# tambetm/simple_dqn

Hardware: AMD Instinct MI355X
Metric: train_steps/sec (batch=32, 4x84x84 uint8) (higher is better)
Workload: dtype f32; 1 GPU; BASELINE.json configs[1]: Breakout shapes, batch_size=32, replay_size=1000000, num_actions=4, HIP Q-net + device replay gather fused into conv1; global_batch=32, parallelism=dp1 (independent learners, RCCL grad all-reduce), ring=HBM mirror

## Files before the change

simple_dqn_amd/csrc/api_internal.h:

```cpp
#pragma once
#include <hip/hip_runtime.h>
#include <dlfcn.h>
#include <stdarg.h>
#include <stdio.h>
#include <stdlib.h>
#include <math.h>
#include <string.h>
#include <string>
#include <vector>
#include <chrono>
#include <thread>

#include "../../include/sdqn.h"
#include "kernels.h"
#include "generic_net.h"
#include "sampler.h"
#include "sdqn_per.h"

using namespace sdqn;


static constexpr int Q_SLOT_FLOATS = 8 * ACT_Q_STRIDE;
static constexpr int COST_RING = 64;
static constexpr int Q_SLOTS = 8;
// ... 44 lines not shown
};
inline bool replay_idx_ok(const sdqn_replay_s* r, int64_t i) {
  if (!r->lanes) return i >= r->hist && i + r->ns.n - 1 < r->count;
  if (i < 0 || i >= r->size) return false;
  const int64_t l = i % r->lane_len;
  return l >= r->hist && l + r->ns.n - 1 < r->lane_fill;
}
inline int64_t replay_filled(const sdqn_replay_s* r) { return r->lanes ? r->lanes * r->lane_fill : r->count; }
extern std::vector<sdqn_replay_s*> g_replays;

struct Id128 { char b[128]; };
struct Rccl {
  void* lib = nullptr;
  int (*GetUniqueId)(void*) = nullptr;
  int (*CommInitRank)(void**, int, Id128, int) = nullptr;
  int (*AllReduce)(const void*, void*, size_t, int, int, void*, hipStream_t) = nullptr;
  int (*Broadcast)(const void*, void*, size_t, int, int, void*, hipStream_t) = nullptr;
  int (*CommDestroy)(void*) = nullptr;
  int (*CommSplit)(void*, int, int, void**, void*) = nullptr;
  int (*CommAbort)(void*) = nullptr;
  int (*GroupStart)() = nullptr;
  int (*GroupEnd)() = nullptr;
  const char* (*GetErrorString)(int) = nullptr;
  int (*CommCount)(void*, int*) = nullptr;
  int (*CommUserRank)(void*, int*) = nullptr;
  int (*CommCuDevice)(void*, int*) = nullptr;
};
extern Rccl g_rccl;
#define NCCLCHK(x) do { int e_ = (x); if (e_ != 0) { set_error("%s -> %s", #x, g_rccl.GetErrorString ? g_rccl.GetErrorString(e_) : "rccl error"); return SDQN_ERR_RCCL; } } while (0)

struct ProfPair { int id; hipEvent_t a, b; };
struct sdqn_net_s {
  GenericNet* gen = nullptr;
  sdqn_net_cfg cfg; int B = 0, A = 0; int64_t NP = 0;
  int64_t NPW = 0;
  bool bn = false;
  float *x1 = nullptr, *x2 = nullptr, *x3 = nullptr;
  float *bn_mean = nullptr, *bn_rstd = nullptr; double* bn_partial = nullptr;
  float *theta = nullptr, *theta_t = nullptr, *state = nullptr, *state2 = nullptr, *g = nullptr;
  int epoch = 0;
  float *a1 = nullptr, *a2 = nullptr, *a3 = nullptr, *slab4 = nullptr, *a4 = nullptr, *d4 = nullptr;
  float *d3 = nullptr, *d2 = nullptr;
  half_t *h_a1 = nullptr, *h_a2 = nullptr, *h_a3 = nullptr, *h_d4 = nullptr, *h_d3p = nullptr, *h_d3 = nullptr,
         *h_d2p = nullptr, *h_d2 = nullptr, *h_d1 = nullptr, *wh[2] = {nullptr, nullptr}, *wht[2] = {nullptr, nullptr};
  float *d3p = nullptr, *d2p = nullptr, *d1 = nullptr, *slab1 = nullptr, *slab2 = nullptr, *slab3 = nullptr;
  float *q = nullptr, *maxq = nullptr, *dq = nullptr, *cost_terms = nullptr, *cost_out = nullptr; double* cost_accum = nullptr;
  bool double_dqn = false, slots3 = false;
  int n_step = 1;
  uint8_t *st_states = nullptr, *st_act = nullptr, *st_term = nullptr; int64_t* st_rew = nullptr; int64_t* d_idx = nullptr;
  float* h_f = nullptr;
  float *q_host = nullptr, *q_host_dev = nullptr;
  int q_slot = 0;
  bool head_q_system = false;
  float *act_scratch = nullptr, *act_q = nullptr; unsigned* act_ctl = nullptr; unsigned act_seq = 0;
  bool act_on = false, act_last = false, act_inject = false; int act_fallbacks = 0;
  int64_t tuple_calls = 0, tuple_states_skipped = 0, tuple_small_skipped = 0;
  double* cost_ring = nullptr; int cost_steps[64] = {0}; int64_t cost_ticket = 0;
  bool spec_pending = false; const void* spec_sb = nullptr; uint64_t spec_gen = 0;
  uint8_t* h_stage[2] = {nullptr, nullptr}; hipEvent_t stage_ev[2] = {nullptr, nullptr}; bool stage_busy[2] = {false, false}; int stage_next = 0;
  int S4 = 7, S4_cap = 7, tps1 = 1, tps2 = 1, tps3 = 1, ns1 = 1, ns2 = 1, ns3 = 1;
  int64_t train_iterations = 0;
  bool keep_grads = false;
  half_t* gh = nullptr; int* ovf_flag = nullptr; int64_t* ovf_count = nullptr;
  int dp_half = 1, dp_half_scale_log2 = -1;
  bool h16_wgrad_mfma = true;
  int c1w_in_wgrads = 1;
  bool half_payload_pending = false;
  bool grad_only = false;
  int nw_override[12] = {0};
  int f4_share[2] = {100, 0};
  int ns_cap[3] = {1, 1, 1};
  bool bt_xcd = true;
  bool bt_on = true; int bt[K_COUNT] = {0};
  int xcd_mask[K_COUNT] = {0};
  bool xcd_map = false;
  bool conv1_bf16 = true;
  unsigned short* w1p[2] = {nullptr, nullptr};
  const int64_t* host_idx_cur = nullptr;
  int r3_xcd = 2;
  bool prep_inline = true;
  int wt = WT_ALL;
  int conv1w_bf16 = 1;
  bool conv3_c36 = true;
  bool fused_launches = true;
  bool prof_on = false; int prof_filter = -1;
  int prof_mode = 1;
  int prof_every = 1; int64_t prof_seen[K_COUNT] = {0};
  std::vector<ProfPair> prof_pending; std::vector<hipEvent_t> prof_free;
  double prof_ms[K_COUNT]; int64_t prof_n[K_COUNT];
  void* comm = nullptr; int rank = 0, nranks = 1; int nccl_rc = 0;
  void* comm2 = nullptr; hipEvent_t ev_g4 = nullptr, ev_w4 = nullptr; bool w4_pending = false;
  bool dp_sync_replicas = true;
  int dp_overlap_req = -1;
  bool dp_overlap = false;
  int dp_probe_result = -1;
  int wt_kid = -1; unsigned long long* wt_words = nullptr;
  uint8_t* col_win = nullptr; void* col_recs = nullptr; int col_N = 0; int64_t col_t = 0; size_t col_state = 0; int col_game = 0;
  std::vector<void*> allocs;
};
#define GENCHK(x) do { hipError_t ge_ = (x); if (ge_ != hipSuccess) { set_error("%s -> %s", #x, hipGetErrorString(ge_)); return ge_ == hipErrorInvalidValue ? SDQN_ERR_ARG : SDQN_ERR_HIP; } } while (0)

constexpr int SB_SLOTS = 64;
uint64_t next_statebuf_gen();
struct sdqn_statebuf_s {
  uint8_t* d = nullptr;
  uint8_t* host = nullptr;
  uint8_t* stage = nullptr;
  int hist = 0;
  int64_t frame = 0;
  int pos = 0;
  uint64_t gen = next_statebuf_gen();
};

enum StepStructure { STEP_FUSED = 0, STEP_H16_BT = 1, STEP_DP_OVERLAP = 2, STEP_UNFUSED = 3 };
enum UpdateForm { UPD_SINGLE = 0, UPD_DP_SERIAL = 1, UPD_DP_OVERLAP = 2, UPD_GRAD_ONLY = 3 };
int ensure_stream();
int sample_checked(uint32_t* mt, const uint8_t* terminals, int64_t count, int64_t current, int hist,
                          int batch, int64_t* idx_out, int64_t* draws_out, int nstep = 1);
int sample_checked_lanes(uint32_t* mt, const uint8_t* terminals, int lanes, int64_t lane_len, int64_t fill, int64_t pos, int hist,
                         int batch, int64_t* idx_out, int64_t* draws_out, int nstep);
int replay_sample_uniform(sdqn_replay_s* r, uint32_t* mt, int64_t* idx_out, int64_t* draws_out);
int nstep_match(const sdqn_net_s* h, const sdqn_replay_s* r);
double nstep_gamma_n(int n, double gamma);
int replay_free(sdqn_replay_s* r);
int64_t replay_add_meta(sdqn_replay_s* r, int action, int64_t reward, int terminal);
int replay_add_commit(sdqn_replay_s* r, int64_t c);
int replay_flush_pending(sdqn_replay_s* r);
int replay_push_idx(sdqn_replay_s* r, const int64_t* idx, int* slot_out, const int64_t** dev);
int replay_release_idx(sdqn_replay_s* r, int slot);
int replay_release_idx_batched(sdqn_replay_s* r, int slot, bool flush);
GatherArgs gather_args(sdqn_replay_s* r, const int64_t* didx);
int replay_gather_generic(sdqn_replay_s* r, const int64_t* didx);
int rccl_load(const char* path);
int dalloc(sdqn_net_s* h, void** p, size_t bytes, bool zero = true);
int net_free(sdqn_net_s* h);
float* which_buf(sdqn_net_s* h, int which);
bool bn_layer_span(sdqn_net_s* h, int which, int layer, float** base, int64_t* n);
int gen_set(sdqn_net_s* h, int which, int layer, const void* w, int64_t n, bool f64);
int gen_get(sdqn_net_s* h, int which, int layer, void* w, int64_t n, bool f64);
int prof_collect(sdqn_net_s* h);
int prof_event(sdqn_net_s* h, hipEvent_t* e);
hipError_t dp_allreduce(sdqn_net_s* h, void* buf, size_t count, int dtype, void* comm, hipStream_t s);
StepArgs step_args(sdqn_net_s* h);
HeadArgs head_args(sdqn_net_s* h, int train);
int join_comm(sdqn_net_s* h);
BnArgs bn_args(sdqn_net_s* h, const StepArgs& a, int layer, int train);
hipError_t launch_tuned(sdqn_net_s* h, int id, StepArgs a, hipStream_t s, int variant = 0);
int run_forward(sdqn_net_s* h, const StepArgs& a, const HeadArgs& hd);
UpdateArgs make_update_args(sdqn_net_s* h, const StepArgs& a);
StepStructure step_structure(const sdqn_net_s* h);
UpdateForm update_form(const sdqn_net_s* h);
int run_train(sdqn_net_s* h, const StepArgs& a, const HeadArgs& hd, const PrepArgs* next = nullptr);
int read_cost(sdqn_net_s* h, float* cost_out);
int read_mean_cost(sdqn_net_s* h, int n_steps, float* mean_cost);
int predict_forward_tuned(sdqn_net_s* h, const uint8_t* states, const HeadArgs& hd, int B = 0);
int predict_forward(sdqn_net_s* h, const uint8_t* states, int rows, const void** q, int* q_f64);
StepArgs ring_step_args(sdqn_net_s* h, const sdqn_replay_s* r);
int run_ring_step(sdqn_net_s* h, sdqn_replay_s* r, const int64_t* host_idx, const HeadArgs& hd, const PrepArgs* next = nullptr);
int check_replay_geometry(const sdqn_net_s* h, const sdqn_replay_s* r);
bool act_sum_partials(const float* part, int A, float* q_out);
const uint8_t* statebuf_window(sdqn_statebuf_s* s);
int statebuf_advance(sdqn_statebuf_s* s, uint8_t** host_frame, uint8_t** dev_slot);
int predict_state_enqueue(sdqn_net_s* h, sdqn_statebuf_s* sb);
bool act_trace();
int predict_state_collect(sdqn_net_s* h, float* q_out);
PrepArgs prep_args(sdqn_net_s* h, sdqn_replay_s* r, const int64_t* pinned_idx);
// ... 47 lines not shown
```

simple_dqn_amd/csrc/gemm_engine.h:

```cpp
#pragma once
#include <hip/hip_runtime.h>
#include <string.h>
#include "problems.h"
#include "launch.h"

namespace sdqn {

typedef float f32x16 __attribute__((ext_vector_type(16)));

template <class P, class = void> struct a_elem { typedef float type; };
template <class P> struct a_elem<P, decltype((void)sizeof(typename P::AT))> { typedef typename P::AT type; };
template <class P, class = void> struct b_elem { typedef float type; };
template <class P> struct b_elem<P, decltype((void)sizeof(typename P::BT))> { typedef typename P::BT type; };
template <class P, class = void> struct stages_lds { static constexpr bool value = false; };
template <class P> struct stages_lds<P, decltype((void)P::STAGE_LDS)> { static constexpr bool value = P::STAGE_LDS; };
template <class P> struct Staged : P { static constexpr bool STAGE_LDS = true; };
template <class P, class = void> struct a_group4 { static constexpr bool value = false; };
template <class P> struct a_group4<P, decltype((void)P::A_GROUP4)> { static constexpr bool value = P::A_GROUP4; };
template <class P, class = void> struct uses_f16_wgrad { static constexpr bool value = false; };
template <class P> struct uses_f16_wgrad<P, decltype((void)P::F16_WGRAD)> { static constexpr bool value = P::F16_WGRAD; };
template <class P, class = void> struct has_preload { static constexpr bool value = false; };
template <class P> struct has_preload<P, decltype((void)P::PRELOAD)> { static constexpr bool value = P::PRELOAD; };
template <class P, class = void> struct has_preload_multi { static constexpr bool value = false; };
template <class P> struct has_preload_multi<P, decltype((void)P::PRELOAD_MULTI)> { static constexpr bool value = P::PRELOAD_MULTI; };
template <class P, class = void> struct uses_f16_mfma { static constexpr bool value = false; };
template <class P> struct uses_f16_mfma<P, decltype((void)P::F16_MFMA)> { static constexpr bool value = P::F16_MFMA; };

constexpr int PANEL = 32 * 33;

__device__ __forceinline__ void wave_lds_sync() {
  __builtin_amdgcn_fence(__ATOMIC_RELEASE, "wavefront");
  __builtin_amdgcn_wave_barrier();
  __builtin_amdgcn_fence(__ATOMIC_ACQUIRE, "wavefront");
}


__device__ __forceinline__ int pick_half(int v, int s, bool hi) {
  const int lo = __builtin_amdgcn_readlane(v, s), up = __builtin_amdgcn_readlane(v, s + 4);
  return hi ? up : lo;
}
__device__ __forceinline__ int64_t pick_half(int64_t v, int s, bool hi) {
  const int i = s;
  const int l0 = __builtin_amdgcn_readlane((int)(v & 0xFFFFFFFF), i), l1 = __builtin_amdgcn_readlane((int)(v >> 32), i);
  const int u0 = __builtin_amdgcn_readlane((int)(v & 0xFFFFFFFF), i + 4), u1 = __builtin_amdgcn_readlane((int)(v >> 32), i + 4);
  const int64_t lo = ((int64_t)l1 << 32) | (uint32_t)l0, up = ((int64_t)u1 << 32) | (uint32_t)u0;
  return hi ? up : lo;
}

#ifdef SDQN_TIMING
__device__ unsigned long long* g_sdqn_dbg = nullptr;
#define SDQN_STAMP(ph) do { if (g_sdqn_dbg && threadIdx.x == 0) g_sdqn_dbg[((size_t)(blockIdx.x + gridDim.x * (blockIdx.y + gridDim.y * blockIdx.z)) * 8) + (ph)] = clock64(); } while (0)
__device__ unsigned long long* g_sdqn_wdbg = nullptr;
__device__ unsigned g_sdqn_wdbg_blocks = 0;
#define SDQN_WSTAMP_DECL unsigned long long wst_[4] = {0, 0, 0, 0}
#define SDQN_WSTAMP(ph) do { if (wst_[ph] == 0) wst_[ph] = clock64(); } while (0)
#define SDQN_WSTAMP_FLUSH do { unsigned long long* wd_ = g_sdqn_wdbg; if (wd_ && (threadIdx.x & 63) == 0) { \
  const size_t b_ = (size_t)(blockIdx.x + gridDim.x * (blockIdx.y + gridDim.y * blockIdx.z)); const unsigned nb_ = g_sdqn_wdbg_blocks; \
  if (b_ < nb_ && (threadIdx.x >> 6) < 16) { \
    for (int q_ = 0; q_ < 4; ++q_) wd_[(b_ * 16 + (threadIdx.x >> 6)) * 4 + q_] = wst_[q_]; \
    if (threadIdx.x == 0) { unsigned x_; asm volatile("s_getreg_b32 %0, hwreg(HW_REG_XCC_ID, 0, 4)" : "=s"(x_)); wd_[(size_t)nb_ * 64 + b_] = x_; } } } } while (0)
#else
#define SDQN_STAMP(ph) do {} while (0)
#define SDQN_WSTAMP_DECL do {} while (0)
#define SDQN_WSTAMP(ph) do {} while (0)
#define SDQN_WSTAMP_FLUSH do {} while (0)
#endif

template <class P, int NW>
constexpr int tile_lds() {
  return NW * PANEL * (stages_lds<P>::value && (P::A_K || P::B_K) ? ((P::A_K ? 1 : 0) + (P::B_K ? 1 : 0)) : 1);
}

__device__ __forceinline__ constexpr int kslot(int t, int h) { return 8 * (t >> 2) + 4 * h + (t & 3); }

template <class T>
__device__ __forceinline__ T ld_byte_off(const T* base, uint32_t byte_off) {
  return *reinterpret_cast<const T*>(reinterpret_cast<const char*>(base) + byte_off);
}

template <class P, int NW, int NT>
__device__ __forceinline__ void gemm_tile(const StepArgs& a, int bx, int by, int bz, float* smem) {
  constexpr bool STG = stages_lds<P>::value;
  constexpr bool STG_A = STG && P::A_K, STG_B = STG && P::B_K;
  constexpr int WAVE_LDS = PANEL * ((STG_A || STG_B) ? ((STG_A ? 1 : 0) + (STG_B ? 1 : 0)) : 1);
  typedef typename P::aoff_t aoff_t;

  SDQN_STAMP(0);
  SDQN_WSTAMP_DECL;
  const int lane = threadIdx.x & 63;
  const int wave = __builtin_amdgcn_readfirstlane(threadIdx.x >> 6);
  const int m0 = bx * 32, n0 = by * 32;
  int z, ks, kbeg, kend;
  P::ksplit(a, bz, z, ks, kbeg, kend);
  if (NW * 64 < NT && wave >= NW) kend = kbeg;
  const int M = P::M(a), N = P::N(a);
  const int hb = lane >> 5;
  const bool hi = lane >= 32;

  const int mrow = m0 + (lane & 31), ncol = n0 + (lane & 31);
  const aoff_t arow = P::a_row(a, z, mrow < M ? mrow : M - 1);
  const int bcol = P::b_col(a, z, ncol < N ? ncol : N - 1);
  typedef typename a_elem<P>::type AT; typedef typename b_elem<P>::type BT;
  const AT* abase = P::a_ptr(a, z);
  const BT* bbase = P::b_ptr(a, z);
  const AT* areg = nullptr; const BT* breg = nullptr;
  if constexpr (!P::A_K && P::A_REG) areg = abase + (uint32_t)arow + (hi ? 4 * P::A_LD : 0);
  if constexpr (!P::B_K && P::B_REG) breg = bbase + (uint32_t)bcol + (hi ? 4 * P::B_LD : 0);
// ... 296 lines not shown
      else pa = P::a_ptr(a, z) + (uint32_t)(arow16 + P::a_col(a, z, kk));
      pa0 = ld_half8(pa); pa1 = ld_half8(pa + 8);
      if (kl >= kend) { pa0 = zero; pa1 = zero; }
    }
  };
  int kc = kbeg + (wave < NW ? wave : 0) * 32;
  if (kc < kend) stage_load(kc);
  while (kc < kend) {
    *reinterpret_cast<half8*>(sb + i * HW_PITCH + 16 * hb) = pb0;
    *reinterpret_cast<half8*>(sb + i * HW_PITCH + 16 * hb + 8) = pb1;
    if constexpr (!P::A_U8) {
      *reinterpret_cast<half8*>(sa + i * HW_PITCH + 16 * hb) = pa0;
      *reinterpret_cast<half8*>(sa + i * HW_PITCH + 16 * hb + 8) = pa1;
    }
    const aoff_t cv = cvn;
    const int kcur = kc;
    kc += NW * 32;
    if (kc < kend) stage_load(kc);
    wave_lds_sync();
#pragma unroll
    for (int s = 0; s < 2; ++s) {
      half8 fa, fb;
#pragma unroll
      for (int j = 0; j < 8; ++j) fb[j] = sb[(16 * s + 8 * hb + j) * HW_PITCH + i];
      if constexpr (P::A_U8) {
#pragma unroll
        for (int g = 0; g < 2; ++g) {
          const int src = 16 * s + 4 * g;
          const int l0 = __builtin_amdgcn_readlane((int)(cv & 0xFFFFFFFF), src), l1 = __builtin_amdgcn_readlane((int)((int64_t)cv >> 32), src);
          const int u0 = __builtin_amdgcn_readlane((int)(cv & 0xFFFFFFFF), src + 8), u1 = __builtin_amdgcn_readlane((int)((int64_t)cv >> 32), src + 8);
          const int64_t lo = ((int64_t)l1 << 32) | (uint32_t)l0, up = ((int64_t)u1 << 32) | (uint32_t)u0;
          const int64_t c = hi ? up : lo;
          const bool ok = kcur + 16 * s + 8 * hb + 4 * g < kend;
          const f4 v = P::a_load_group4(a, z, arow_own + c);
          fa[4 * g] = ok ? (half_t)v.x : (half_t)0.0f; fa[4 * g + 1] = ok ? (half_t)v.y : (half_t)0.0f;
          fa[4 * g + 2] = ok ? (half_t)v.z : (half_t)0.0f; fa[4 * g + 3] = ok ? (half_t)v.w : (half_t)0.0f;
        }
      } else {
#pragma unroll
        for (int j = 0; j < 8; ++j) fa[j] = sa[(16 * s + 8 * hb + j) * HW_PITCH + i];
      }
      acc = __builtin_amdgcn_mfma_f32_32x32x16_f16(fa, fb, acc, 0, 0, 0);
    }
    wave_lds_sync();
  }

  if constexpr (NW > 1) {
    if (wave < NW) {
      float* cw = smem + wave * HW_WAVE_LDS;
#pragma unroll
      for (int r = 0; r < 16; ++r) cw[((r & 3) + 8 * (r >> 2) + 4 * hb) * 33 + i] = acc[r];
    }
    __syncthreads();
    for (int e = threadIdx.x; e < 1024; e += NT) {
      const int ml = e >> 5, nl = e & 31;
      float v = smem[ml * 33 + nl];
#pragma unroll
      for (int w = 1; w < NW; ++w) v += smem[w * HW_WAVE_LDS + ml * 33 + nl];
      if (m0 + ml < M && n0 + nl < N) P::store(a, z, ks, m0 + ml, n0 + nl, v);
    }
  } else {
    float v[16];
#pragma unroll
    for (int r = 0; r < 16; ++r) v[r] = acc[r];
    P::store16(a, z, ks, m0, n0, lane, M, N, v, epi);
  }
}

template <class P, int NW, int NT>
__device__ __forceinline__ void run_tile(const StepArgs& a, int bx, int by, int bz, float* smem) {
  if constexpr (uses_f16_wgrad<P>::value) gemm_tile_hw<P, NW, NT>(a, bx, by, bz, smem);
  else if constexpr (uses_f16_mfma<P>::value) gemm_tile_h<P, NW, NT>(a, bx, by, bz, smem);
  else gemm_tile<P, NW, NT>(a, bx, by, bz, smem);
}
template <class P, int NW>
constexpr int tile_lds_any() {
  if constexpr (uses_f16_wgrad<P>::value) return NW * HW_WAVE_LDS;
  else return uses_f16_mfma<P>::value ? NW * PANEL : tile_lds<P, NW>();
}
template <class P> constexpr int tile_m() { return 32; }
template <class P> constexpr int tile_n() { return 32; }


template <class P, int NW>
__global__ void __launch_bounds__(NW * 64) gemm_kernel(const StepArgs a) {
  __shared__ float smem[tile_lds_any<P, NW>()];
  if constexpr (has_preload<P>::value) P::preload(a, gridDim.x, gridDim.y, gridDim.z);
  const int gx = gridDim.x, gy = gridDim.y;
  const int lin = blockIdx.x + gx * (blockIdx.y + gy * blockIdx.z);
  const int t = (a.xcd_map & 1) ? xcd_tile_id(lin, gx * gy * gridDim.z) : lin;
  const int bz = t / (gx * gy), r = t - bz * (gx * gy);
  run_tile<P, NW, NW * 64>(a, r % gx, r / gx, bz, smem);
}

struct MultiDims { int n[3]; int gx[3], gy[3]; };

template <class P, int NW, int NT>
__device__ __forceinline__ void multi_dispatch(const StepArgs& a, const MultiDims& d, int which, int local, float* smem) {
  if constexpr (NW == 1) {
    const int wave = __builtin_amdgcn_readfirstlane(threadIdx.x >> 6);
    const int t = local * (NT / 64) + wave;
    const int per_z = d.gx[which] * d.gy[which];
    if (t < a.f4w_count) {
      const int tile = a.f4w_first + t;
      const int bz = tile / per_z, r = tile - bz * per_z;
      run_tile<P, 1, 64>(a, r % d.gx[which], r / d.gx[which], bz, smem);
    }
  } else {
    const int per_z = d.gx[which] * d.gy[which];
    const int bz = local / per_z, r = local - bz * per_z;
    run_tile<P, NW, NT>(a, r % d.gx[which], r / d.gx[which], bz, smem);
  }
}

template <int NT, class P0, int NW0, class P1, int NW1, class P2, int NW2>
__global__ void __launch_bounds__(NT) gemm_multi_kernel(const StepArgs a, const MultiDims d) {
  constexpr int L0 = tile_lds_any<P0, NW0>() * (NW0 == 1 ? NT / 64 : 1), L1 = tile_lds_any<P1, NW1>() * (NW1 == 1 ? NT / 64 : 1),
                L2 = tile_lds_any<P2, NW2>() * (NW2 == 1 ? NT / 64 : 1);
  constexpr int L = L0 > L1 ? (L0 > L2 ? L0 : L2) : (L1 > L2 ? L1 : L2);
  __shared__ float smem[L];
  if constexpr (has_preload_multi<P1>::value) P1::preload_multi(a, d);
  const int b = blockIdx.x;
  const int xm = a.xcd_map;
  if (b < d.n[0]) multi_dispatch<P0, NW0, NT>(a, d, 0, (xm & 1) ? xcd_tile_id_range(b, 0, d.n[0]) : b, smem);
  else if (b < d.n[0] + d.n[1]) multi_dispatch<P1, NW1, NT>(a, d, 1, (xm & 2) ? xcd_tile_id_range(b, d.n[0], d.n[1]) : b - d.n[0], smem);
  else multi_dispatch<P2, NW2, NT>(a, d, 2, (xm & 4) ? xcd_tile_id_range(b, d.n[0] + d.n[1], d.n[2]) : b - d.n[0] - d.n[1], smem);
}

struct NoProblem {
  static constexpr bool A_K = false, B_K = false; typedef int aoff_t; struct Epi {};
  static constexpr bool A_REG = false, A_U8 = false, B_REG = false; static constexpr int A_LD = 0, B_LD = 0;
  SDQN_HD static const float* a_ptr(const StepArgs&, int) { return nullptr; }
  SDQN_HD static const float* b_ptr(const StepArgs&, int) { return nullptr; }
  SDQN_HD static int M(const StepArgs&) { return 0; }
  SDQN_HD static int N(const StepArgs&) { return 0; }
  SDQN_HD static int nbz(const StepArgs&) { return 0; }
  SDQN_HD static void ksplit(const StepArgs&, int, int& z, int& ks, int& kb, int& ke) { z = ks = kb = ke = 0; }
  SDQN_HD static int a_row(const StepArgs&, int, int) { return 0; }
  SDQN_HD static int a_col(const StepArgs&, int, int) { return 0; }
  SDQN_HD static float a_load(const StepArgs&, int, int) { return 0.f; }
  SDQN_HD static f4 a_load4(const StepArgs&, int, int) { f4 o; o.x = o.y = o.z = o.w = 0.f; return o; }
  SDQN_HD static f4 b_load4(const StepArgs&, int, int) { f4 o; o.x = o.y = o.z = o.w = 0.f; return o; }
  SDQN_HD static int b_row(const StepArgs&, int, int) { return 0; }
  SDQN_HD static int b_col(const StepArgs&, int, int) { return 0; }
  SDQN_HD static float b_load(const StepArgs&, int, int) { return 0.f; }
  SDQN_HD static void store(const StepArgs&, int, int, int, int, float) {}
  __device__ static void epi_begin(const StepArgs&, int, int, int, Epi&) {}
  __device__ static void store16(const StepArgs&, int, int, int, int, int, int, int, const float*, Epi&) {}
};

template <class P, int NW>
inline hipError_t launch_gemm(const StepArgs& a, hipStream_t stream) {
  dim3 grid((P::M(a) + tile_m<P>() - 1) / tile_m<P>(), (P::N(a) + tile_n<P>() - 1) / tile_n<P>(), P::nbz(a));
  SDQN_LAUNCH((gemm_kernel<P, NW>), grid, dim3(NW * 64), 0, stream, a);
  return hipGetLastError();
}

template <int NT, class P, int NW>
inline void multi_fill(const StepArgs& a, MultiDims& d, int i) {
  d.gx[i] = (P::M(a) + tile_m<P>() - 1) / tile_m<P>(); d.gy[i] = (P::N(a) + tile_n<P>() - 1) / tile_n<P>();
  const int tiles = d.gx[i] * d.gy[i] * P::nbz(a);
  d.n[i] = NW == 1 ? (a.f4w_count + NT / 64 - 1) / (NT / 64) : tiles;
}
template <int NT, class P0, int NW0, class P1, int NW1, class P2, int NW2>
inline hipError_t launch_multi(const StepArgs& a, bool has1, bool has2, hipStream_t stream) {
  static_assert(NW0 * 64 <= NT && NW1 * 64 <= NT && NW2 * 64 <= NT, "waves per tile exceed the workgroup");
  MultiDims d; memset(&d, 0, sizeof d);
  multi_fill<NT, P0, NW0>(a, d, 0);
  if (has1) multi_fill<NT, P1, NW1>(a, d, 1);
  if (has2) multi_fill<NT, P2, NW2>(a, d, 2);
  if (d.n[0] + d.n[1] + d.n[2] == 0) return hipSuccess;
  SDQN_LAUNCH((gemm_multi_kernel<NT, P0, NW0, P1, NW1, P2, NW2>), dim3(d.n[0] + d.n[1] + d.n[2]), dim3(NT), 0, stream, a, d);
  return hipGetLastError();
}

}
```

simple_dqn_amd/csrc/kernels.h:

```cpp
#pragma once
#include <cstddef>
#include <hip/hip_runtime.h>
#include "problems.h"
#include "launch.h"

namespace sdqn {

enum KernelId {
  K_CONV1_FWD = 0, K_CONV2_FWD, K_CONV3_FWD, K_FC4_FWD, K_HEAD,
  K_FC4_DGRAD, K_FC4_WGRAD, K_CONV3_DGRAD, K_CONV3_WGRAD, K_CONV2_DGRAD, K_CONV2_WGRAD,
  K_CONV1_WGRAD, K_UPDATE, K_ALLREDUCE, K_GATHER, K_PREP,
  K_BWD3,
  K_BWD2,
  K_BWD1,
  K_BN,
  K_RESERVED_20, K_RESERVED_21, K_RESERVED_22, K_RESERVED_23,
  K_WGRADS,
  K_ACT,
  K_COLLECT,
  K_COUNT
};
static_assert(K_BN == 19 && K_WGRADS == 24 && K_ACT == 25 && K_COLLECT == 26 && K_COUNT == 27, "kernel ids are public numbers");
const char* kernel_name(int id);


struct HeadArgs {
  const uint8_t* st_actions;
  const int64_t* st_rewards;
  const uint8_t* st_terminals;
  float* q;
  float* maxq;
  float* dq;
  float* cost_terms;
  double discount, min_reward, max_reward;
  float clip_error;
  int train;
  int reserved_[6];
  const float* per_w; float* per_p; double per_alpha, per_eps;
  int nstep; double gamma_n;
};

struct PrepArgs {
  const int64_t* idx_pinned;
  const MetaRec* meta;
  int64_t* idx;
  uint8_t* actions;
  int64_t* rewards;
  uint8_t* terminals;
  int B;
  int idx_in_valid;
  int64_t idx_in[32];
  NStepArgs ns;
};

struct UpdateArgs {
  float* theta;
  float* state;
  float* g;
  const float* slab[3];
  int ns[3];
  const float* dq;
  const float* a4;
  const float* cost_terms;
  float* cost_out;
  double* cost_accum;
  int B, A;
  int mode;
  int skip_fc4;
  int only_fc4;
  PrepArgs next;
  float bsz;
  float rho, one_minus_rho, lr, eps;
  int opt;
  float* state2;
  float beta1, one_minus_beta1, beta2, one_minus_beta2, lr_t;
  half_t* wh;
  half_t* wht;
  unsigned short* w1p;
  int reserved_[4];
  int wt;
  int reserved2_[3];
  int64_t bn_first;
  const int* ovf_flag;
  int64_t* ovf_count;
  int ovf_dynamic;
};

static_assert(sizeof(HeadArgs) == 160 && offsetof(HeadArgs, train) == 84 && offsetof(HeadArgs, per_w) == 112 && offsetof(HeadArgs, per_eps) == 136 &&
              offsetof(HeadArgs, nstep) == 144 && offsetof(HeadArgs, gamma_n) == 152, "HeadArgs layout");
static_assert(sizeof(PrepArgs) == 344 && offsetof(PrepArgs, idx_in_valid) == 52 && offsetof(PrepArgs, idx_in) == 56 && offsetof(PrepArgs, ns) == 312, "PrepArgs layout");
static_assert(sizeof(UpdateArgs) == 616 && offsetof(UpdateArgs, next) == 128 && offsetof(UpdateArgs, next) + offsetof(PrepArgs, idx_in) == 184 &&
              offsetof(UpdateArgs, bsz) == 472 && offsetof(UpdateArgs, w1p) == 544 && offsetof(UpdateArgs, wt) == 568 && offsetof(UpdateArgs, bn_first) == 584 &&
              offsetof(UpdateArgs, ovf_flag) == 592 && offsetof(UpdateArgs, ovf_count) == 600 && offsetof(UpdateArgs, ovf_dynamic) == 608, "UpdateArgs layout");

struct BnArgs {
  int layer;
  int C, rows;
  int nz;
  int train;
  const float* x;
  int S4, B;
  float* a;
  float* theta[2];
  int64_t off_bn;
  double* partial;
  float* mean; float* rstd;
  float* d;
  float* dpad;
  int PQ, Qw, PD, pad;
  float* g;
};

struct GatherArgs {
  const uint8_t* ring;
  const MetaRec* meta;
  const int64_t* idx;
  uint8_t* pre;
  uint8_t* post;
  uint8_t* actions;
  int64_t* rewards;
  uint8_t* terminals;
  int B;
  NStepArgs ns;
};

#if defined(__HIPCC__)
__device__ inline float opt_apply(float w, float& s1, float& s2, float gsum, const UpdateArgs& u) {
  if (u.opt == 0) return rms_step(w, s1, gsum, u.bsz, u.rho, u.one_minus_rho, u.lr, u.eps);
  const float g = div_bsz(gsum, u.bsz);
  if (u.opt == 1) {
    s1 = s1 * u.beta1 + u.one_minus_beta1 * g;
    s2 = s2 * u.beta2 + (u.one_minus_beta2 * g) * g;
    return w - (u.lr_t * s1) / (sqrtf(s2) + u.eps);
  }
  s1 = s1 * u.rho + (u.one_minus_rho * g) * g;
  const float upd = sqrtf((s2 + u.eps) / (s1 + u.eps)) * g;
  s2 = s2 * u.rho + (u.one_minus_rho * upd) * upd;
  return w - upd;
}
#endif

enum LaunchVariant {
  LV_CONV3_C36 = 2,
  LV_CONV1_FWD_BF16 = 4,
  LV_CONV1_WGRAD_BF16 = 8,
  LV_C1W_IN_WGRADS = 16,
  LV_C1W_FIRST = 32,
};
enum WriteThrough {
  WT_CONV2_FWD = 1, WT_CONV3_FWD = 2, WT_FC4_FWD = 4, WT_FC4_DGRAD = 8, WT_BWD3 = 16, WT_BWD2 = 32, WT_CONV1_WGRAD = 64, WT_CONV1_FWD = 128,
  WT_UPDATE = 256, WT_ALL = 511
};
struct LaunchTune {
  int nw_override[12];
  const int64_t* host_idx;
  int r3_xcd;
  int wt;
  int bt[K_COUNT];
  int variant;
};
hipError_t launch_kernel(int id, const StepArgs& a, const LaunchTune& t, hipStream_t s);
hipError_t launch_head(const StepArgs& a, const HeadArgs& h, hipStream_t s, bool q_system_scope = false);
// ... 30 lines not shown
```

simple_dqn_amd/csrc/problems.h:

```cpp
#pragma once
#include <stddef.h>
#include <stdint.h>
#include <math.h>

#if defined(__HIPCC__)
#define SDQN_HD __host__ __device__ inline
#else
#define SDQN_HD inline
#endif

namespace sdqn {

constexpr int H0 = 84, W0 = 84, C0 = 4;
constexpr int FRAME = H0 * W0;
constexpr int STATE = C0 * FRAME;
constexpr int ST1 = 4, P1 = 20, Q1 = 20, K1 = 32;
constexpr int ST2 = 2, P2 = 9, Q2 = 9, K2 = 64;
constexpr int P3 = 7, Q3 = 7, K3 = 64;
constexpr int PIX1 = P1 * Q1, PIX2 = P2 * Q2, PIX3 = P3 * Q3;
constexpr int CRS1 = 256, CRS2 = 512, CRS3 = 576;
constexpr int NFC = 512, NIN4 = PIX3 * K3;
constexpr int PD3 = 11, PD2 = 11;
constexpr int NW1 = CRS1 * K1, NW2 = CRS2 * K2, NW3 = CRS3 * K3, NW4 = NIN4 * NFC;
constexpr int OFF1 = 0, OFF2 = OFF1 + NW1, OFF3 = OFF2 + NW2, OFF4 = OFF3 + NW3, OFF5 = OFF4 + NW4;
constexpr int MAX_ACTIONS = 18;
constexpr int BN_LAYERS = 4;
constexpr int BN_PARAMS = 2 * (32 + 64 + 64 + 512);
SDQN_HD constexpr int bn_features(int l) { return l == 0 ? 32 : (l == 3 ? 512 : 64); }
SDQN_HD constexpr int bn_off(int l) { return l == 0 ? 0 : (l == 1 ? 64 : (l == 2 ? 192 : 320)); }

#if defined(__HIPCC__)
typedef _Float16 half_t;
typedef _Float16 half8 __attribute__((ext_vector_type(8)));
#else
typedef uint16_t half_t;
#endif

struct MetaRec {
  int64_t reward;
  uint8_t action;
  uint8_t terminal;
  uint8_t pad[6];
};

struct NStepArgs { int n, pad_; double gamma, min_reward, max_reward; };
SDQN_HD void nstep_return(const MetaRec* meta, int64_t i, const NStepArgs& s, double& R, uint8_t& done) {
  double r = 0.0, g = 1.0; uint8_t d = 0;
  for (int k = 0; k < s.n; ++k) {
    const MetaRec rec = meta[i + k];
    double c = (double)rec.reward;
    c = c < s.min_reward ? s.min_reward : (c > s.max_reward ? s.max_reward : c);
    r = r + g * c;
    if (rec.terminal) { d = 1; break; }
    g = g * s.gamma;
  }
  R = r; done = d;
}
SDQN_HD void stage_meta(const MetaRec* meta, int64_t i, const NStepArgs& s, uint8_t* act, int64_t* rew, uint8_t* term, int n) {
  const MetaRec rec = meta[i];
  act[n] = rec.action;
  if (s.n > 1) {
    double R; uint8_t d; nstep_return(meta, i, s, R, d);
    reinterpret_cast<double*>(rew)[n] = R; term[n] = d;
  } else { rew[n] = rec.reward; term[n] = rec.terminal; }
}

struct StepArgs {
  const uint8_t* src;
  const int64_t* idx;
  int from_ring;
  int B, A, nz;
  const float* theta[2];
  float* a1;
  float* a2;
  float* a3;
  float* slab4;
  float* a4;
  float* d4;
  float* d3p;
  float* d2p;
  float* d3;
  float* d2;
  float* d1;
  float* g;
  float* slab1;
  float* slab2;
  float* slab3;
  int S4;
  int tps1, tps2, tps3;
  int fuse_rms;
  int f4w_first, f4w_count;
  half_t *h_a1, *h_a2, *h_a3;
  half_t *h_d4, *h_d3p, *h_d3, *h_d2p, *h_d2, *h_d1;
  const half_t* wh[2];
  const half_t* wht[2];
  half_t *wh_w, *wht_w;
  float loss_scale, inv_loss_scale;
  int h16;
  int xcd_map;
  int post_off;
  int reserved_[11];
  float* __restrict__ theta_w;
  float* __restrict__ state;
  float bsz, rho, one_minus_rho, lr, eps;
  int bn;
  int reserved2_[6];
  const unsigned short* w1p[2];
  int reserved3_[8];
};

static_assert(sizeof(StepArgs) == 496 && offsetof(StepArgs, post_off) == 336 && offsetof(StepArgs, theta_w) == 384 && offsetof(StepArgs, bn) == 420 &&
              offsetof(StepArgs, w1p) == 448, "StepArgs layout: part of the tuned kernels (reserved_)");

SDQN_HD float div_bsz(float x, float bsz) {
  union { float f; uint32_t u; } b, r; b.f = bsz;
  if ((b.u & 0x007FFFFFu) == 0u && b.u >= 0x00800000u && b.u < 0x7E800000u) { r.u = 0x7F000000u - b.u; return x * r.f; }
  return x / bsz;
}
SDQN_HD float rms_step(float w, float& st, float gsum, float bsz, float rho, float omr, float lr, float eps) {
  const float g = div_bsz(gsum, bsz);
  st = rho * st + (g * g) * omr;
  return w - (g * lr) / (sqrtf(st + eps) + eps);
}

#if defined(__HIPCC__)
typedef float f2v __attribute__((ext_vector_type(2)));
__device__ inline void rms_step2(float& w0, float& w1, float& st0, float& st1, float gs0, float gs1,
                                 float bsz, float rho, float omr, float lr, float eps) {
  union { float f; uint32_t u; } b, r; b.f = bsz;
  f2v gsum = {gs0, gs1}, g;
  if ((b.u & 0x007FFFFFu) == 0u && b.u >= 0x00800000u && b.u < 0x7E800000u) { r.u = 0x7F000000u - b.u; g = gsum * r.f; }
  else { g.x = gs0 / bsz; g.y = gs1 / bsz; }
  f2v st = {st0, st1};
  const f2v a = rho * st, q = (g * g) * omr;
  st = a + q;
  const f2v num = g * lr, rad = st + eps;
  f2v den; den.x = sqrtf(rad.x); den.y = sqrtf(rad.y);
  den = den + eps;
  f2v quo; quo.x = num.x / den.x; quo.y = num.y / den.y;
  const f2v w = (f2v){w0, w1} - quo;
  w0 = w.x; w1 = w.y; st0 = st.x; st1 = st.y;
}
#endif

SDQN_HD uint16_t bf16_rn(float f) {
  union { float f; uint32_t u; } x; x.f = f;
  return (uint16_t)((x.u + 0x7FFFu + ((x.u >> 16) & 1u)) >> 16);
}
SDQN_HD float bf16_up(uint16_t b) { union { float f; uint32_t u; } x; x.u = (uint32_t)b << 16; return x.f; }
SDQN_HD void split_bf16x3(float w, uint16_t& hi, uint16_t& mid, uint16_t& lo) {
  hi = bf16_rn(w); const float r1 = w - bf16_up(hi);
  mid = bf16_rn(r1); const float r2 = r1 - bf16_up(mid);
  lo = bf16_rn(r2);
}
constexpr int W1P_PLANE = K1 * CRS1;

SDQN_HD int wslot(int z) { return z & 1; }
SDQN_HD int sslot(int z) { return z != 0 ? 1 : 0; }
SDQN_HD int soff(int post_off, int z) { return z != 0 ? post_off : 0; }
SDQN_HD int64_t slab4_row(const StepArgs& a, int ks, int z) { return z < 2 ? (int64_t)ks * 2 + z : (int64_t)2 * a.S4 + ks; }
SDQN_HD int64_t sbase(const StepArgs& a, int z, int n) {
  return a.from_ring ? (a.idx[n] - C0 + soff(a.post_off, z)) * (int64_t)FRAME : ((int64_t)sslot(z) * a.B + n) * (int64_t)STATE;
}
SDQN_HD float norm_u8(uint32_t v) {
  const float x = (float)v, r = 1.0f / 255.0f;
  const float q = x * r;
  const float e = fmaf(-q, 255.0f, x);
  return fmaf(e, r, q);
}
struct f4 { float x, y, z, w; };
SDQN_HD f4 ld4(const float* p) {
#if defined(__HIP_DEVICE_COMPILE__)
  const float4 v = *reinterpret_cast<const float4*>(p); f4 o; o.x = v.x; o.y = v.y; o.z = v.z; o.w = v.w; return o;
#else
  f4 o; o.x = p[0]; o.y = p[1]; o.z = p[2]; o.w = p[3]; return o;
#endif
}
constexpr int SRC_PAD = 16;
SDQN_HD f4 ld4_u8_stride4(const uint8_t* p) {
  f4 o;
#if defined(__HIP_DEVICE_COMPILE__)
  typedef uint32_t u32x4 __attribute__((ext_vector_type(4), aligned(1)));
  const u32x4 w = *reinterpret_cast<const u32x4*>(p);
  o.x = norm_u8(w.x & 255u); o.y = norm_u8(w.y & 255u); o.z = norm_u8(w.z & 255u); o.w = norm_u8(w.w & 255u);
// ... 491 lines not shown
```

simple_dqn_amd/csrc/problems_wt.h:

```cpp
#pragma once
#include "gemm_engine.h"

namespace sdqn {

#ifndef SDQN_NT_W4
#define SDQN_NT_W4 0
#endif
constexpr bool NT_W4 = SDQN_NT_W4 != 0;
#ifndef SDQN_PRELOAD
#define SDQN_PRELOAD 1
#endif
#define SDQN_TOUCH(...) asm volatile("" :: __VA_ARGS__)
#define SDQN_PRELOAD_MULTI_DEF \
  static constexpr bool PRELOAD_MULTI = SDQN_PRELOAD != 0; \
  __device__ static void preload_multi(const StepArgs& a, const MultiDims& d) { \
    SDQN_TOUCH("s"(a.d3p), "s"(a.theta[0]), "s"(a.a2), "s"(a.d2p), "s"(a.d2), "s"(a.d3), "s"(a.slab3), "s"(a.a3), "s"(a.d4), "s"(a.theta_w), "s"(a.state), \
               "s"(a.g), "s"(a.a1), "s"(a.d1), "s"(a.slab2), "s"(a.B), "s"(a.tps2), "s"(a.tps3), "s"(a.fuse_rms), "s"(a.f4w_first), "s"(a.f4w_count), \
               "s"(a.xcd_map), "s"(a.bsz), "s"(a.rho), "s"(a.one_minus_rho), "s"(a.lr), "s"(a.eps), "s"(d.n[0]), "s"(d.n[1]), "s"(d.gx[1])); \
  }
#ifdef SDQN_WT_PLAIN
__device__ __forceinline__ void wt_store(float* p, float v) { *p = v; }
#else
__device__ __forceinline__ void wt_store(float* p, float v) { __hip_atomic_store(p, v, __ATOMIC_RELAXED, __HIP_MEMORY_SCOPE_AGENT); }
#endif
struct Conv2FwdWT : Conv2Fwd {
  static constexpr bool PRELOAD = SDQN_PRELOAD != 0;
  __device__ static void preload(const StepArgs& a, unsigned g0, unsigned g1, unsigned g2) { SDQN_TOUCH("s"(a.a1), "s"(a.a2), "s"(a.theta[0]), "s"(a.theta[1]), "s"(a.B), "s"(a.nz), "s"(a.xcd_map), "s"(g0), "s"(g1), "s"(g2)); }

  __device__ static void store(const StepArgs& a, int z, int, int m, int n, float v) { wt_store(&a.a2[((int64_t)z * M(a) + m) * K2 + n], fmaxf(v, 0.0f)); }
};
struct Conv3FwdWT : Conv3Fwd {
  static constexpr bool PRELOAD = SDQN_PRELOAD != 0;
  __device__ static void preload(const StepArgs& a, unsigned g0, unsigned g1, unsigned g2) { SDQN_TOUCH("s"(a.a2), "s"(a.a3), "s"(a.theta[0]), "s"(a.theta[1]), "s"(a.B), "s"(a.nz), "s"(a.xcd_map), "s"(g0), "s"(g1), "s"(g2)); }

  __device__ static void store(const StepArgs& a, int z, int, int m, int n, float v) { wt_store(&a.a3[((int64_t)z * M(a) + m) * K3 + n], fmaxf(v, 0.0f)); }
};
__device__ __forceinline__ f4 ld4_nt(const float* p) {
  typedef float v4f __attribute__((ext_vector_type(4)));
  const v4f v = __builtin_nontemporal_load(reinterpret_cast<const v4f*>(p)); f4 o; o.x = v.x; o.y = v.y; o.z = v.z; o.w = v.w; return o;
}
struct Fc4FwdWT : Fc4Fwd {
  static constexpr bool PRELOAD = SDQN_PRELOAD != 0;
  __device__ static void preload(const StepArgs& a, unsigned g0, unsigned g1, unsigned g2) { SDQN_TOUCH("s"(a.a3), "s"(a.slab4), "s"(a.theta[0]), "s"(a.theta[1]), "s"(a.B), "s"(a.nz), "s"(a.S4), "s"(a.xcd_map), "s"(g0), "s"(g1), "s"(g2)); }

  __device__ static f4 b_load4(const StepArgs& a, int z, int o) { return NT_W4 ? ld4_nt(a.theta[wslot(z)] + OFF4 + o) : ld4(a.theta[wslot(z)] + OFF4 + o); }
  __device__ static void store(const StepArgs& a, int z, int ks, int m, int n, float v) { wt_store(&a.slab4[(slab4_row(a, ks, z) * a.B + m) * NFC + n], v); }
};
struct Fc4DgradWT : Fc4Dgrad {
  static constexpr bool PRELOAD = SDQN_PRELOAD != 0;
  __device__ static void preload(const StepArgs& a, unsigned g0, unsigned g1, unsigned g2) { SDQN_TOUCH("s"(a.d4), "s"(a.theta[0]), "s"(a.a3), "s"(a.d3p), "s"(a.d3), "s"(a.B), "s"(a.xcd_map), "s"(g0), "s"(g1), "s"(g2)); }

  __device__ static f4 b_load4(const StepArgs& a, int, int o) { return NT_W4 ? ld4_nt(a.theta[0] + OFF4 + o) : ld4(a.theta[0] + OFF4 + o); }
  static constexpr bool GATED = true;
  __device__ static float gate_load(const StepArgs& a, int, int m, int n) { return a.a3[(int64_t)m * NIN4 + n]; }
  __device__ static void store_gated(const StepArgs& a, int, int, int m, int n, float v, float g) {
    const int pix = n >> 6, f = n & 63, p = pix / Q3, q = pix - p * Q3;
    const float dv = g > 0.0f ? v : 0.0f;
    wt_store(&a.d3p[((m * PD3 + p + 2) * PD3 + q + 2) * K3 + f], dv);
    wt_store(&a.d3[(int64_t)m * NIN4 + n], dv);
  }
  __device__ static void store(const StepArgs& a, int z, int ks, int m, int n, float v) { store_gated(a, z, ks, m, n, v, gate_load(a, z, m, n)); }
};
struct Conv3DgradWT : Conv3Dgrad {
  static constexpr bool PRELOAD = SDQN_PRELOAD != 0;
  SDQN_PRELOAD_MULTI_DEF
  __device__ static void preload(const StepArgs& a, unsigned g0, unsigned g1, unsigned g2) { SDQN_TOUCH("s"(a.d3p), "s"(a.theta[0]), "s"(a.a2), "s"(a.d2p), "s"(a.d2), "s"(a.B), "s"(g0), "s"(g1), "s"(g2)); }

  static constexpr bool GATED = true;
  __device__ static float gate_load(const StepArgs& a, int, int m, int c) { return a.a2[(int64_t)m * K2 + c]; }
  __device__ static void store_gated(const StepArgs& a, int, int, int m, int c, float v, float g) {
    const float dv = g > 0.0f ? v : 0.0f;
    wt_store(&a.d2p[prow2(m) + c], dv);
    wt_store(&a.d2[(int64_t)m * K2 + c], dv);
  }
  __device__ static void store(const StepArgs& a, int z, int ks, int m, int c, float v) { store_gated(a, z, ks, m, c, v, gate_load(a, z, m, c)); }
};
struct Conv3WgradWT : Conv3Wgrad {
  static constexpr bool PRELOAD = SDQN_PRELOAD != 0;
  SDQN_PRELOAD_MULTI_DEF
  __device__ static void preload(const StepArgs& a, unsigned g0, unsigned g1, unsigned g2) { SDQN_TOUCH("s"(a.a2), "s"(a.d3), "s"(a.slab3), "s"(a.tps3), "s"(a.B), "s"(g0), "s"(g1), "s"(g2)); }

  __device__ static void store(const StepArgs& a, int, int ks, int m, int n, float v) { wt_store(&a.slab3[(int64_t)ks * NW3 + m * K3 + n], v); }
};
struct Conv2DgradWT : Conv2Dgrad {
  static constexpr bool PRELOAD = SDQN_PRELOAD != 0;
  SDQN_PRELOAD_MULTI_DEF
  __device__ static void preload(const StepArgs& a, unsigned g0, unsigned g1, unsigned g2) { SDQN_TOUCH("s"(a.d2p), "s"(a.theta[0]), "s"(a.a1), "s"(a.d1), "s"(a.B), "s"(g0), "s"(g1), "s"(g2)); }

  static constexpr bool GATED = true;
  __device__ static int out_off(int z, int m, int c) {
    const int py = z >> 1, px = z & 1;
    const int n = m / 100, pix = m - n * 100, i = pix / 10, j = pix - i * 10;
    return ((n * P1 + 2 * i + py) * Q1 + 2 * j + px) * K1 + c;
  }
  __device__ static float gate_load(const StepArgs& a, int z, int m, int c) { return a.a1[out_off(z, m, c)]; }
  __device__ static void store_gated(const StepArgs& a, int z, int, int m, int c, float v, float g) { wt_store(&a.d1[out_off(z, m, c)], g > 0.0f ? v : 0.0f); }
  __device__ static void store(const StepArgs& a, int z, int ks, int m, int c, float v) { store_gated(a, z, ks, m, c, v, gate_load(a, z, m, c)); }
};
struct Conv2WgradWT : Conv2Wgrad {
  static constexpr bool PRELOAD = SDQN_PRELOAD != 0;
  __device__ static void preload(const StepArgs& a, unsigned g0, unsigned g1, unsigned g2) { SDQN_TOUCH("s"(a.a1), "s"(a.d2), "s"(a.slab2), "s"(a.tps2), "s"(a.B), "s"(g0), "s"(g1), "s"(g2)); }

  __device__ static void store(const StepArgs& a, int, int ks, int m, int n, float v) { wt_store(&a.slab2[(int64_t)ks * NW2 + m * K2 + n], v); }
};
struct Conv1WgradWT : Conv1Wgrad {
  __device__ static void store(const StepArgs& a, int, int ks, int m, int n, float v) { wt_store(&a.slab1[(int64_t)ks * NW1 + m * K1 + n], v); }
};
struct Fc4WgradWT : Fc4Wgrad {
  __device__ static void preload(const StepArgs& a, unsigned g0, unsigned g1, unsigned g2) { SDQN_TOUCH("s"(a.a3), "s"(a.d4), "s"(a.theta_w), "s"(a.state), "s"(a.g), "s"(a.fuse_rms), "s"(a.f4w_first), "s"(a.f4w_count), "s"(a.B)); SDQN_TOUCH("s"(a.bsz), "s"(a.rho), "s"(a.one_minus_rho), "s"(a.lr), "s"(a.eps), "s"(g0), "s"(g1), "s"(g2)); }
  __device__ static void store(const StepArgs& a, int, int, int m, int n, float v) {
    const int64_t e = OFF4 + (int64_t)m * NFC + n;
    if (a.fuse_rms) { float st = a.state[e]; const float w = rms_step(a.theta_w[e], st, v, a.bsz, a.rho, a.one_minus_rho, a.lr, a.eps); wt_store(&a.theta_w[e], w); wt_store(&a.state[e], st); }
    else wt_store(&a.g[e], v);
  }
  __device__ static void store16(const StepArgs& a, int z, int ks, int m0, int n0, int lane, int M, int N, const float* v, Epi& e) {
    const uint32_t base = epi_base(m0, n0, lane);
    auto stw = [](float* p, uint32_t off, float x) { wt_store(reinterpret_cast<float*>(reinterpret_cast<char*>(p) + off), x); };
    if (!a.fuse_rms) {
#pragma unroll
      for (int r = 0; r < 16; ++r) stw(a.g, base + epi_row(r), v[r]);
      return;
    }
#pragma unroll
    for (int r = 0; r < 16; r += 2) rms_step2(e.w[r], e.w[r + 1], e.st[r], e.st[r + 1], v[r], v[r + 1], a.bsz, a.rho, a.one_minus_rho, a.lr, a.eps);
#pragma unroll
    for (int r = 0; r < 16; ++r) { stw(a.theta_w, base + epi_row(r), e.w[r]); stw(a.state, base + epi_row(r), e.st[r]); }
  }
};

struct Fc4WgradBT : Fc4WgradWT {
  struct Epi {};
  __device__ static void epi_begin(const StepArgs&, int, int, int, Epi&) {}
  static constexpr bool STORE_TILE = true;
  __device__ static void store_tile(const StepArgs& a, int m0, int n0, int lane, const float* v) {
    const uint32_t base = epi_base(m0, n0, lane);
    auto stw = [](float* p, uint32_t off, float x) { wt_store(reinterpret_cast<float*>(reinterpret_cast<char*>(p) + off), x); };
    if (!a.fuse_rms) {
#pragma unroll
      for (int r = 0; r < 16; ++r) stw(a.g, base + epi_row(r), v[r]);
      return;
    }
    const float* __restrict__ tw = a.theta_w; const float* __restrict__ sp = a.state;
#pragma unroll
    for (int g = 0; g < 4; ++g) {
      float w[4], st[4];
#pragma unroll
      for (int e = 0; e < 4; ++e) { w[e] = ldb(tw, base + epi_row(4 * g + e)); st[e] = ldb(sp, base + epi_row(4 * g + e)); }
      rms_step2(w[0], w[1], st[0], st[1], v[4 * g], v[4 * g + 1], a.bsz, a.rho, a.one_minus_rho, a.lr, a.eps);
      rms_step2(w[2], w[3], st[2], st[3], v[4 * g + 2], v[4 * g + 3], a.bsz, a.rho, a.one_minus_rho, a.lr, a.eps);
#pragma unroll
      for (int e = 0; e < 4; ++e) { stw(a.theta_w, base + epi_row(4 * g + e), w[e]); stw(a.state, base + epi_row(4 * g + e), st[e]); }
      __builtin_amdgcn_sched_barrier(0);
    }
  }
};

}
```

simple_dqn_amd/csrc/sdqn_api_net.hip:

```cpp
#include "api_internal.h"

static const char* const RETIRED_OPTIONS[] = {"hoist", "two_streams", "fuse_dbg", "fwd_rb", "head_f4d", "fuse_upd", "f4w_early", "bt_planes", "bt_x", "bwd_order", nullptr};
#define RETIRED_OPTION_REFUSED(NAME) do { set_error("option %s belonged to an experiment that was measured slower than the default step and has been removed from " \
                                                    "the library (tools/exp/README.md; tools/exp/experiments_r04.patch)", NAME); return SDQN_ERR_ARG; } while (0)

int dalloc(sdqn_net_s* h, void** p, size_t bytes, bool zero) {
  HIPCHK(hipMalloc(p, bytes)); h->allocs.push_back(*p);
  if (zero) HIPCHK(hipMemsetAsync(*p, 0, bytes, g_stream));
  return SDQN_OK;
}
int net_free(sdqn_net_s* h) {
  if (!h) return SDQN_OK;
  if (g_stream) hipStreamSynchronize(g_stream);
  delete h->gen; h->gen = nullptr;
  if (g_comm) hipStreamSynchronize(g_comm);
  if (h->comm2 && g_rccl.CommDestroy) g_rccl.CommDestroy(h->comm2);
  if (h->comm && g_rccl.CommDestroy) g_rccl.CommDestroy(h->comm);
  if (h->ev_g4) hipEventDestroy(h->ev_g4);
  if (h->ev_w4) hipEventDestroy(h->ev_w4);
  for (void* p : h->allocs) hipFree(p);
  hipHostFree(h->h_f);
  if (h->q_host) hipHostFree(h->q_host);
  if (h->cost_ring) hipHostFree(h->cost_ring);
  for (int i = 0; i < 2; ++i) { if (h->h_stage[i]) hipHostFree(h->h_stage[i]); if (h->stage_ev[i]) hipEventDestroy(h->stage_ev[i]); }
// ... 357 lines not shown
  if (h->gen) { GENCHK(h->gen->last_q(preq, maxpostq, false)); return SDQN_OK; }
  const size_t nq = (size_t)h->B * h->A;
  HIPCHK(hipMemcpyAsync(h->h_f, h->q, nq * 4, hipMemcpyDeviceToHost, g_stream));
  HIPCHK(hipMemcpyAsync(h->h_f + nq, h->maxq, (size_t)h->B * 4, hipMemcpyDeviceToHost, g_stream));
  HIPCHK(hipStreamSynchronize(g_stream));
  if (preq) memcpy(preq, h->h_f, nq * 4);
  if (maxpostq) memcpy(maxpostq, h->h_f + nq, (size_t)h->B * 4);
  return SDQN_OK;
}
extern "C" int sdqn_net_overflow_steps(sdqn_net_t h, int64_t* n) {
  ARGCHK(h && n, "NULL argument");
  *n = 0;
  if (!h->ovf_count) return SDQN_OK;
  { int rc = join_comm(h); if (rc) return rc; } HIPCHK(hipStreamSynchronize(g_stream));
  HIPCHK(hipMemcpy(n, h->ovf_count, 8, hipMemcpyDeviceToHost));
  return SDQN_OK;
}
extern "C" int sdqn_net_train_iterations(sdqn_net_t h, int64_t* n) { ARGCHK(h && n, "NULL"); *n = h->train_iterations; return SDQN_OK; }

extern "C" int sdqn_net_set_epoch(sdqn_net_t h, int epoch) { ARGCHK(h && epoch >= 0, "bad epoch"); h->epoch = epoch; return SDQN_OK; }

extern "C" int sdqn_net_set_option(sdqn_net_t h, const char* name, int value) {
  ARGCHK(h && name, "NULL argument");
  if (!strcmp(name, "n_step")) {
    ARGCHK(value >= 1 && value <= SDQN_MAX_N_STEP, "n_step %d out of range [1, %d]", value, SDQN_MAX_N_STEP);
    h->n_step = value;
    if (h->gen) h->gen->set_nstep(value, nstep_gamma_n(value, h->cfg.discount_rate));
    return SDQN_OK;
  }
  if (h->gen) {
    if (!strcmp(name, "dp_overlap") && value < 0) return SDQN_OK;
    if (!strcmp(name, "double_dqn")) {
      ARGCHK(value == 0 || value == 1, "double_dqn must be 0 or 1");
      GENCHK(h->gen->set_double_dqn(value != 0));
      return SDQN_OK;
    }
    if (!strcmp(name, "grad_only") || !strcmp(name, "dp_overlap") || !strcmp(name, "keep_gradients")) {
      ARGCHK(value == 0 || !strcmp(name, "keep_gradients"), "option %s is implemented for the 84x84x4 float32 / float16 configurations", name);
    }
    return SDQN_OK;
  }
  bool retired = !strncmp(name, "rb:", 3) || !strncmp(name, "btx:", 4);
  for (int i = 0; RETIRED_OPTIONS[i]; ++i) retired = retired || !strcmp(name, RETIRED_OPTIONS[i]);
  if (retired) { if (value) RETIRED_OPTION_REFUSED(name); return SDQN_OK; }
  if (!strcmp(name, "double_dqn")) {
    ARGCHK(value == 0 || value == 1, "double_dqn must be 0 or 1");
    if (value && !h->slots3) {
      { int rc_ = join_comm(h); if (rc_) return rc_; } HIPCHK(hipStreamSynchronize(g_stream));
      const size_t B = (size_t)h->B;
      float** f32[5] = {&h->a1, &h->a2, &h->a3, &h->a4, &h->q};
      const size_t n32[5] = {B * PIX1 * K1, B * PIX2 * K2, B * PIX3 * K3, B * NFC, B * h->A};
      for (int i = 0; i < 5; ++i) { int r_ = dalloc(h, (void**)f32[i], 3 * n32[i] * 4); if (r_) return r_; }
      { int r_ = dalloc(h, (void**)&h->slab4, (size_t)h->S4_cap * 3 * B * NFC * 4); if (r_) return r_; }
      if (h->h_a1) {
        half_t** f16[3] = {&h->h_a1, &h->h_a2, &h->h_a3};
        const size_t n16[3] = {B * PIX1 * K1, B * PIX2 * K2, B * PIX3 * K3};
        for (int i = 0; i < 3; ++i) { int r_ = dalloc(h, (void**)f16[i], 3 * n16[i] * 2); if (r_) return r_; }
      }
      HIPCHK(hipStreamSynchronize(g_stream));
      h->slots3 = true;
    }
    h->double_dqn = value != 0;
  }
  else if (!strcmp(name, "keep_gradients")) h->keep_grads = value != 0;
  else if (!strcmp(name, "grad_only")) h->grad_only = value != 0;
  else if (!strcmp(name, "h16_wgrad_mfma")) h->h16_wgrad_mfma = value != 0;
  else if (!strcmp(name, "c1w_in_wgrads")) { if (value < 0 || value > 2) { set_error("bad c1w_in_wgrads (0..2)"); return SDQN_ERR_ARG; } h->c1w_in_wgrads = value; }
  else if (!strcmp(name, "dp_half")) h->dp_half = value != 0;
  else if (!strcmp(name, "dp_half_scale_log2")) {
    ARGCHK(value >= -1 && value <= 40 && h->ovf_flag, "bad scale (or not a float16 network)");
    { int rc_ = join_comm(h); if (rc_) return rc_; } HIPCHK(hipStreamSynchronize(g_stream));
    h->dp_half_scale_log2 = value;
    const int st0[4] = {0, value < 0 ? 10 : value, 0, 0};
    HIPCHK(hipMemcpy(h->ovf_flag, st0, 16, hipMemcpyHostToDevice));
  }
  else if (!strcmp(name, "dp_half_scale_seed")) {
    ARGCHK(value >= 0 && value <= 15 && h->ovf_flag, "bad scale seed (0..15; float16 networks only)");
    { int rc_ = join_comm(h); if (rc_) return rc_; } HIPCHK(hipStreamSynchronize(g_stream));
    h->dp_half_scale_log2 = -1;
    const int st0[4] = {0, value, 0, 0};
    HIPCHK(hipMemcpy(h->ovf_flag, st0, 16, hipMemcpyHostToDevice));
  }
  else if (!strcmp(name, "fused_launches")) h->fused_launches = value != 0;
  else if (!strcmp(name, "conv1_bf16")) h->conv1_bf16 = value != 0;
  else if (!strcmp(name, "wt")) h->wt = value;
  else if (!strcmp(name, "prep_inline")) h->prep_inline = value != 0;
  else if (!strcmp(name, "r3_xcd")) h->r3_xcd = value;
  else if (!strcmp(name, "conv1w_bf16")) h->conv1w_bf16 = value;
  else if (!strcmp(name, "conv3_c36")) h->conv3_c36 = value != 0;
  else if (!strcmp(name, "xcd_map")) h->xcd_map = value != 0;
  else if (!strcmp(name, "dp_sync_replicas")) h->dp_sync_replicas = value != 0;
  else if (!strcmp(name, "dp_overlap")) {
    ARGCHK(value >= -2 && value <= 1, "dp_overlap must be -1 (auto), 0 or 1 (-2: auto also for a 1-rank communicator, tests)");
    ARGCHK(!h->comm, "dp_overlap is chosen before sdqn_dp_init (afterwards: sdqn_dp_set_overlap)");
    h->dp_overlap_req = value; h->dp_overlap = value == 1;
  }
  else if (!strcmp(name, "f4_share3")) h->f4_share[0] = value;
  else if (!strcmp(name, "f4_share2")) h->f4_share[1] = value;
  else if (!strcmp(name, "profile_mode")) { ARGCHK(value == 0 || value == 1, "profile_mode must be 0 (event markers) or 1 (kernel-packet timestamps)"); h->prof_mode = value; }
  else if (!strcmp(name, "profile_every")) { ARGCHK(value >= 1, "profile_every must be >= 1"); h->prof_every = value; }
  else if (!strncmp(name, "xcd:", 4)) {
    int id = atoi(name + 4);
    if (id < 0 || id >= K_COUNT || value < 0 || value > 8) { set_error("bad xcd override"); return SDQN_ERR_ARG; }
    h->xcd_mask[id] = value;
  }
  else if (!strcmp(name, "act_inject_failure")) {
    ARGCHK(h->act_scratch, "act_inject_failure needs a network with the one-launch acting forward");
    h->act_inject = value != 0;
  }
  else if (!strcmp(name, "act_kernel")) {
    ARGCHK(value == 0 || h->act_scratch, "act_kernel needs a float32 network without batch_norm");
    h->act_on = value != 0; h->spec_pending = false;
  }
  else if (!strcmp(name, "bt_xcd")) h->bt_xcd = value != 0;
  else if (!strcmp(name, "bt")) h->bt_on = value != 0;
  else if (!strncmp(name, "bt:", 3)) {
    int id = atoi(name + 3);
    if (id < 0 || id >= K_COUNT || value < -1 || value > (id == K_WGRADS ? 2 : 8)) { set_error("bad bt override"); return SDQN_ERR_ARG; }
    h->bt[id] = value;
  }
  else if (!strcmp(name, "s4")) {
    if (value < 1 || value > h->S4_cap) { set_error("bad s4 (1..%d)", h->S4_cap); return SDQN_ERR_ARG; }
    { int rc_ = join_comm(h); if (rc_) return rc_; } HIPCHK(hipStreamSynchronize(g_stream));
    h->S4 = value;
  }
  else if (!strncmp(name, "tps:", 4)) {
    int l = atoi(name + 4);
    if (l < 1 || l > 3 || value < 1) { set_error("bad tps override"); return SDQN_ERR_ARG; }
    const int pix[3] = {PIX1, PIX2, PIX3};
    const int T = ceil_div(h->B * pix[l - 1], 32), ns = ceil_div(T, value);
    if (ns > h->ns_cap[l - 1]) { set_error("tps:%d = %d needs %d slabs (%d allocated)", l, value, ns, h->ns_cap[l - 1]); return SDQN_ERR_ARG; }
    { int rc_ = join_comm(h); if (rc_) return rc_; } HIPCHK(hipStreamSynchronize(g_stream));
    if (l == 1) { h->tps1 = value; h->ns1 = ns; } else if (l == 2) { h->tps2 = value; h->ns2 = ns; } else { h->tps3 = value; h->ns3 = ns; }
  }
  else if (!strncmp(name, "nw:", 3)) {
    int id = atoi(name + 3);
    if (id < 0 || id >= 12 || !(value == 0 || value == 1 || value == 2 || value == 4 || value == 8 || value == 16 || (value == 9 && id == 2))) { set_error("bad nw override"); return SDQN_ERR_ARG; }
    h->nw_override[id] = value;
  }
  else { set_error("unknown option %s", name); return SDQN_ERR_ARG; }
  return SDQN_OK;
}

extern "C" int sdqn_net_debug_read(sdqn_net_t h, const char* name, float* out, int64_t n) {
  ARGCHK(h && name && out, "NULL argument");
  ARGCHK(!h->gen, "debug_read exposes the tuned path's internal buffers (84x84x4 float32 / float16 only)");
  const int B = h->B;
  struct { const char* n; float* p; int64_t len; } tab[] = {
    {"a1", h->a1, (int64_t)2 * B * PIX1 * K1}, {"a2", h->a2, (int64_t)2 * B * PIX2 * K2}, {"a3", h->a3, (int64_t)2 * B * PIX3 * K3},
    {"a4", h->a4, (int64_t)2 * B * NFC}, {"d4", h->d4, (int64_t)B * NFC}, {"d3p", h->d3p, (int64_t)B * PD3 * PD3 * K3},
    {"d2p", h->d2p, (int64_t)B * PD2 * PD2 * K2}, {"d1", h->d1, (int64_t)B * PIX1 * K1}, {"q", h->q, (int64_t)2 * B * h->A},
    {"dq", h->dq, (int64_t)B * h->A}, {"g", h->g, h->NP}, {"theta", h->theta, h->NP}, {"cost_terms", h->cost_terms, B}};
  for (auto& e : tab) if (!strcmp(e.n, name)) {
    ARGCHK(n <= e.len, "buffer %s holds %lld floats", name, (long long)e.len);
    { int rc_ = join_comm(h); if (rc_) return rc_; } HIPCHK(hipStreamSynchronize(g_stream));
    HIPCHK(hipMemcpy(out, e.p, (size_t)n * 4, hipMemcpyDeviceToHost));
    return SDQN_OK;
  }
  set_error("unknown buffer %s", name); return SDQN_ERR_ARG;
}

#ifdef SDQN_TIMING
namespace sdqn { hipError_t set_timing_buffer(unsigned long long* p); }
extern "C" int sdqn_debug_time_kernel(sdqn_net_t h, sdqn_replay_t r, const int64_t* idx_host, int kernel, unsigned long long* out, int max_blocks) {
  ARGCHK(h && r && idx_host && out, "NULL");
  unsigned long long* d = nullptr;
// ... 44 lines not shown
```

simple_dqn_amd/csrc/sdqn_api_step.hip:

```cpp
#include "api_internal.h"

hipError_t dp_allreduce(sdqn_net_s* h, void* buf, size_t count, int dtype, void* comm, hipStream_t s) {
  h->nccl_rc = g_rccl.AllReduce(buf, buf, count, dtype,  0, comm, s);
  return h->nccl_rc == 0 ? hipSuccess : hipErrorUnknown;
}

StepArgs step_args(sdqn_net_s* h) {
  StepArgs a; memset(&a, 0, sizeof a);
  a.B = h->B; a.A = h->A; a.nz = 2; a.theta[0] = h->theta; a.theta[1] = h->theta_t;
  a.a1 = h->a1; a.a2 = h->a2; a.a3 = h->a3; a.slab4 = h->slab4; a.a4 = h->a4; a.d4 = h->d4; a.d3p = h->d3p; a.d2p = h->d2p; a.d3 = h->d3; a.d2 = h->d2;
  a.d1 = h->d1; a.g = h->g; a.slab1 = h->slab1; a.slab2 = h->slab2; a.slab3 = h->slab3;
  a.S4 = h->S4; a.tps1 = h->tps1; a.tps2 = h->tps2; a.tps3 = h->tps3;

  a.xcd_map = h->xcd_map ? 7 : 0;
  if (h->cfg.datatype == 1) {
    a.h16 = h->h16_wgrad_mfma ? 2 : 1; a.h_a1 = h->h_a1; a.h_a2 = h->h_a2; a.h_a3 = h->h_a3; a.h_d4 = h->h_d4; a.h_d3p = h->h_d3p; a.h_d3 = h->h_d3;
    a.h_d2p = h->h_d2p; a.h_d2 = h->h_d2; a.h_d1 = h->h_d1; a.wh[0] = h->wh[0]; a.wh[1] = h->wh[1]; a.wht[0] = h->wht[0]; a.wht[1] = h->wht[1];
    a.wh_w = h->wh[0]; a.wht_w = h->wht[0];
    a.loss_scale = (float)h->cfg.loss_scale; a.inv_loss_scale = (float)(1.0 / h->cfg.loss_scale);
  }
  a.f4w_first = 0; a.f4w_count = (NIN4 / 32) * (NFC / 32);
  a.w1p[0] = h->w1p[0]; a.w1p[1] = h->w1p[1];
  a.fuse_rms = (!h->comm && !h->keep_grads && !h->grad_only && h->cfg.optimizer == 0) ? 1 : 0;
  a.theta_w = h->theta; a.state = h->state; a.bsz = (float)h->B;
  a.rho = (float)h->cfg.decay_rate; a.one_minus_rho = (float)(1.0 - h->cfg.decay_rate);
  a.lr = (float)h->cfg.learning_rate; a.eps = (float)h->cfg.epsilon;
  a.post_off = h->n_step;
  return a;
}
double nstep_gamma_n(int n, double gamma) { double g = 1.0; for (int k = 0; k < n; ++k) g = g * gamma; return g; }
int nstep_match(const sdqn_net_s* h, const sdqn_replay_s* r) {
  const int rn = r->ns.n > 1 ? r->ns.n : 1;
  if (rn == 1 && h->n_step == 1) return SDQN_OK;
  ARGCHK(rn == h->n_step, "replay memory n_step %d != network n_step %d", rn, h->n_step);
  ARGCHK(r->ns.gamma == h->cfg.discount_rate, "replay memory n-step discount %.17g != network discount_rate %.17g", r->ns.gamma, h->cfg.discount_rate);
  ARGCHK(r->ns.min_reward == h->cfg.min_reward && r->ns.max_reward == h->cfg.max_reward,
         "replay memory n-step reward clip [%g, %g] != network [%g, %g]", r->ns.min_reward, r->ns.max_reward, h->cfg.min_reward, h->cfg.max_reward);
  return SDQN_OK;
}
HeadArgs head_args(sdqn_net_s* h, int train) {
  HeadArgs hd; memset(&hd, 0, sizeof hd);
  hd.st_actions = h->st_act; hd.st_rewards = h->st_rew; hd.st_terminals = h->st_term;
  hd.q = h->q; hd.maxq = h->maxq; hd.dq = h->dq; hd.cost_terms = h->cost_terms;
  hd.discount = h->cfg.discount_rate; hd.min_reward = h->cfg.min_reward; hd.max_reward = h->cfg.max_reward;
  hd.clip_error = (float)h->cfg.clip_error; hd.train = train;
  if (h->n_step > 1) { hd.nstep = h->n_step; hd.gamma_n = nstep_gamma_n(h->n_step, h->cfg.discount_rate); }
  return hd;
}
int join_comm(sdqn_net_s* h) {
  if (h->w4_pending) { HIPCHK(hipStreamWaitEvent(g_stream, h->ev_w4, 0)); h->w4_pending = false; }
  return SDQN_OK;
}
BnArgs bn_args(sdqn_net_s* h, const StepArgs& a, int layer, int train) {
  BnArgs b; memset(&b, 0, sizeof b);
  const int pix[4] = {PIX1, PIX2, PIX3, 1};
  b.layer = layer; b.C = bn_features(layer); b.rows = a.B * pix[layer]; b.nz = a.nz; b.train = train; b.B = a.B;
  b.theta[0] = h->theta; b.theta[1] = h->theta_t; b.off_bn = h->NPW; b.partial = h->bn_partial;
  b.mean = h->bn_mean + bn_off(layer) / 2; b.rstd = h->bn_rstd + bn_off(layer) / 2; b.g = h->g;
  switch (layer) {
    case 0: b.x = h->x1; b.a = h->a1; b.d = h->d1; break;
    case 1: b.x = h->x2; b.a = h->a2; b.d = h->d2; b.dpad = h->d2p; b.PQ = PIX2; b.Qw = Q2; b.PD = PD2; b.pad = 1; break;
    case 2: b.x = h->x3; b.a = h->a3; b.d = h->d3; b.dpad = h->d3p; b.PQ = PIX3; b.Qw = Q3; b.PD = PD3; b.pad = 2; break;
    default: b.x = h->slab4; b.S4 = a.S4; b.a = h->a4; b.d = h->d4; break;
  }
  return b;
}
#define XCD_TUNE(ARGS, KID) do { if (h->xcd_mask[KID] > 0) (ARGS).xcd_map = h->xcd_mask[KID] - 1; } while (0)
hipError_t launch_tuned(sdqn_net_s* h, int id, StepArgs a, hipStream_t s, int variant) {
  XCD_TUNE(a, id);
  LaunchTune t;
  for (int i = 0; i < 12; ++i) t.nw_override[i] = h->nw_override[i];
  for (int i = 0; i < K_COUNT; ++i) t.bt[i] = h->bt_on ? h->bt[i] : -1;
  t.variant = variant; t.host_idx = h->host_idx_cur; t.r3_xcd = h->r3_xcd; t.wt = h->wt;
  return launch_kernel(id, a, t, s);
}
int run_forward(sdqn_net_s* h, const StepArgs& a, const HeadArgs& hd) {
  if (h->bn) {
    StepArgs f = a; f.bn = 1;
    f.a1 = h->x1; LAUNCH(K_CONV1_FWD, launch_tuned(h, K_CONV1_FWD, f, g_stream)); f.a1 = h->a1;
    LAUNCH(K_BN, launch_bn_forward(bn_args(h, a, 0, hd.train != 0), g_stream));
    f.a2 = h->x2; LAUNCH(K_CONV2_FWD, launch_tuned(h, K_CONV2_FWD, f, g_stream)); f.a2 = h->a2;
    LAUNCH(K_BN, launch_bn_forward(bn_args(h, a, 1, hd.train != 0), g_stream));
    f.a3 = h->x3; LAUNCH(K_CONV3_FWD, launch_tuned(h, K_CONV3_FWD, f, g_stream)); f.a3 = h->a3;
    LAUNCH(K_BN, launch_bn_forward(bn_args(h, a, 2, hd.train != 0), g_stream));
    { int rc = join_comm(h); if (rc) return rc; }
    LAUNCH(K_FC4_FWD, launch_tuned(h, K_FC4_FWD, f, g_stream));
    LAUNCH(K_BN, launch_bn_forward(bn_args(h, a, 3, hd.train != 0), g_stream));
    LAUNCH(K_HEAD, launch_head(f, hd, g_stream));
    return SDQN_OK;
  }
  StepArgs fm = a; fm.xcd_map = 1;
  LAUNCH(K_CONV1_FWD, launch_tuned(h, K_CONV1_FWD, fm, g_stream, (h->conv1_bf16 && h->nw_override[K_CONV1_FWD] == 0) ? LV_CONV1_FWD_BF16 : 0));
  { StepArgs f2 = fm; if (h->B >= 128) f2.xcd_map = a.xcd_map;
    LAUNCH(K_CONV2_FWD, launch_tuned(h, K_CONV2_FWD, f2, g_stream)); }
  { StepArgs f3 = fm; f3.xcd_map = a.xcd_map;
    const int c36 = (h->conv3_c36 && h->nw_override[K_CONV3_FWD] == 0) ? LV_CONV3_C36 : 0;
    LAUNCH(K_CONV3_FWD, launch_tuned(h, K_CONV3_FWD, f3, g_stream, c36)); }
  { int rc = join_comm(h); if (rc) return rc; }
  LAUNCH(K_FC4_FWD, launch_tuned(h, K_FC4_FWD, fm, g_stream));
  LAUNCH(K_HEAD, launch_head(a, hd, g_stream, h->head_q_system));
  return SDQN_OK;
}
UpdateArgs make_update_args(sdqn_net_s* h, const StepArgs& a) {
  UpdateArgs u; memset(&u, 0, sizeof u);
  u.theta = h->theta; u.state = h->state; u.g = h->g;
  u.slab[0] = h->slab1; u.slab[1] = h->slab2; u.slab[2] = h->slab3; u.ns[0] = h->ns1; u.ns[1] = h->ns2; u.ns[2] = h->ns3;
  u.dq = h->dq; u.a4 = h->a4; u.cost_terms = h->cost_terms; u.cost_out = h->cost_out; u.cost_accum = h->cost_accum;
  u.B = h->B; u.A = h->A;
  u.rho = (float)h->cfg.decay_rate; u.one_minus_rho = (float)(1.0 - h->cfg.decay_rate);
  u.lr = (float)h->cfg.learning_rate; u.eps = (float)h->cfg.epsilon;
  u.skip_fc4 = a.fuse_rms;
  u.opt = h->cfg.optimizer; u.state2 = h->state2;
  if (h->cfg.datatype == 1) { u.wh = h->wh[0]; u.wht = h->wht[0]; }
  u.w1p = h->w1p[0];
  u.wt = (h->wt & WT_UPDATE) ? 1 : 0;
  u.bn_first = h->bn ? h->NPW : 0;
  if (u.opt == 1) {
    const double b1 = h->cfg.beta_1, b2 = h->cfg.beta_2, t = (double)h->epoch + 1.0;
    u.beta1 = (float)b1; u.one_minus_beta1 = (float)(1.0 - b1); u.beta2 = (float)b2; u.one_minus_beta2 = (float)(1.0 - b2);
    u.lr_t = (float)(h->cfg.learning_rate * sqrt(1.0 - pow(b2, t)) / (1.0 - pow(b1, t)));
  }
  return u;
}
StepStructure step_structure(const sdqn_net_s* h) {
  if (h->comm && h->comm2 && h->dp_overlap && h->fused_launches) return STEP_DP_OVERLAP;
  if (h->cfg.datatype == 1 && h->B >= 128 && h->bt_on && !h->bn && h->fused_launches && h->bt[K_CONV3_DGRAD] >= 0 && h->bt[K_CONV2_DGRAD] >= 0 &&
      h->nw_override[K_CONV3_DGRAD] == 0 && h->nw_override[K_CONV2_DGRAD] == 0) return STEP_H16_BT;
  return h->fused_launches ? STEP_FUSED : STEP_UNFUSED;
}
UpdateForm update_form(const sdqn_net_s* h) {
  if (step_structure(h) == STEP_DP_OVERLAP) return UPD_DP_OVERLAP;
  if (h->comm) return UPD_DP_SERIAL;
  return h->grad_only ? UPD_GRAD_ONLY : UPD_SINGLE;
}
extern "C" int sdqn_net_step_structure(sdqn_net_t h, int* structure, int* update) {
  ARGCHK(h && structure && update, "NULL argument");
  if (h->gen) { *structure = 4; *update = 0; return SDQN_OK; }
  *structure = (int)step_structure(h); *update = (int)update_form(h);
  return SDQN_OK;
}
bool ddqn_active(const sdqn_net_s* h) { return h->double_dqn && h->theta_t != h->theta; }
int run_online_post_bn(sdqn_net_s* h, const StepArgs& a) {
  StepArgs p = a; p.nz = 1;
  p.src = a.from_ring ? a.src + (size_t)soff(a.post_off, 1) * FRAME : a.src + (size_t)a.B * STATE;
  HeadArgs hp = head_args(h, 0); hp.q = h->q + (size_t)2 * a.B * h->A;
  return run_forward(h, p, hp);
}
int run_train(sdqn_net_s* h, const StepArgs& a, const HeadArgs& hd0, const PrepArgs* next) {
  HeadArgs hd = hd0;
  StepArgs af = a;
  if (ddqn_active(h)) {
    hd.train = 2;
    if (h->bn) { int rc0 = run_online_post_bn(h, a); if (rc0) return rc0; }
    else af.nz = 3;
  }
  int rc = run_forward(h, af, hd);
  if (rc) return rc;
#define BN_BWD(L) do { if (h->bn) LAUNCH(K_BN, launch_bn_backward(bn_args(h, a, (L), 1), g_stream)); } while (0)
  BN_BWD(3);
  const StepStructure st = step_structure(h);
  const bool c1w = (h->conv1w_bf16 == 2 || (h->conv1w_bf16 == 1 && h->B < 128)) && h->cfg.datatype == 0 && !h->bn && h->nw_override[K_CONV1_WGRAD] == 0;
  const bool bt_xcd = h->B >= 128 && h->cfg.datatype == 0 && h->bt_on && !h->bn && h->bt_xcd;
  { StepArgs fd = a; if (bt_xcd) fd.xcd_map |= 1;
    LAUNCH(K_FC4_DGRAD, launch_tuned(h, K_FC4_DGRAD, fd, g_stream)); }
  BN_BWD(2);
  const int f4_tiles = (NIN4 / 32) * (NFC / 32);
  if (st == STEP_DP_OVERLAP) {
    StepArgs b3 = a, b2 = a, b1 = a;
    b3.f4w_first = 0; b3.f4w_count = f4_tiles; b2.f4w_count = b1.f4w_count = 0;
    LAUNCH(K_BWD3, launch_tuned(h, K_BWD3, b3, g_stream));
    HIPCHK(hipEventRecord(h->ev_g4, g_stream));
    HIPCHK(hipStreamWaitEvent(g_comm, h->ev_g4, 0));
    LAUNCH_ON(g_comm, K_ALLREDUCE, dp_allreduce(h, h->g + OFF4, (size_t)NW4,  7, h->comm2, g_comm));
    UpdateArgs u4 = make_update_args(h, a);
    u4.mode = 2; u4.only_fc4 = 1; u4.skip_fc4 = 0; u4.bsz = (float)h->B * (float)h->nranks;
    LAUNCH_ON(g_comm, K_UPDATE, launch_update(u4, g_comm));
    HIPCHK(hipEventRecord(h->ev_w4, g_comm));
    h->w4_pending = true;
    BN_BWD(1);
    LAUNCH(K_BWD2, launch_tuned(h, K_BWD2, b2, g_stream));
    BN_BWD(0);
    LAUNCH(K_BWD1, launch_tuned(h, K_BWD1, b1, g_stream, c1w ? LV_CONV1_WGRAD_BF16 : 0));
  } else if (st == STEP_H16_BT) {
    StepArgs w = a; w.f4w_first = 0; w.f4w_count = f4_tiles;
    if (h->bt_xcd) w.xcd_map |= 7;
    StepArgs b1 = a; b1.f4w_count = 0; b1.xcd_map |= 2;
    LAUNCH(K_CONV3_DGRAD, launch_tuned(h, K_CONV3_DGRAD, a, g_stream));
// ... 357 lines not shown
```

simple_dqn_amd/csrc/sdqn_kernels.hip:

```cpp
#include "gemm_engine.h"
#include "problems_h16.h"
#include "kernels.h"
#include "update_body.h"

namespace sdqn {

static const char* k_names[K_COUNT] = {
  "conv1_fwd(gather+norm+conv+relu)", "conv2_fwd", "conv3_fwd", "fc4_fwd(splitK)", "head(fc5+td+delta)",
  "fc4_dgrad", "fc4_wgrad", "conv3_dgrad", "conv3_wgrad", "conv2_dgrad", "conv2_wgrad",
  "conv1_wgrad", "update(reduce+fc5wgrad+rmsprop)", "rccl_allreduce", "replay_gather_u8", "prep(idx+meta)",
  "bwd3(conv3_dgrad+conv3_wgrad+fc4_wgrad)", "bwd2(conv2_dgrad+conv2_wgrad+fc4_wgrad)", "bwd1(conv1_wgrad+fc4_wgrad)",
  "batchnorm(layer fwd/bwd)", "reserved", "reserved", "reserved", "reserved",
  "wgrads(fc4+conv3+conv2)", "act(conv1..fc5, one state)", "catch_collect(lockstep)"};
const char* kernel_name(int id) { return (id >= 0 && id < K_COUNT) ? k_names[id] : "?"; }
LaunchEvents& launch_events() { static thread_local LaunchEvents le; return le; }

template <class P>
static hipError_t launch_nw(int nw, const StepArgs& a, hipStream_t s) {
  switch (nw) {
    case 2: return launch_gemm<P, 2>(a, s);
    case 4: return launch_gemm<P, 4>(a, s);
    case 8: return launch_gemm<P, 8>(a, s);
    case 16: return launch_gemm<P, 16>(a, s);
    default: return hipErrorInvalidValue;
// ... 15 lines not shown
    if (handled) return e;
  }
  if (t.variant || t.wt) {
    bool handled = false;
    const hipError_t e = launch_kernel_r3(id, a, t, s, &handled);
    if (handled) return e;
  }
  if (a.h16) {
    bool handled = false;
    const hipError_t e = launch_kernel_ext(id, a, t, s, &handled);
    if (handled) return e;
  }
  if (a.bn) {
    switch (id) {
      case K_CONV1_FWD: return launch_gemm<Conv1FwdRaw, 8>(a, s);
      case K_CONV2_FWD: return a.B >= 128 ? launch_gemm<Staged<Conv2FwdRaw>, 8>(a, s) : launch_gemm<Conv2FwdRaw, 16>(a, s);
      case K_CONV3_FWD: return a.B >= 128 ? launch_gemm<Staged<Conv3FwdRaw>, 8>(a, s) : launch_gemm<Staged<Conv3FwdRaw>, 9>(a, s);
      default: break;
    }
  }
  if (id >= 0 && id < 12 && t.nw_override[id] > 0) {
    const int nw = t.nw_override[id];
    switch (id) {
      case K_CONV1_FWD: return launch_nw<Conv1Fwd>(nw, a, s);
      case K_CONV2_FWD: return launch_nw<Conv2Fwd>(nw, a, s);
      case K_CONV3_FWD: if (nw == 9) return launch_gemm<Staged<Conv3Fwd>, 9>(a, s); return launch_nw<Conv3Fwd>(nw, a, s);
      case K_FC4_FWD: return launch_nw<Fc4Fwd>(nw, a, s);
      case K_FC4_DGRAD: return launch_nw<Fc4Dgrad>(nw, a, s);
      case K_CONV3_DGRAD: return launch_nw<Conv3Dgrad>(nw, a, s);
      case K_CONV3_WGRAD: return launch_nw<Conv3Wgrad>(nw, a, s);
      case K_CONV2_DGRAD: return launch_nw<Conv2Dgrad>(nw, a, s);
      case K_CONV2_WGRAD: return launch_nw<Conv2Wgrad>(nw, a, s);
      case K_CONV1_WGRAD: return launch_nw<Conv1Wgrad>(nw, a, s);
      default: break;
    }
  }
  if (a.B >= 128) {
    switch (id) {
      case K_CONV1_FWD: return launch_gemm<Conv1Fwd, 8>(a, s);
      case K_CONV2_FWD: return launch_gemm<Staged<Conv2Fwd>, 8>(a, s);
      case K_CONV3_FWD: return launch_gemm<Staged<Conv3Fwd>, 8>(a, s);
      case K_FC4_FWD: return launch_gemm<Staged<Fc4Fwd>, 8>(a, s);
      case K_FC4_DGRAD: return launch_gemm<Staged<Fc4Dgrad>, 4>(a, s);
      case K_CONV3_DGRAD: return launch_gemm<Staged<Conv3Dgrad>, 8>(a, s);
      case K_CONV2_DGRAD: return launch_gemm<Staged<Conv2Dgrad>, 8>(a, s);
      case K_BWD3:
        if (a.f4w_count > 0) return launch_multi<512, Fc4Wgrad, 8, Staged<Conv3Dgrad>, 8, Conv3Wgrad, 8>(a, true, true, s);
        return launch_multi<512, NoProblem, 2, Staged<Conv3Dgrad>, 8, Conv3Wgrad, 8>(a, true, true, s);
      case K_BWD2: return launch_multi<512, NoProblem, 2, Staged<Conv2Dgrad>, 8, Conv2Wgrad, 8>(a, true, true, s);
      default: break;
    }
  }
  switch (id) {
    case K_CONV1_FWD: return launch_gemm<Conv1Fwd, 8>(a, s);
    case K_CONV2_FWD: return launch_gemm<Conv2Fwd, 16>(a, s);
    case K_CONV3_FWD: return launch_gemm<Conv3Fwd, 16>(a, s);
    case K_FC4_FWD: return launch_gemm<Staged<Fc4Fwd>, 14>(a, s);
    case K_FC4_DGRAD: return launch_gemm<Staged<Fc4Dgrad>, 16>(a, s);
    case K_FC4_WGRAD:
      if (a.B <= 32) return launch_gemm<Fc4Wgrad, 1>(a, s);
      if (a.B <= 64) return launch_gemm<Fc4Wgrad, 2>(a, s);
      if (a.B <= 128) return launch_gemm<Fc4Wgrad, 4>(a, s);
      return launch_gemm<Fc4Wgrad, 8>(a, s);
    case K_CONV3_DGRAD: return launch_gemm<Staged<Conv3Dgrad>, 8>(a, s);
    case K_CONV3_WGRAD: return launch_gemm<Conv3Wgrad, 8>(a, s);
    case K_CONV2_DGRAD: return launch_gemm<Conv2Dgrad, 8>(a, s);
    case K_CONV2_WGRAD: return launch_gemm<Conv2Wgrad, 8>(a, s);
    case K_CONV1_WGRAD: return launch_gemm<Conv1Wgrad, 16>(a, s);
    case K_BWD3:
      if (a.B <= 32 && a.f4w_count > 0) return launch_multi<512, Staged<Conv3Dgrad>, 8, Conv3Wgrad, 8, Fc4Wgrad, 1>(a, true, true, s);
      if (a.f4w_count > 0) return launch_multi<512, Fc4Wgrad, 8, Staged<Conv3Dgrad>, 8, Conv3Wgrad, 8>(a, true, true, s);
      return launch_multi<512, NoProblem, 2, Staged<Conv3Dgrad>, 8, Conv3Wgrad, 8>(a, true, true, s);
    case K_BWD2:
      if (a.B <= 32 && a.f4w_count > 0) return launch_multi<512, Fc4Wgrad, 1, Conv2Dgrad, 8, Conv2Wgrad, 8>(a, true, true, s);
      return launch_multi<512, NoProblem, 2, Conv2Dgrad, 8, Conv2Wgrad, 8>(a, true, true, s);
    case K_BWD1:
      if (a.B <= 32 && a.f4w_count > 0) return launch_multi<1024, Fc4Wgrad, 1, Conv1Wgrad, 16, NoProblem, 2>(a, true, false, s);
      return launch_multi<1024, NoProblem, 2, Conv1Wgrad, 16, NoProblem, 2>(a, true, false, s);
    default: return hipErrorInvalidValue;
  }
}

template <int AMAX, bool BN, bool QSYS, bool DDQN, bool PER, bool NSTEP>
__global__ void __launch_bounds__(512) head_kernel(const StepArgs a, const HeadArgs h) {
  SDQN_STAMP(0);
  const int n = blockIdx.x, j = threadIdx.x, lane = j & 63, wave = j >> 6;
  constexpr int NZ = (DDQN && !BN) ? 3 : 2;
  __shared__ float prod[NZ * AMAX][NFC];
  __shared__ float sh_q[NZ][AMAX];
  __shared__ float sh_dc;
  __shared__ int sh_act;
  const int nz = a.nz, A = a.A;
  const float* __restrict__ th0 = a.theta[0];
  const float* __restrict__ th1 = a.theta[nz > 1 ? 1 : 0];
  const float* __restrict__ slab = a.slab4;
  float a4v[NZ];
#pragma unroll
  for (int z = 0; z < NZ; ++z) a4v[z] = 0.0f;
  const int64_t sstride = (int64_t)2 * a.B * NFC;
  const int64_t s2base = (int64_t)2 * a.S4 * a.B * NFC + (int64_t)n * NFC + j;
  float t[NZ][7];
  if constexpr (BN) {
#pragma unroll
    for (int z = 0; z < 2; ++z) a4v[z] = a.a4[((int64_t)(z < nz ? z : 0) * a.B + n) * NFC + j];
  } else if (a.S4 == 7) {
#pragma unroll
    for (int z = 0; z < 2; ++z)
#pragma unroll
      for (int s = 0; s < 7; ++s)
        t[z][s] = slab[s * sstride + ((int64_t)(z < nz ? z : 0) * a.B + n) * NFC + j];
    if constexpr (NZ == 3) {
#pragma unroll
      for (int s = 0; s < 7; ++s) t[2][s] = slab[s2base + (int64_t)s * a.B * NFC];
    }
  }
  float w5[2][AMAX];
#pragma unroll
  for (int act = 0; act < AMAX; ++act) {
    const int ac = act < A ? act : A - 1;
    w5[0][act] = th0[OFF5 + ac * NFC + j];
    w5[1][act] = th1[OFF5 + ac * NFC + j];
  }
  int m_act = 0, m_term = 0; int64_t m_rew = 0;
  if (h.train && j == 0) { m_act = h.st_actions[n]; m_rew = h.st_rewards[n]; m_term = h.st_terminals[n]; }
  float m_w = 1.0f;
  if constexpr (PER) { if (j == 0) m_w = h.per_w[n]; }
  m_act = m_act < A ? m_act : A - 1;
  if constexpr (BN) {
  } else if (a.S4 == 7) {
#pragma unroll
    for (int z = 0; z < NZ; ++z) { float v = 0.0f;
#pragma unroll
      for (int s = 0; s < 7; ++s) v += t[z][s];
      a4v[z] = v; }
  } else {
#pragma unroll
    for (int z = 0; z < 2; ++z) { float v = 0.0f;
      if (z < nz) for (int s = 0; s < a.S4; ++s) v += slab[s * sstride + ((int64_t)z * a.B + n) * NFC + j];
      a4v[z] = v; }
    if constexpr (NZ == 3) { float v = 0.0f;
      if (nz > 2) for (int s = 0; s < a.S4; ++s) v += slab[s2base + (int64_t)s * a.B * NFC];
      a4v[2] = v; }
  }
#ifdef SDQN_TIMING
  asm volatile("" :: "v"(a4v[0]), "v"(a4v[1]), "v"(w5[0][0]));
  SDQN_STAMP(1);
#endif
#pragma unroll
  for (int z = 0; z < NZ; ++z) {
    if (z >= nz) continue;
    const float v = fmaxf(a4v[z], 0.0f);
    a4v[z] = v;
    if constexpr (!BN) a.a4[((int64_t)z * a.B + n) * NFC + j] = v;
#pragma unroll
    for (int act = 0; act < AMAX; ++act)
      if (act < A) prod[z * A + act][j] = w5[z & 1][act] * v;
  }
  SDQN_STAMP(2);
  __syncthreads();
  SDQN_STAMP(3);
  for (int row = wave; row < nz * A; row += 8) {
    float p = 0.0f;
#pragma unroll
    for (int k = 0; k < 8; ++k) p += prod[row][lane + 64 * k];
#pragma unroll
    for (int off = 32; off >= 1; off >>= 1) p += __shfl_xor(p, off, 64);
    if (lane == 0) {
      const int z = row / A, act = row - z * A;
      sh_q[z][act] = p;
      if constexpr (QSYS) __hip_atomic_store(&h.q[((int64_t)z * a.B + n) * A + act], p, __ATOMIC_RELAXED, __HIP_MEMORY_SCOPE_SYSTEM);
      else h.q[((int64_t)z * a.B + n) * A + act] = p;
    }
  }
  if (!h.train) return;
  __syncthreads();
  SDQN_STAMP(4);
  if (j == 0) {
    const int act = m_act, term = m_term; const int64_t rew = m_rew;
    float m;
    if constexpr (DDQN) {
      const float* qs;
      if constexpr (NZ == 3) qs = sh_q[NZ - 1]; else qs = h.q + ((int64_t)2 * a.B + n) * A;
      int best = 0; float bv = qs[0];
      for (int k = 1; k < A; ++k) { const float v = qs[k]; if (v > bv) { bv = v; best = k; } }
      m = sh_q[1][best];
    } else {
      m = sh_q[1][0];
      for (int k = 1; k < A; ++k) m = fmaxf(m, sh_q[1][k]);
    }
    double rr, gam;
    if constexpr (NSTEP) { rr = __builtin_bit_cast(double, rew); gam = h.gamma_n; }
    else {
      rr = (double)rew;
      rr = rr < h.min_reward ? h.min_reward : (rr > h.max_reward ? h.max_reward : rr);
      gam = h.discount;
    }
    const double y = term ? rr : rr + gam * (double)m;
    const float d = sh_q[0][act] - (float)y;
    float dc = d;
    if (h.clip_error != 0.0f) dc = fminf(fmaxf(d, -h.clip_error), h.clip_error);
    if constexpr (PER) {
      h.cost_terms[n] = m_w * (0.5f * (d * d));
      dc = m_w * dc;
      h.per_p[n] = (float)pow(fabs((double)d) + h.per_eps, h.per_alpha);
    } else
    h.cost_terms[n] = 0.5f * (d * d);
    h.maxq[n] = m;
    sh_dc = dc; sh_act = act;
  }
  SDQN_STAMP(5);
  __syncthreads();
  SDQN_STAMP(6);
  const float dc = sh_dc; const int act = sh_act;
  float wa = 0.0f;
#pragma unroll
  for (int k = 0; k < AMAX; ++k) wa = (k == act) ? w5[0][k] : wa;
  const float d4v = a4v[0] > 0.0f ? wa * dc : 0.0f;
  if (a.h16) a.h_d4[(int64_t)n * NFC + j] = (half_t)(d4v * a.loss_scale);
  else a.d4[(int64_t)n * NFC + j] = d4v;
  if (j < A) h.dq[(int64_t)n * A + j] = (j == act) ? dc : 0.0f;
  SDQN_STAMP(7);
}

#ifdef SDQN_TIMING
hipError_t set_timing_buffer_rb(unsigned long long* p);
hipError_t set_timing_buffer_r3(unsigned long long* p);
hipError_t set_timing_buffer_bt(unsigned long long* p);
hipError_t set_timing_buffer_ss(unsigned long long* p);
hipError_t set_timing_buffer(unsigned long long* p) {
  hipError_t e = set_timing_buffer_rb(p);
  if (e == hipSuccess) e = set_timing_buffer_r3(p);
  if (e == hipSuccess) e = set_timing_buffer_bt(p);
  if (e == hipSuccess) e = set_timing_buffer_ss(p);
  return e != hipSuccess ? e : hipMemcpyToSymbol(HIP_SYMBOL(g_sdqn_dbg), &p, sizeof p);
}
hipError_t set_wave_timing_buffer_rb(unsigned long long* const* p, const unsigned* nb, hipStream_t s);
hipError_t set_wave_timing_buffer_r3(unsigned long long* const* p, const unsigned* nb, hipStream_t s);
hipError_t set_wave_timing_buffer_bt(unsigned long long* const* p, const unsigned* nb, hipStream_t s);
hipError_t set_wave_timing_buffer(unsigned long long* const* p, const unsigned* nb, hipStream_t s) {
  hipError_t e = set_wave_timing_buffer_rb(p, nb, s);
  if (e == hipSuccess) e = set_wave_timing_buffer_r3(p, nb, s);
  if (e == hipSuccess) e = set_wave_timing_buffer_bt(p, nb, s);
  if (e == hipSuccess) e = hipMemcpyToSymbolAsync(HIP_SYMBOL(g_sdqn_wdbg_blocks), nb, sizeof *nb, 0, hipMemcpyHostToDevice, s);
  return e != hipSuccess ? e : hipMemcpyToSymbolAsync(HIP_SYMBOL(g_sdqn_wdbg), p, sizeof *p, 0, hipMemcpyHostToDevice, s);
}
#endif

typedef void (*HeadKernel)(const StepArgs, const HeadArgs);
template <bool QSYS, bool DDQN, bool PER, bool NSTEP>
static HeadKernel head_for(int bucket) {
  if constexpr (!QSYS) { if (bucket == 3) return head_kernel<MAX_ACTIONS, true, false, DDQN, PER, NSTEP>; }
  return bucket == 0 ? head_kernel<4, false, QSYS, DDQN, PER, NSTEP> : bucket == 1 ? head_kernel<8, false, QSYS, DDQN, PER, NSTEP>
                                                                                   : head_kernel<MAX_ACTIONS, false, QSYS, DDQN, PER, NSTEP>;
}

hipError_t launch_head(const StepArgs& a, const HeadArgs& h, hipStream_t s, bool q_system_scope) {
  if (a.nz > 2 && (h.train != 2 || a.bn)) return hipErrorInvalidValue;
  const int bucket = a.bn ? 3 : (a.A <= 4 ? 0 : (a.A <= 8 ? 1 : 2));
  const bool qsys = q_system_scope && !a.bn && !h.train;
  const bool ddqn = h.train == 2, per = h.per_w && h.train, nstep = h.nstep > 1 && h.train;
  static HeadKernel (*const select[9])(int) = {
    head_for<false, false, false, false>, head_for<false, true, false, false>, head_for<false, false, true, false>, head_for<false, true, true, false>,
    head_for<false, false, false, true>, head_for<false, true, false, true>, head_for<false, false, true, true>, head_for<false, true, true, true>,
    head_for<true, false, false, false>};
  const HeadKernel k = select[qsys ? 8 : (nstep ? 4 : 0) + (per ? 2 : 0) + (ddqn ? 1 : 0)](bucket);
  SDQN_LAUNCH(k, dim3(a.B), dim3(512), 0, s, a, h);
  return hipGetLastError();
}

template <bool OVF>
__global__ void __launch_bounds__(256) update_kernel(const UpdateArgs u) {
  __shared__ float4 part[8][32];
  __shared__ float cost_sh[4096];
#ifndef SDQN_NO_UPDATE_PRELOAD
  asm volatile("" :: "s"(u.theta), "s"(u.state), "s"(u.g), "s"(u.slab[0]), "s"(u.slab[1]), "s"(u.slab[2]), "s"(u.dq), "s"(u.a4), "s"(u.cost_terms),
               "s"(u.cost_out), "s"(u.cost_accum), "s"(u.w1p), "s"(u.next.meta), "s"(u.next.idx), "s"(u.next.actions), "s"(u.next.rewards),
               "s"(u.next.terminals), "s"(u.ns[0]), "s"(u.ns[1]), "s"(u.ns[2]), "s"(u.B), "s"(u.A), "s"(u.mode), "s"(u.skip_fc4), "s"(u.next.B),
               "s"(u.next.idx_in_valid), "s"(u.bsz), "s"(u.rho), "s"(u.one_minus_rho), "s"(u.lr));
#endif
  update_body<OVF>(u, (int)blockIdx.x, (int)gridDim.x, part, cost_sh);
}

hipError_t launch_update(const UpdateArgs& u, hipStream_t s) {
  int dense = 2;
  if (!u.skip_fc4) { dense = (NW4 / 4 + 255) / 256; if (dense > 1792) dense = 1792; }
  const dim3 grid(CONV_BLOCKS + u.A * FC5_BLOCKS_PER_ACTION + dense);
  if (u.ovf_flag) SDQN_LAUNCH(update_kernel<true>, grid, dim3(256), 0, s, u);
  else SDQN_LAUNCH(update_kernel<false>, grid, dim3(256), 0, s, u);
  return hipGetLastError();
}

__global__ void __launch_bounds__(256) refresh16_kernel(const float* theta, half_t* wh, half_t* wht) {
  for (int64_t e = (int64_t)blockIdx.x * 256 + threadIdx.x; e < OFF5; e += (int64_t)gridDim.x * 256) {
    const int L = e < OFF2 ? 0 : (e < OFF3 ? 1 : (e < OFF4 ? 2 : 3));
    const int off = L == 0 ? OFF1 : (L == 1 ? OFF2 : (L == 2 ? OFF3 : OFF4));
    const int K = L == 0 ? CRS1 : (L == 1 ? CRS2 : (L == 2 ? CRS3 : NIN4));
    const int N = L == 0 ? K1 : (L == 1 ? K2 : (L == 2 ? K3 : NFC));
    const int64_t r = e - off; const int k = (int)(r / N), n = (int)(r - (int64_t)k * N);
    const half_t w = (half_t)theta[e];
    wh[e] = w; wht[off + (int64_t)n * K + k] = w;
  }
}
hipError_t launch_refresh16(const float* theta, half_t* wh, half_t* wht, hipStream_t s) {
  hipLaunchKernelGGL(refresh16_kernel, dim3(2048), dim3(256), 0, s, theta, wh, wht);
  return hipGetLastError();
}

__global__ void __launch_bounds__(256) grad_to_half_kernel(const float* __restrict__ g, half_t* __restrict__ gh, int64_t n, int* state) {
  const float scale = ldexpf(1.0f, state[1]);
  if (blockIdx.x == 0 && threadIdx.x == 0) state[0] = 0;
  for (int64_t i = ((int64_t)blockIdx.x * 256 + threadIdx.x) * 4; i < n; i += (int64_t)gridDim.x * 1024) {
    if (i + 4 <= n) {
      const float4 v = *reinterpret_cast<const float4*>(g + i);
      typedef _Float16 half4 __attribute__((ext_vector_type(4)));
      half4 h; h[0] = (half_t)(v.x * scale); h[1] = (half_t)(v.y * scale); h[2] = (half_t)(v.z * scale); h[3] = (half_t)(v.w * scale);
      *reinterpret_cast<half4*>(gh + i) = h;
    } else for (int64_t k = i; k < n; ++k) gh[k] = (half_t)(g[k] * scale);
  }
}
__global__ void __launch_bounds__(256) grad_from_half_kernel(const half_t* __restrict__ gh, float* __restrict__ g, int64_t n, int* state) {
  const float inv_scale = ldexpf(1.0f, -state[1]);
  int* flag = state;
  bool bad = false;
  for (int64_t i = ((int64_t)blockIdx.x * 256 + threadIdx.x) * 4; i < n; i += (int64_t)gridDim.x * 1024) {
    const int64_t e = i + 4 <= n ? i + 4 : n;
    for (int64_t k = i; k < e; ++k) { const float v = (float)gh[k]; bad |= !(fabsf(v) <= 65504.0f); g[k] = v * inv_scale; }
  }
  if (__any(bad) && (threadIdx.x & 63) == 0) atomicOr(flag, 1);
}
hipError_t launch_grad_to_half(const float* g, half_t* gh, int64_t n, int* state, hipStream_t s) {
  hipLaunchKernelGGL(grad_to_half_kernel, dim3(512), dim3(256), 0, s, g, gh, n, state);
  return hipGetLastError();
}
hipError_t launch_grad_from_half(const half_t* gh, float* g, int64_t n, int* state, hipStream_t s) {
  hipLaunchKernelGGL(grad_from_half_kernel, dim3(512), dim3(256), 0, s, gh, g, n, state);
  return hipGetLastError();
}

__global__ void __launch_bounds__(256) prep_kernel(const PrepArgs p, double* zero8) {
  if (zero8 && threadIdx.x == 0) *zero8 = 0.0;
  const char* ka = (const char*)__builtin_amdgcn_kernarg_segment_ptr() + offsetof(PrepArgs, idx_in);
  for (int n = threadIdx.x; n < p.B; n += 256) {
    const int64_t i = p.idx_in_valid ? *reinterpret_cast<const int64_t*>(ka + 8 * (n & 31)) : p.idx_pinned[n];
    p.idx[n] = i;
    stage_meta(p.meta, i, p.ns, p.actions, p.rewards, p.terminals, n);
  }
}
hipError_t launch_prep(const PrepArgs& p, hipStream_t s, double* zero8) {
  SDQN_LAUNCH(prep_kernel, dim3(1), dim3(256), 0, s, p, zero8);
  return hipGetLastError();
}

struct IdxBlock { int64_t v[256]; };
template <bool INLINE>
__global__ void __launch_bounds__(256) gather_kernel(const GatherArgs g, const IdxBlock ib) {
  const int n = blockIdx.y;
  const int64_t index = INLINE ? ib.v[n] : g.idx[n];
  constexpr int V = FRAME / 16;
  const uint4* src = reinterpret_cast<const uint4*>(g.ring + (index - C0) * (int64_t)FRAME);
  uint4* pre = reinterpret_cast<uint4*>(g.pre + (int64_t)n * STATE);
  uint4* post = reinterpret_cast<uint4*>(g.post + (int64_t)n * STATE);
  if (g.ns.n <= 1) {
    for (int i = blockIdx.x * 256 + threadIdx.x; i < (C0 + 1) * V; i += gridDim.x * 256) {
      const uint4 v = src[i];
      if (i < C0 * V) pre[i] = v;
      if (i >= V) post[i - V] = v;
    }
  } else {
    const int64_t po = (int64_t)g.ns.n * V;
    for (int i = blockIdx.x * 256 + threadIdx.x; i < C0 * V; i += gridDim.x * 256) { pre[i] = src[i]; post[i] = src[po + i]; }
  }
// ... 18 lines not shown
```

simple_dqn_amd/csrc/sdqn_kernels_r3.hip:

```cpp
#include "gemm_engine.h"
#include "problems_h16.h"
#include "kernels.h"
#include "update_body.h"
#include "problems_wt.h"

namespace sdqn {

template <class P>
__global__ void __launch_bounds__(1024) gemm36_kernel(const StepArgs a) {
  if constexpr (has_preload<P>::value) P::preload(a, gridDim.x, gridDim.y, gridDim.z);
  static_assert(P::A_K && !P::B_K && P::B_REG, "36-deep routine: k-contiguous A (own-row loads), row-major B");
  __shared__ float smem[16 * PANEL];
  const int gx = gridDim.x, gy = gridDim.y;
  const int lin = blockIdx.x + gx * (blockIdx.y + gy * blockIdx.z);
  const int tl = (a.xcd_map & 1) ? xcd_tile_id(lin, gx * gy * gridDim.z) : lin;
  const int bz = tl / (gx * gy), rr = tl - bz * (gx * gy);
  const int bx = rr % gx, by = rr / gx;
  const int lane = threadIdx.x & 63;
  const int wave = __builtin_amdgcn_readfirstlane(threadIdx.x >> 6);
  const int m0 = bx * 32, n0 = by * 32;
  int z, ks, kbeg, kend;
  P::ksplit(a, bz, z, ks, kbeg, kend);
  const int M = P::M(a), N = P::N(a);
  const int hb = lane >> 5;
  const int mrow = m0 + (lane & 31), ncol = n0 + (lane & 31);
  const typename P::aoff_t arow = P::a_row(a, z, mrow < M ? mrow : M - 1);
  const int bcol = P::b_col(a, z, ncol < N ? ncol : N - 1);
  const float* abase = P::a_ptr(a, z);
  const float* bbase = P::b_ptr(a, z);
  const int kc = kbeg + wave * 36;
  float fa[18], fb[18];
#pragma unroll
  for (int j = 0; j < 4; ++j) {
    const f4 v = P::a_load4(a, z, arow + P::a_col(a, z, kc + 8 * j + 4 * hb));
    fa[4 * j] = v.x; fa[4 * j + 1] = v.y; fa[4 * j + 2] = v.z; fa[4 * j + 3] = v.w;
  }
  { const float2 v = *reinterpret_cast<const float2*>(abase + (arow + P::a_col(a, z, kc + 32 + 2 * hb)));
    fa[16] = v.x; fa[17] = v.y; }
  const uint32_t boff = 4u * ((uint32_t)bcol + (uint32_t)(kc + 4 * hb) * (uint32_t)P::B_LD);
#pragma unroll
  for (int t = 0; t < 16; ++t) fb[t] = ld_byte_off(bbase, boff + 4u * (uint32_t)((8 * (t >> 2) + (t & 3)) * P::B_LD));
  const uint32_t boff2 = 4u * ((uint32_t)bcol + (uint32_t)(kc + 32 + 2 * hb) * (uint32_t)P::B_LD);
  fb[16] = ld_byte_off(bbase, boff2); fb[17] = ld_byte_off(bbase, boff2 + 4u * (uint32_t)P::B_LD);
  f32x16 acc;
#pragma unroll
  for (int r = 0; r < 16; ++r) acc[r] = 0.0f;
#pragma unroll
  for (int t = 0; t < 18; ++t) acc = __builtin_amdgcn_mfma_f32_32x32x2f32(fa[t], fb[t], acc, 0, 0, 0);
  float* cw = smem + wave * PANEL;
#pragma unroll
  for (int r = 0; r < 16; ++r) cw[((r & 3) + 8 * (r >> 2) + 4 * (lane >> 5)) * 33 + (lane & 31)] = acc[r];
  __syncthreads();
  {
    const int e = threadIdx.x, ml = e >> 5, nl = e & 31;
    float v = smem[ml * 33 + nl];
#pragma unroll
    for (int w = 1; w < 16; ++w) v += smem[w * PANEL + ml * 33 + nl];
    if (m0 + ml < M && n0 + nl < N) P::store(a, z, ks, m0 + ml, n0 + nl, v);
  }
}

typedef __bf16 bf16x8_t __attribute__((ext_vector_type(8)));
constexpr int W1P_PITCH = CRS1 + 8;

struct Conv1Args {
  const uint8_t* src; float* a1; const unsigned short* w1p[2]; const int64_t* idx;
  int B, nz, from_ring, tiles_per_net, wgs_per_net, tpw, xcd, pad_;
  int post_off, reserved_;
};
struct IdxIn { int64_t v[32]; };

__device__ __forceinline__ float div255(float s) {
  const float r = 1.0f / 255.0f;
  const float q = s * r;
  return fmaf(fmaf(-q, 255.0f, s), r, q);
}

template <bool IDX_IN>
__device__ __forceinline__ void conv1_bf16_body(const Conv1Args& c, const int64_t my_idx, const int cb, unsigned short* sw) {
  const int lane = threadIdx.x & 63, i = lane & 31, h = lane >> 5;
  {
    const uint8_t* f0 = c.src; float* f1 = c.a1; const unsigned short *f2 = c.w1p[0], *f3 = c.w1p[1]; const int64_t* f4 = c.idx;
    int g0 = c.B, g1 = c.from_ring, g2 = c.tiles_per_net, g3 = c.wgs_per_net, g4 = c.tpw;
    asm volatile("" :: "s"(f0), "s"(f1), "s"(f2), "s"(f3), "s"(f4), "s"(g0), "s"(g1), "s"(g2), "s"(g3), "s"(g4));
  }
  const int zi = cb / c.wgs_per_net, wg = c.xcd ? xcd_tile_id(cb - zi * c.wgs_per_net, c.wgs_per_net) : cb - zi * c.wgs_per_net;
  const int z = zi;
  const int wave = __builtin_amdgcn_readfirstlane(threadIdx.x >> 6);
  const int M = c.B * PIX1, tiles_per_net = c.tiles_per_net, tpw = c.tpw;
  typedef uint32_t u32x2 __attribute__((ext_vector_type(2), aligned(4)));
  const int tile0 = (wg * 4 + wave) * tpw;
  SDQN_STAMP(0);
  auto load_tile = [&](int tile, u32x2* raw) {
    const int m0 = tile * 32, mrow = m0 + i, mc = mrow < M ? mrow : M - 1;
    const int n = mc / PIX1, pix = mc - n * PIX1, p = pix / Q1, q = pix - p * Q1;
    int64_t org;
    if constexpr (IDX_IN) {
      const int n_lo = m0 / PIX1, n_hi = n_lo + 1 < c.B ? n_lo + 1 : n_lo;
      const uint32_t lo0 = __builtin_amdgcn_readlane((int)(my_idx & 0xFFFFFFFF), n_lo), lo1 = __builtin_amdgcn_readlane((int)(my_idx >> 32), n_lo);
      const uint32_t hi0 = __builtin_amdgcn_readlane((int)(my_idx & 0xFFFFFFFF), n_hi), hi1 = __builtin_amdgcn_readlane((int)(my_idx >> 32), n_hi);
      const int64_t i_lo = (int64_t)(((uint64_t)lo1 << 32) | lo0), i_hi = (int64_t)(((uint64_t)hi1 << 32) | hi0);
      org = ((n == n_lo ? i_lo : i_hi) - C0 + soff(c.post_off, z)) * (int64_t)FRAME;
    } else org = c.from_ring ? (c.idx[n] - C0 + soff(c.post_off, z)) * (int64_t)FRAME : ((int64_t)sslot(z) * c.B + n) * (int64_t)STATE;
    const uint8_t* src = c.src + org + (int64_t)(p * ST1 + h) * W0 + q * ST1;
#pragma unroll
    for (int t = 0; t < 16; ++t) raw[t] = *reinterpret_cast<const u32x2*>(src + (t >> 2) * FRAME + 2 * (t & 3) * W0);
  };
  u32x2 raw[16];
#ifdef SDQN_TIMING
#pragma unroll
  for (int t = 0; t < 16; ++t) raw[t] = (u32x2){0u, 0u};
#endif
  if (tile0 < tiles_per_net) load_tile(tile0, raw);
  SDQN_STAMP(1);
  {
    const uint4* wp = reinterpret_cast<const uint4*>(c.w1p[wslot(z)]);
    static_assert(3 * K1 * (CRS1 / 8) == 12 * 256, "3072 chunks of 8 bf16: 12 per thread");
    uint4 v[12];
#pragma unroll
    for (int u = 0; u < 12; ++u) v[u] = wp[threadIdx.x + 256 * u];
#pragma unroll
    for (int u = 0; u < 12; ++u) {
      const int cc = threadIdx.x + 256 * u, row = cc >> 5, col = cc & 31;
      *reinterpret_cast<uint4*>(sw + row * W1P_PITCH + col * 8) = v[u];
    }
  }
  SDQN_STAMP(2);
  __syncthreads();
  SDQN_STAMP(3);
#ifdef SDQN_TIMING
  asm volatile("" :: "v"(raw[0].x), "v"(raw[15].y));
  SDQN_STAMP(4);
#endif
  const unsigned short* bw = sw + i * W1P_PITCH + 8 * h;
  auto cvt = [](const u32x2& r, bf16x8_t& out) {
    union { uint32_t u[4]; bf16x8_t v; } A;
#pragma unroll
    for (int d = 0; d < 2; ++d) {
      const uint32_t w = d ? r.y : r.x;
      const uint32_t f0 = __float_as_uint((float)(w & 255u)), f1 = __float_as_uint((float)((w >> 8) & 255u));
      const uint32_t f2 = __float_as_uint((float)((w >> 16) & 255u)), f3 = __float_as_uint((float)(w >> 24));
      A.u[2 * d] = __builtin_amdgcn_perm(f1, f0, 0x07060302u);
      A.u[2 * d + 1] = __builtin_amdgcn_perm(f3, f2, 0x07060302u);
    }
    out = A.v;
  };
  for (int it = 0; it < tpw; ++it) {
    const int tile = tile0 + it;
    if (tile >= tiles_per_net) break;
    const int m0 = tile * 32;
    u32x2 nxt[16];
    const bool more = it + 1 < tpw && tile + 1 < tiles_per_net;
    if (more) load_tile(tile + 1, nxt);
    f32x16 acc0, acc1, acc2;
#pragma unroll
    for (int r = 0; r < 16; ++r) { acc0[r] = 0.0f; acc1[r] = 0.0f; acc2[r] = 0.0f; }
    bf16x8_t Bc0 = *reinterpret_cast<const bf16x8_t*>(bw), Bc1 = *reinterpret_cast<const bf16x8_t*>(bw + K1 * W1P_PITCH),
             Bc2 = *reinterpret_cast<const bf16x8_t*>(bw + 2 * K1 * W1P_PITCH), Ac;
    cvt(raw[0], Ac);
#pragma unroll
    for (int t = 0; t < 16; ++t) {
      bf16x8_t Bn0 = Bc0, Bn1 = Bc1, Bn2 = Bc2, An = Ac;
      if (t + 1 < 16) {
        Bn0 = *reinterpret_cast<const bf16x8_t*>(bw + 16 * (t + 1));
        Bn1 = *reinterpret_cast<const bf16x8_t*>(bw + K1 * W1P_PITCH + 16 * (t + 1));
        Bn2 = *reinterpret_cast<const bf16x8_t*>(bw + 2 * K1 * W1P_PITCH + 16 * (t + 1));
        cvt(raw[t + 1], An);
      }
      acc0 = __builtin_amdgcn_mfma_f32_32x32x16_bf16(Ac, Bc0, acc0, 0, 0, 0);
      acc1 = __builtin_amdgcn_mfma_f32_32x32x16_bf16(Ac, Bc1, acc1, 0, 0, 0);
      acc2 = __builtin_amdgcn_mfma_f32_32x32x16_bf16(Ac, Bc2, acc2, 0, 0, 0);
      Ac = An; Bc0 = Bn0; Bc1 = Bn1; Bc2 = Bn2;
    }
#ifdef SDQN_TIMING
    asm volatile("" :: "v"(acc0[0]), "v"(acc1[7]), "v"(acc2[15]));
    SDQN_STAMP(5);
#endif
    float* out = c.a1 + ((int64_t)z * M + m0 + 4 * h) * K1 + i;
    if (m0 + 32 <= M) {
#pragma unroll
      for (int r = 0; r < 16; ++r) {
        const float v = fmaxf(div255((acc0[r] + acc1[r]) + acc2[r]), 0.0f);
        if (c.pad_) wt_store(out + ((r & 3) + 8 * (r >> 2)) * K1, v);
        else out[((r & 3) + 8 * (r >> 2)) * K1] = v;
      }
    } else {
#pragma unroll
      for (int r = 0; r < 16; ++r) {
        const int ml = (r & 3) + 8 * (r >> 2);
        if (m0 + 4 * h + ml < M) out[ml * K1] = fmaxf(div255((acc0[r] + acc1[r]) + acc2[r]), 0.0f);
      }
    }
    if (more) {
#pragma unroll
      for (int t = 0; t < 16; ++t) raw[t] = nxt[t];
    }
  }
  SDQN_STAMP(6);
}

template <bool IDX_IN>
__global__ void __launch_bounds__(256) conv1_bf16_kernel(const Conv1Args c, const IdxIn ix) {
  __shared__ __attribute__((aligned(16))) unsigned short sw[3 * K1 * W1P_PITCH];
  int64_t my_idx = 0;
  if constexpr (IDX_IN) {
    const char* ka = (const char*)__builtin_amdgcn_kernarg_segment_ptr();
    my_idx = *reinterpret_cast<const int64_t*>(ka + sizeof(Conv1Args) + 8 * (threadIdx.x & 31));
  }
  (void)ix;
  conv1_bf16_body<IDX_IN>(c, my_idx, (int)blockIdx.x, sw);
}

constexpr int C1R_ROWS = 4 * ST1 + 4;
constexpr int C1R_SEG = C1R_ROWS * W0;
constexpr int C1R_ITEM = C0 * C1R_SEG;
constexpr int C1R_CHUNKS = C1R_ITEM / 16;
constexpr int C1R_OPITCH = K1 + 4;
constexpr int C1R_OUT = 4 * Q1 * C1R_OPITCH;
static_assert(4 * Q1 * K1 * 4 == 640 * 16, "an item's output is exactly one 16-byte store per thread of the 640");
constexpr int C1R_NCH = P1 / 4;
constexpr int C1R_D = C1R_NCH;
typedef float c1p_f32x4 __attribute__((ext_vector_type(4)));
typedef uint32_t c1p_u32x4 __attribute__((ext_vector_type(4)));
typedef uint32_t c1p_u32x2 __attribute__((ext_vector_type(2)));
static_assert(P1 % 4 == 0 && (4 * Q1) % 16 == 0 && C1R_SEG % 16 == 0 && (4 * ST1 * W0) % 16 == 0, "an item is whole tiles and whole 16-byte pieces");

struct C1wArgs { const uint8_t* src; const float* d1; float* slab1; const int64_t* idx; int B, from_ring, tps1, Kt, xcd, pad_; };

template <bool IDX_IN>
__global__ void __launch_bounds__(1024) conv1_wgrad_bf16_kernel(const C1wArgs c, const IdxIn ix) {
  __shared__ float smem[16 * PANEL];
  const int lane = threadIdx.x & 63, i = lane & 31, h = lane >> 5;
  int64_t my_idx = 0;
  if constexpr (IDX_IN) {
    const char* ka = (const char*)__builtin_amdgcn_kernarg_segment_ptr();
    my_idx = *reinterpret_cast<const int64_t*>(ka + sizeof(C1wArgs) + 8 * i);
  }
  (void)ix;
  {
    const uint8_t* f0 = c.src; const float* f1 = c.d1; float* f2 = c.slab1; const int64_t* f4 = c.idx;
    int g0 = c.B, g1 = c.from_ring, g2 = c.tps1, g3 = c.Kt;
    asm volatile("" :: "s"(f0), "s"(f1), "s"(f2), "s"(f4), "s"(g0), "s"(g1), "s"(g2), "s"(g3));
  }
  const int wave = __builtin_amdgcn_readfirstlane(threadIdx.x >> 6);
  const int lin = (int)(blockIdx.x + gridDim.x * blockIdx.z);
  const int tl = c.xcd ? xcd_tile_id(lin, (int)(gridDim.x * gridDim.z)) : lin;
  const int bx = tl & 7, ks = tl >> 3;
  const int m = 32 * bx + i;
  const int colm = (m >> 6) * FRAME + ((m >> 3) & 7) * W0 + (m & 7);
  const int Kt = c.Kt, kb = ks * c.tps1 * 32;
  int ke = kb + c.tps1 * 32; if (ke > Kt) ke = Kt;
  typedef uint32_t u32x4 __attribute__((ext_vector_type(4), aligned(1)));
  auto load_chunk = [&](int kc, u32x4* ra, float* rb) {
    const int n0 = kc / PIX1, n1 = n0 + 1 < c.B ? n0 + 1 : n0;
    int64_t i0, i1;
    if constexpr (IDX_IN) {
      const uint32_t a0 = __builtin_amdgcn_readlane((int)(my_idx & 0xFFFFFFFF), n0), a1 = __builtin_amdgcn_readlane((int)(my_idx >> 32), n0);
      const uint32_t b0 = __builtin_amdgcn_readlane((int)(my_idx & 0xFFFFFFFF), n1), b1 = __builtin_amdgcn_readlane((int)(my_idx >> 32), n1);
      i0 = (int64_t)(((uint64_t)a1 << 32) | a0); i1 = (int64_t)(((uint64_t)b1 << 32) | b0);
    } else if (c.from_ring) { i0 = c.idx[n0]; i1 = c.idx[n1]; }
    else { i0 = n0; i1 = n1; }
    const int64_t unit = c.from_ring ? (int64_t)FRAME : (int64_t)STATE, off = c.from_ring ? -(int64_t)C0 * FRAME : 0;
    auto group_org = [&](int k4u) -> int64_t {
      const int k4 = k4u < Kt - 4 ? k4u : Kt - 4;
      const int n = k4 / PIX1, pix = k4 - n * PIX1, y = pix / Q1, x = pix - y * Q1;
      return (n == n0 ? i0 : i1) * unit + off + (int64_t)(y * ST1) * W0 + x * ST1;
    };
#pragma unroll
    for (int st = 0; st < 2; ++st)
#pragma unroll
      for (int g = 0; g < 2; ++g) {
        const int64_t o0 = group_org(kc + 16 * st + 4 * g), o1 = group_org(kc + 16 * st + 8 + 4 * g);
        ra[2 * st + g] = *reinterpret_cast<const u32x4*>(c.src + (h ? o1 : o0) + colm);
      }
#pragma unroll
    for (int st = 0; st < 2; ++st)
#pragma unroll
      for (int e = 0; e < 8; ++e) {
        const int k = kc + 16 * st + 8 * h + e, kcl = k < Kt ? k : Kt - 1;
        const float v = c.d1[(uint32_t)(kcl * K1 + i)];
        rb[8 * st + e] = k < ke ? v : 0.0f;
      }
  };
  f32x16 acc;
#pragma unroll
  for (int r = 0; r < 16; ++r) acc[r] = 0.0f;
  int kc = kb + wave * 32;
  u32x4 ra[4]; float rb[16];
  if (kc < ke) load_chunk(kc, ra, rb);
  while (kc < ke) {
    u32x4 na[4]; float nb[16];
    const int kn = kc + 16 * 32;
    if (kn < ke) load_chunk(kn, na, nb);
#pragma unroll
    for (int st = 0; st < 2; ++st) {
      union { uint32_t u[4]; bf16x8_t v; } A;
#pragma unroll
      for (int g = 0; g < 2; ++g) {
        const u32x4 w = ra[2 * st + g];
        const uint32_t f0 = __float_as_uint((float)(w.x & 255u)), f1 = __float_as_uint((float)(w.y & 255u));
        const uint32_t f2 = __float_as_uint((float)(w.z & 255u)), f3 = __float_as_uint((float)(w.w & 255u));
        A.u[2 * g] = __builtin_amdgcn_perm(f1, f0, 0x07060302u);
        A.u[2 * g + 1] = __builtin_amdgcn_perm(f3, f2, 0x07060302u);
      }
      bf16x8_t B0, B1, B2;
#pragma unroll
      for (int e = 0; e < 8; ++e) {
        const float x = rb[8 * st + e];
        const __bf16 hi = (__bf16)x; const float r1 = x - (float)hi;
        const __bf16 mid = (__bf16)r1; const float r2 = r1 - (float)mid;
        B0[e] = hi; B1[e] = mid; B2[e] = (__bf16)r2;
      }
      acc = __builtin_amdgcn_mfma_f32_32x32x16_bf16(A.v, B0, acc, 0, 0, 0);
      acc = __builtin_amdgcn_mfma_f32_32x32x16_bf16(A.v, B1, acc, 0, 0, 0);
      acc = __builtin_amdgcn_mfma_f32_32x32x16_bf16(A.v, B2, acc, 0, 0, 0);
    }
    kc = kn;
    if (kc < ke) {
#pragma unroll
      for (int t = 0; t < 4; ++t) ra[t] = na[t];
#pragma unroll
      for (int t = 0; t < 16; ++t) rb[t] = nb[t];
    }
  }
  float* cw = smem + wave * PANEL;
#pragma unroll
  for (int r = 0; r < 16; ++r) cw[((r & 3) + 8 * (r >> 2) + 4 * h) * 33 + i] = acc[r];
  __syncthreads();
  {
// ... 145 lines not shown
        }
        c1p_u32x4* d = reinterpret_cast<c1p_u32x4*>(dst + pdst[j]);
        d[0] = o[0]; d[1] = o[1];
      }
    };
    auto flush = [&](int item) {
      const int si = item / C1R_NCH, ch = item - si * C1R_NCH;
      float* outs = c.a1 + (((int64_t)z * c.B + g + (int64_t)si * Gz) * PIX1 + ch * (4 * Q1)) * K1;
      const __amdgpu_buffer_rsrc_t rs = __builtin_amdgcn_make_buffer_rsrc((void*)outs, 0, 4 * Q1 * K1 * 4, 0x00020000);
#pragma unroll
      for (int u = 0; u < C1S_FPT; ++u) {
        const int pc = lid + C1S_LOADERS * u;
        if (pc >= 640) continue;
        const c1p_f32x4 v = *reinterpret_cast<const c1p_f32x4*>(outl + (item & 1) * C1R_OUT + (pc >> 3) * C1R_OPITCH + 4 * (pc & 7));
        c1p_u32x4 w;
#pragma unroll
        for (int e = 0; e < 4; ++e) w[e] = __float_as_uint(v[e]);
        if (c.pad_) __builtin_amdgcn_raw_buffer_store_b128(w, rs, 16 * pc, 0, 16); else __builtin_amdgcn_raw_buffer_store_b128(w, rs, 16 * pc, 0, 0);
      }
    };
    c1p_u32x4 fv[C1R_D][C1S_LPT];
#pragma unroll
    for (int u = 0; u < C1R_D; ++u) gload(u, fv[u]);
    lstore(fv[0], img);
    gload(C1R_D, fv[0]);
    __syncthreads();
    for (int i0 = 0; i0 < nitems; i0 += C1R_D) {
#pragma unroll
      for (int u = 0; u < C1R_D; ++u) {
        const int item = i0 + u;
        if (item > 0) flush(item - 1);
        lstore(fv[(u + 1) % C1R_D], img + ((item + 1) & 1) * C1R_ITEM);
        gload(item + 1 + C1R_D, fv[(u + 1) % C1R_D]);
        __syncthreads();
      }
    }
    if (nitems > 0) flush(nitems - 1);
    return;
  }
  const int tj = wave >> 1, nh = wave & 1;
  __syncthreads();
  bf16x8_t Bf[3][8];
  {
    const unsigned short* bw = sw + (nh * 16 + m) * W1P_PITCH + 8 * kg;
#pragma unroll
    for (int p = 0; p < 3; ++p)
#pragma unroll
      for (int t = 0; t < 8; ++t) Bf[p][t] = *reinterpret_cast<const bf16x8_t*>(bw + p * K1 * W1P_PITCH + 32 * t);
  }
  const int pos = 16 * tj + m, pl = pos / Q1, q = pos - pl * Q1;
  const int a_off = (ST1 * pl + kg) * W0 + ST1 * q;
  for (int item = 0; item < nitems; ++item) {
    const unsigned short* cur = img + (item & 1) * C1R_ITEM + a_off;
    bf16x8_t A[8];
#pragma unroll
    for (int t = 0; t < 8; ++t) {
      const unsigned short* ap = cur + (t >> 1) * C1R_SEG + 4 * (t & 1) * W0;
      union { c1p_u32x2 u[2]; bf16x8_t v; } X;
      X.u[0] = *reinterpret_cast<const c1p_u32x2*>(ap); X.u[1] = *reinterpret_cast<const c1p_u32x2*>(ap + 4);
      A[t] = X.v;
    }
    c1p_f32x4 acc[3];
#pragma unroll
    for (int p = 0; p < 3; ++p) acc[p] = c1p_f32x4{0.f, 0.f, 0.f, 0.f};
#pragma unroll
    for (int t = 0; t < 8; ++t)
#pragma unroll
      for (int p = 0; p < 3; ++p) acc[p] = __builtin_amdgcn_mfma_f32_16x16x32_bf16(Bf[p][t], A[t], acc[p], 0, 0, 0);
    c1p_f32x4 v;
#pragma unroll
    for (int e = 0; e < 4; ++e) v[e] = fmaxf(div255((acc[0][e] + acc[1][e]) + acc[2][e]), 0.0f);
    *reinterpret_cast<c1p_f32x4*>(outl + (item & 1) * C1R_OUT + pos * C1R_OPITCH + nh * 16 + 4 * kg) = v;
    __syncthreads();
  }
}

hipError_t launch_kernel_r3(int id, const StepArgs& a, const LaunchTune& t, hipStream_t s, bool* handled) {
  *handled = true;
  if (id == K_CONV1_FWD && (t.variant & LV_CONV1_FWD_BF16) && !a.h16 && !a.bn && a.w1p[0] && a.w1p[a.nz > 1 ? 1 : 0]) {
    const int tiles = (a.B * PIX1 + 31) / 32, tpw = a.B >= 128 ? 4 : 1, wgs = (tiles + 4 * tpw - 1) / (4 * tpw);
    Conv1Args c; c.src = a.src; c.a1 = a.a1; c.w1p[0] = a.w1p[0]; c.w1p[1] = a.w1p[1]; c.idx = a.idx;
    c.B = a.B; c.nz = a.nz; c.from_ring = a.from_ring; c.tiles_per_net = tiles; c.wgs_per_net = wgs; c.tpw = tpw; c.xcd = t.r3_xcd & 1; c.pad_ = (t.wt & WT_CONV1_FWD) ? 1 : 0;
    c.post_off = a.post_off; c.reserved_ = 0;
    static_assert(sizeof(Conv1Args) == 80 && offsetof(Conv1Args, post_off) == 72, "the index block follows 8-byte aligned at byte 80");
    if (a.B >= 128 && t.bt[K_CONV1_FWD] >= 0) {
      const int cap = 256 / a.nz, per = (a.B + cap - 1) / cap;
      c.wgs_per_net = (a.B + per - 1) / per;
      SDQN_LAUNCH(conv1_bf16_rows2_kernel<4>, dim3(a.nz * c.wgs_per_net), dim3(896), 0, s, c);
      return hipGetLastError();
    }
    IdxIn ix;
    if (t.host_idx && a.from_ring && a.B <= 32) {
      memset(ix.v, 0, sizeof ix.v);
      memcpy(ix.v, t.host_idx, (size_t)a.B * sizeof(int64_t));
      SDQN_LAUNCH(conv1_bf16_kernel<true>, dim3(a.nz * wgs), dim3(256), 0, s, c, ix);
    } else {
      memset(ix.v, 0, sizeof ix.v);
      SDQN_LAUNCH(conv1_bf16_kernel<false>, dim3(a.nz * wgs), dim3(256), 0, s, c, ix);
    }
    return hipGetLastError();
  }
  if ((id == K_BWD1 || id == K_CONV1_WGRAD) && (t.variant & LV_CONV1_WGRAD_BF16) && (id == K_CONV1_WGRAD || a.f4w_count == 0) && !a.h16 && !a.bn) {
    C1wArgs c; c.src = a.src; c.d1 = a.d1; c.slab1 = a.slab1; c.idx = a.idx; c.B = a.B; c.from_ring = a.from_ring; c.tps1 = a.tps1; c.Kt = a.B * PIX1; c.xcd = (t.r3_xcd >> 1) & 1; c.pad_ = (t.wt & WT_CONV1_WGRAD) ? 1 : 0;
    static_assert(sizeof(C1wArgs) == 56, "the index block follows at byte 56 of the argument segment");
    const dim3 grid(CRS1 / 32, 1, Conv1Wgrad::nbz(a));
    IdxIn ix; memset(ix.v, 0, sizeof ix.v);
    if (t.host_idx && a.from_ring && a.B <= 32) {
      memcpy(ix.v, t.host_idx, (size_t)a.B * sizeof(int64_t));
      SDQN_LAUNCH(conv1_wgrad_bf16_kernel<true>, grid, dim3(1024), 0, s, c, ix);
    } else SDQN_LAUNCH(conv1_wgrad_bf16_kernel<false>, grid, dim3(1024), 0, s, c, ix);
    return hipGetLastError();
  }
  if (a.B <= 32 && a.h16 == 2 && !a.bn && t.wt && !(id >= 0 && id < 12 && t.nw_override[id] > 0)) {
    if (id == K_CONV1_FWD && (t.wt & WT_CONV1_FWD)) return launch_gemm<Conv1FwdHWT, 8>(a, s);
    if (id == K_CONV2_FWD && (t.wt & WT_CONV2_FWD)) return launch_gemm<Conv2FwdHWT, 16>(a, s);
    if (id == K_CONV3_FWD && (t.wt & WT_CONV3_FWD)) return launch_gemm<Conv3FwdHWT, 16>(a, s);
    if (id == K_FC4_FWD && (t.wt & WT_FC4_FWD)) return launch_gemm<Fc4FwdHWT, 14>(a, s);
    if (id == K_FC4_DGRAD && (t.wt & WT_FC4_DGRAD)) return launch_gemm<Fc4DgradHWT, 16>(a, s);
    if (id == K_BWD2 && (t.wt & WT_BWD2)) return launch_multi<512, NoProblem, 2, Conv2DgradHWT, 8, Conv2WgradHWWT, 8>(a, true, true, s);
    if (id == K_BWD1 && (t.wt & WT_CONV1_WGRAD)) return launch_multi<1024, NoProblem, 2, Conv1WgradHWWT, 16, NoProblem, 2>(a, true, false, s);
  }
  if (a.B <= 32 && !a.h16 && !a.bn && t.wt && !(id >= 0 && id < 12 && t.nw_override[id] > 0)) {
    if (id == K_CONV2_FWD && (t.wt & WT_CONV2_FWD)) return launch_gemm<Conv2FwdWT, 16>(a, s);
    if (id == K_FC4_FWD && (t.wt & WT_FC4_FWD)) return launch_gemm<Staged<Fc4FwdWT>, 14>(a, s);
    if (id == K_FC4_DGRAD && (t.wt & WT_FC4_DGRAD)) return launch_gemm<Staged<Fc4DgradWT>, 16>(a, s);
    if (id == K_BWD3 && (t.wt & WT_BWD3) && a.f4w_count > 0) return launch_multi<512, Staged<Conv3DgradWT>, 8, Conv3WgradWT, 8, Fc4WgradWT, 1>(a, true, true, s);
    if (id == K_BWD2 && (t.wt & WT_BWD2) && a.f4w_count == 0) return launch_multi<512, NoProblem, 2, Conv2DgradWT, 8, Conv2WgradWT, 8>(a, true, true, s);
  }
  if (a.B >= 128 && !a.h16 && !a.bn && t.wt && !(id >= 0 && id < 12 && t.nw_override[id] > 0)) {
    if (id == K_CONV2_FWD && (t.wt & WT_CONV2_FWD)) return launch_gemm<Staged<Conv2FwdWT>, 8>(a, s);
    if (id == K_CONV3_FWD && (t.wt & WT_CONV3_FWD)) return launch_gemm<Staged<Conv3FwdWT>, 8>(a, s);
    if (id == K_FC4_FWD && (t.wt & WT_FC4_FWD)) return launch_gemm<Staged<Fc4FwdWT>, 8>(a, s);
    if (id == K_FC4_DGRAD && (t.wt & WT_FC4_DGRAD)) return launch_gemm<Staged<Fc4DgradWT>, 4>(a, s);
    if (id == K_BWD3 && (t.wt & WT_BWD3) && a.f4w_count > 0) return launch_multi<512, Fc4WgradWT, 8, Staged<Conv3DgradWT>, 8, Conv3WgradWT, 8>(a, true, true, s);
    if (id == K_BWD2 && (t.wt & WT_BWD2) && a.f4w_count == 0) return launch_multi<512, NoProblem, 2, Staged<Conv2DgradWT>, 8, Conv2WgradWT, 8>(a, true, true, s);
    if (id == K_BWD1 && (t.wt & WT_CONV1_WGRAD) && a.f4w_count == 0 && !(t.variant & LV_CONV1_WGRAD_BF16)) return launch_multi<1024, NoProblem, 2, Conv1WgradWT, 16, NoProblem, 2>(a, true, false, s);
  }
  if (id == K_CONV3_FWD && (t.variant & LV_CONV3_C36) && a.B < 128 && !a.h16 && !a.bn) {
    static_assert(CRS3 == 16 * 36, "conv3's K is 16 chunks of 36");
    const dim3 grid((Conv3Fwd::M(a) + 31) / 32, (Conv3Fwd::N(a) + 31) / 32, Conv3Fwd::nbz(a));
    if ((t.wt & WT_CONV3_FWD) && a.B <= 32) SDQN_LAUNCH((gemm36_kernel<Conv3FwdWT>), grid, dim3(1024), 0, s, a);
    else SDQN_LAUNCH((gemm36_kernel<Conv3Fwd>), grid, dim3(1024), 0, s, a);
    return hipGetLastError();
  }
  *handled = false;
  return hipSuccess;
}

#ifdef SDQN_TIMING
hipError_t set_timing_buffer_r3(unsigned long long* p) { return hipMemcpyToSymbol(HIP_SYMBOL(g_sdqn_dbg), &p, sizeof p); }
hipError_t set_wave_timing_buffer_r3(unsigned long long* const* p, const unsigned* nb, hipStream_t s) {
  hipError_t e = hipMemcpyToSymbolAsync(HIP_SYMBOL(g_sdqn_wdbg_blocks), nb, sizeof *nb, 0, hipMemcpyHostToDevice, s);
  return e != hipSuccess ? e : hipMemcpyToSymbolAsync(HIP_SYMBOL(g_sdqn_wdbg), p, sizeof *p, 0, hipMemcpyHostToDevice, s);
}
#endif

}
```

simple_dqn_amd/csrc/update_body.h:

```cpp
#pragma once
#include <cstddef>
#include "kernels.h"

namespace sdqn {

__device__ inline void opt_apply4(float* __restrict__ theta, float* __restrict__ st1, float* __restrict__ st2,
                                  int64_t e, const float4& gs, const UpdateArgs& u, const float4* pre = nullptr) {
  float4 w = pre ? pre[0] : *reinterpret_cast<float4*>(theta + e);
  float4 a = pre ? pre[1] : *reinterpret_cast<float4*>(st1 + e);
  float4 b = make_float4(0.f, 0.f, 0.f, 0.f);
  if (u.opt != 0) b = *reinterpret_cast<float4*>(st2 + e);
  w.x = opt_apply(w.x, a.x, b.x, gs.x, u); w.y = opt_apply(w.y, a.y, b.y, gs.y, u);
  w.z = opt_apply(w.z, a.z, b.z, gs.z, u); w.w = opt_apply(w.w, a.w, b.w, gs.w, u);
  if (u.wt) {
    typedef unsigned int u4_t __attribute__((ext_vector_type(4)));
    u4_t v; v.x = __float_as_uint(w.x); v.y = __float_as_uint(w.y); v.z = __float_as_uint(w.z); v.w = __float_as_uint(w.w);
    constexpr int FLAT_BYTES = (OFF5 + MAX_ACTIONS * NFC) * 4;
    __builtin_amdgcn_raw_buffer_store_b128(v, __builtin_amdgcn_make_buffer_rsrc((void*)theta, 0, FLAT_BYTES, 0x00020000), (int)(e * 4), 0, 16);
    v.x = __float_as_uint(a.x); v.y = __float_as_uint(a.y); v.z = __float_as_uint(a.z); v.w = __float_as_uint(a.w);
    __builtin_amdgcn_raw_buffer_store_b128(v, __builtin_amdgcn_make_buffer_rsrc((void*)st1, 0, FLAT_BYTES, 0x00020000), (int)(e * 4), 0, 16);
  } else { *reinterpret_cast<float4*>(theta + e) = w; *reinterpret_cast<float4*>(st1 + e) = a; }
  if (u.opt != 0) *reinterpret_cast<float4*>(st2 + e) = b;
  if (u.w1p && e < OFF2) {
    const int k = (int)(e >> 5), n = (int)(e & 31);
    const float wv[4] = {w.x, w.y, w.z, w.w};
#pragma unroll
    for (int i = 0; i < 4; ++i) {
      uint16_t hi, mid, lo; split_bf16x3(wv[i], hi, mid, lo);
      u.w1p[(n + i) * CRS1 + k] = hi; u.w1p[W1P_PLANE + (n + i) * CRS1 + k] = mid; u.w1p[2 * W1P_PLANE + (n + i) * CRS1 + k] = lo;
    }
  }
  if (u.wh && e < OFF5) {
    const int L = e < OFF2 ? 0 : (e < OFF3 ? 1 : (e < OFF4 ? 2 : 3));
    const int off = L == 0 ? OFF1 : (L == 1 ? OFF2 : (L == 2 ? OFF3 : OFF4));
    const int K = L == 0 ? CRS1 : (L == 1 ? CRS2 : (L == 2 ? CRS3 : NIN4));
    const int N = L == 0 ? K1 : (L == 1 ? K2 : (L == 2 ? K3 : NFC));
    const int64_t r = e - off; const int k = (int)(r / N), n = (int)(r - (int64_t)k * N);
    const float wv[4] = {w.x, w.y, w.z, w.w};
#pragma unroll
    for (int i = 0; i < 4; ++i) { u.wh[e + i] = (half_t)wv[i]; u.wht[off + (int64_t)(n + i) * K + k] = (half_t)wv[i]; }
  }
}

constexpr int CONV_F4 = OFF4 / 4;
constexpr int CONV_BLOCKS = CONV_F4 / 32;
constexpr int FC5_BLOCKS_PER_ACTION = NFC / 4 / 32;

template <bool OVF>
__device__ __forceinline__ void update_body(const UpdateArgs& u, const int bid, const int nblocks, float4 (*part)[32], float* cost_sh) {
  const int t = threadIdx.x;
#ifdef SDQN_TIMING
  SDQN_STAMP(0);
  struct StampAtExit { __device__ ~StampAtExit() { SDQN_STAMP(7); } } stamp_at_exit_;
#endif
  bool skip_apply = false;
  if constexpr (OVF) {
    skip_apply = u.ovf_flag[0] != 0;
    if (bid == 0 && t == 0) {
      int* st = const_cast<int*>(u.ovf_flag);
      if (skip_apply) { u.ovf_count[0] += 1; st[2] = 0; if (u.ovf_dynamic && st[1] > 0) st[1] -= 1; }
      else if (u.ovf_dynamic && ++st[2] >= 200) { st[2] = 0; if (st[1] < 15) st[1] += 1; }
    }
  }
  if (u.only_fc4 && bid < CONV_BLOCKS + u.A * FC5_BLOCKS_PER_ACTION) return;
  if (bid < CONV_BLOCKS) {
    const int c4 = t & 31, sg = t >> 5;
    const int64_t e = ((int64_t)bid * 32 + c4) * 4;
    float4 gs = make_float4(0.f, 0.f, 0.f, 0.f);
    float4 pre[2] = {gs, gs};
    const bool applies = sg == 0 && u.mode != 1 && !skip_apply;
    if (applies) { pre[0] = *reinterpret_cast<const float4*>(u.theta + e); pre[1] = *reinterpret_cast<const float4*>(u.state + e); }
    if (u.mode == 2) {
      if (sg == 0) gs = *reinterpret_cast<const float4*>(u.g + e);
    } else {
      const int L = e < OFF2 ? 0 : (e < OFF3 ? 1 : 2);
      const int64_t off = e - (L == 0 ? OFF1 : (L == 1 ? OFF2 : OFF3));
      const int64_t nw = L == 0 ? NW1 : (L == 1 ? NW2 : NW3);
      const float* sp = u.slab[L] + off;
      const int ns = u.ns[L];
      if (ns > 32) {
        for (int s = sg; s < ns; s += 128) {
          float4 v[16];
#pragma unroll
          for (int j = 0; j < 16; ++j) { const int sj = s + 8 * j; v[j] = *reinterpret_cast<const float4*>(sp + (int64_t)(sj < ns ? sj : ns - 1) * nw); }
#pragma unroll
          for (int j = 0; j < 16; ++j)
            if (s + 8 * j < ns) { gs.x += v[j].x; gs.y += v[j].y; gs.z += v[j].z; gs.w += v[j].w; }
        }
      } else
      for (int s = sg; s < ns; s += 32) {
        float4 v[4];
#pragma unroll
        for (int j = 0; j < 4; ++j) { const int sj = s + 8 * j; v[j] = *reinterpret_cast<const float4*>(sp + (int64_t)(sj < ns ? sj : ns - 1) * nw); }
#pragma unroll
        for (int j = 0; j < 4; ++j)
          if (s + 8 * j < ns) { gs.x += v[j].x; gs.y += v[j].y; gs.z += v[j].z; gs.w += v[j].w; }
      }
      part[sg][c4] = gs;
      __syncthreads();
      if (sg == 0) {
#pragma unroll
        for (int k = 1; k < 8; ++k) { const float4 v = part[k][c4]; gs.x += v.x; gs.y += v.y; gs.z += v.z; gs.w += v.w; }
        *reinterpret_cast<float4*>(u.g + e) = gs;
      }
    }
    if (applies) opt_apply4(u.theta, u.state, u.state2, e, gs, u, pre);
    return;
  }
  const int fc5_blocks = u.A * FC5_BLOCKS_PER_ACTION;
  if (bid < CONV_BLOCKS + fc5_blocks) {
    const int fb = bid - CONV_BLOCKS, c4 = t & 31, sg = t >> 5;
    const int act = fb / FC5_BLOCKS_PER_ACTION, j0 = ((fb - act * FC5_BLOCKS_PER_ACTION) * 32 + c4) * 4;
    const int64_t e = OFF5 + (int64_t)act * NFC + j0;
    float4 gs = make_float4(0.f, 0.f, 0.f, 0.f);
    if (u.mode == 2) {
      if (sg == 0) gs = *reinterpret_cast<const float4*>(u.g + e);
    } else {
      int n = sg;
      for (; n + 24 < u.B; n += 32) {
        const float d0 = u.dq[(int64_t)n * u.A + act], d1 = u.dq[(int64_t)(n + 8) * u.A + act];
        const float d2 = u.dq[(int64_t)(n + 16) * u.A + act], d3 = u.dq[(int64_t)(n + 24) * u.A + act];
        const float4 v0 = *reinterpret_cast<const float4*>(u.a4 + (int64_t)n * NFC + j0);
        const float4 v1 = *reinterpret_cast<const float4*>(u.a4 + (int64_t)(n + 8) * NFC + j0);
        const float4 v2 = *reinterpret_cast<const float4*>(u.a4 + (int64_t)(n + 16) * NFC + j0);
        const float4 v3 = *reinterpret_cast<const float4*>(u.a4 + (int64_t)(n + 24) * NFC + j0);
        gs.x += d0 * v0.x; gs.y += d0 * v0.y; gs.z += d0 * v0.z; gs.w += d0 * v0.w;
        gs.x += d1 * v1.x; gs.y += d1 * v1.y; gs.z += d1 * v1.z; gs.w += d1 * v1.w;
        gs.x += d2 * v2.x; gs.y += d2 * v2.y; gs.z += d2 * v2.z; gs.w += d2 * v2.w;
        gs.x += d3 * v3.x; gs.y += d3 * v3.y; gs.z += d3 * v3.z; gs.w += d3 * v3.w;
      }
      for (; n < u.B; n += 8) {
        const float d = u.dq[(int64_t)n * u.A + act];
        const float4 v = *reinterpret_cast<const float4*>(u.a4 + (int64_t)n * NFC + j0);
        gs.x += d * v.x; gs.y += d * v.y; gs.z += d * v.z; gs.w += d * v.w;
      }
      part[sg][c4] = gs;
      __syncthreads();
      if (sg == 0) {
#pragma unroll
        for (int k = 1; k < 8; ++k) { const float4 v = part[k][c4]; gs.x += v.x; gs.y += v.y; gs.z += v.z; gs.w += v.w; }
        *reinterpret_cast<float4*>(u.g + e) = gs;
      }
    }
    if (sg == 0 && u.mode != 1 && !skip_apply) opt_apply4(u.theta, u.state, u.state2, e, gs, u);
    return;
  }
  const int first_dense = CONV_BLOCKS + fc5_blocks;
  const int nb = nblocks - first_dense;
  if (!u.skip_fc4) {
    for (int64_t i4 = CONV_F4 + (int64_t)(bid - first_dense) * 256 + t; i4 < OFF5 / 4; i4 += (int64_t)nb * 256) {
      const int64_t e = i4 * 4;
      const float4 gs = *reinterpret_cast<const float4*>(u.g + e);
      if (u.mode != 1 && !skip_apply) opt_apply4(u.theta, u.state, u.state2, e, gs, u);
    }
  }
  if (u.next.B > 0 && bid == first_dense) {
    const char* ka = (const char*)__builtin_amdgcn_kernarg_segment_ptr() + offsetof(UpdateArgs, next) + offsetof(PrepArgs, idx_in);
    for (int n = t; n < u.next.B; n += 256) {
      const int64_t i = u.next.idx_in_valid ? *reinterpret_cast<const int64_t*>(ka + 8 * (n & 31)) : u.next.idx_pinned[n];
      u.next.idx[n] = i;
      stage_meta(u.next.meta, i, u.next.ns, u.next.actions, u.next.rewards, u.next.terminals, n);
    }
  }
  if (u.mode != 2 && bid == first_dense + (nb > 1 ? 1 : 0)) {
    for (int n = t; n < u.B; n += 256) cost_sh[n] = u.cost_terms[n];
    __syncthreads();
    if (t == 0) {
      float c = 0.0f;
      for (int n = 0; n < u.B; ++n) c += cost_sh[n];
      c = c / (float)u.B;
      u.cost_out[0] = c;
      u.cost_accum[0] += (double)c;
    }
  }
}


}
```

Baseline: 15340 train_steps/sec.

## Pass hot kernel arguments in a leading 64-byte block for SGPR preload

Adds a 16-dword leading argument block holding the most-used pointers, batch size, grid dims and packed control bits, and passes it first to the GEMM, multi-GEMM, head, conv1, conv1-wgrad and conv3 kernels. When enabled, kernels read these scalars from the leading block instead of the large StepArgs struct. The aim is to let hardware kernarg preload place them in SGPRs and cut scalar-load latency at kernel start in this launch-bound small-batch step. The change adds packing and unpacking logic plus fit checks, and shifts the offsets used to read inline index blocks from the kernarg segment, which risks misreads if any offset is wrong.

New measurement: 15940 train_steps/sec (median of 6 runs). 3.9% higher.

```diff
diff --git a/simple_dqn_amd/csrc/api_internal.h b/simple_dqn_amd/csrc/api_internal.h
--- a/simple_dqn_amd/csrc/api_internal.h
+++ b/simple_dqn_amd/csrc/api_internal.h
@@ -150,6 +150,7 @@
   int wt = WT_ALL;
   int conv1w_bf16 = 1;
   bool conv3_c36 = true;
+  bool arg_preload = true;
   bool fused_launches = true;
   bool prof_on = false; int prof_filter = -1;
   int prof_mode = 1;
diff --git a/simple_dqn_amd/csrc/gemm_engine.h b/simple_dqn_amd/csrc/gemm_engine.h
--- a/simple_dqn_amd/csrc/gemm_engine.h
+++ b/simple_dqn_amd/csrc/gemm_engine.h
@@ -23,6 +23,30 @@
 template <class P> struct has_preload<P, decltype((void)P::PRELOAD)> { static constexpr bool value = P::PRELOAD; };
 template <class P, class = void> struct has_preload_multi { static constexpr bool value = false; };
 template <class P> struct has_preload_multi<P, decltype((void)P::PRELOAD_MULTI)> { static constexpr bool value = P::PRELOAD_MULTI; };
+struct Lead { const void* p[5]; int B, s0, s1, ctl, r0, r1; };
+static_assert(sizeof(Lead) == 64, "leading block: 16 dwords");
+constexpr int LEAD_ON = 256;
+#define SDQN_LEAD_PARAMS const void* lp0, const void* lp1, const void* lp2, const void* lp3, const void* lp4, int lB, int ls0, int ls1, int lctl, int lr0, int lr1
+#define SDQN_LEAD_ARGS(L) (L).p[0], (L).p[1], (L).p[2], (L).p[3], (L).p[4], (L).B, (L).s0, (L).s1, (L).ctl, (L).r0, (L).r1
+template <class T> struct lead_noref { typedef T type; };
+template <class T> struct lead_noref<T&> { typedef T type; };
+#define SDQN_LEAD_SET_(f, v) a.f = (typename lead_noref<decltype(a.f)>::type)(v)
+#define SDQN_LEAD_FIELDS(f0, f1, f2, f3, f4, X) \
+  static void lead_pack(const StepArgs& a, Lead& l) { l.p[0] = a.f0; l.p[1] = a.f1; l.p[2] = a.f2; l.p[3] = a.f3; l.p[4] = a.f4; l.s1 = a.X; } \
+  __device__ static void lead_apply(StepArgs& a, const void* q0, const void* q1, const void* q2, const void* q3, const void* q4, int x) { \
+    SDQN_LEAD_SET_(f0, q0); SDQN_LEAD_SET_(f1, q1); SDQN_LEAD_SET_(f2, q2); SDQN_LEAD_SET_(f3, q3); SDQN_LEAD_SET_(f4, q4); a.X = x; }
+template <class P, class = void> struct has_lead { static constexpr bool value = false; };
+template <class P> struct has_lead<P, decltype((void)P::LEAD)> { static constexpr bool value = P::LEAD; };
+template <class P, class = void> struct has_lead_multi { static constexpr bool value = false; };
+template <class P> struct has_lead_multi<P, decltype((void)P::LEAD_MULTI)> { static constexpr bool value = P::LEAD_MULTI; };
+inline int lead_grid(const dim3& g) { return (int)(g.x | g.y << 16 | g.z << 24); }
+inline bool lead_grid_fits(const dim3& g) { return g.x < 65536u && g.y < 256u && g.z < 128u; }
+inline int lead_ctl(const StepArgs& a, bool on) {
+  const bool fits = a.B < 128 && a.xcd_map >= 0 && a.xcd_map < 256 && a.nz >= 0 && a.nz < 16 && a.S4 >= 0 && a.S4 < 256;
+  return (a.xcd_map & 255) | (on && fits ? LEAD_ON : 0) | ((a.nz & 15) << 12) | ((a.S4 & 255) << 16);
+}
+__device__ __forceinline__ void lead_scalars(StepArgs& a, int B, int ctl) { a.B = B; a.xcd_map = ctl & 255; a.nz = (ctl >> 12) & 15; a.S4 = (ctl >> 16) & 255; }
+#define SDQN_LEAD_FWD lp0, lp1, lp2, lp3, lp4, lB, ls0, ls1, lctl, lr0, lr1
 template <class P, class = void> struct uses_f16_mfma { static constexpr bool value = false; };
 template <class P> struct uses_f16_mfma<P, decltype((void)P::F16_MFMA)> { static constexpr bool value = P::F16_MFMA; };
 
@@ -485,15 +509,32 @@
 template <class P> constexpr int tile_n() { return 32; }
 
 
+template <class P>
+__device__ __forceinline__ void lead_take(StepArgs& a, int& gx, int& gy, int& gz, const StepArgs& a_, SDQN_LEAD_PARAMS) {
+  (void)lr0; (void)lr1;
+  if (lctl & LEAD_ON) { lead_scalars(a, lB, lctl); P::lead_apply(a, lp0, lp1, lp2, lp3, lp4, ls1); gx = ls0 & 0xFFFF; gy = (ls0 >> 16) & 255; gz = ls0 >> 24; }
+  else { if constexpr (has_preload<P>::value) P::preload(a_, gridDim.x, gridDim.y, gridDim.z); gx = gridDim.x; gy = gridDim.y; gz = gridDim.z; }
+}
 template <class P, int NW>
-__global__ void __launch_bounds__(NW * 64) gemm_kernel(const StepArgs a) {
-  __shared__ float smem[tile_lds_any<P, NW>()];
-  if constexpr (has_preload<P>::value) P::preload(a, gridDim.x, gridDim.y, gridDim.z);
-  const int gx = gridDim.x, gy = gridDim.y;
+__device__ __forceinline__ void gemm_kernel_body(const StepArgs& a, int gx, int gy, int gz, float* smem) {
   const int lin = blockIdx.x + gx * (blockIdx.y + gy * blockIdx.z);
-  const int t = (a.xcd_map & 1) ? xcd_tile_id(lin, gx * gy * gridDim.z) : lin;
+  const int t = (a.xcd_map & 1) ? xcd_tile_id(lin, gx * gy * gz) : lin;
   const int bz = t / (gx * gy), r = t - bz * (gx * gy);
   run_tile<P, NW, NW * 64>(a, r % gx, r / gx, bz, smem);
+}
+template <class P, int NW>
+__global__ void __launch_bounds__(NW * 64) gemm_kernel(SDQN_LEAD_PARAMS, const StepArgs a_) {
+  __shared__ float smem[tile_lds_any<P, NW>()];
+  (void)lr0; (void)lr1;
+  if constexpr (has_lead<P>::value) {
+    StepArgs a = a_;
+    int gx, gy, gz;
+    lead_take<P>(a, gx, gy, gz, a_, SDQN_LEAD_FWD);
+    gemm_kernel_body<P, NW>(a, gx, gy, gz, smem);
+  } else {
+    if constexpr (has_preload<P>::value) P::preload(a_, gridDim.x, gridDim.y, gridDim.z);
+    gemm_kernel_body<P, NW>(a_, gridDim.x, gridDim.y, gridDim.z, smem);
+  }
 }
 
 struct MultiDims { int n[3]; int gx[3], gy[3]; };
@@ -517,17 +558,34 @@
 }
 
 template <int NT, class P0, int NW0, class P1, int NW1, class P2, int NW2>
-__global__ void __launch_bounds__(NT) gemm_multi_kernel(const StepArgs a, const MultiDims d) {
-  constexpr int L0 = tile_lds_any<P0, NW0>() * (NW0 == 1 ? NT / 64 : 1), L1 = tile_lds_any<P1, NW1>() * (NW1 == 1 ? NT / 64 : 1),
-                L2 = tile_lds_any<P2, NW2>() * (NW2 == 1 ? NT / 64 : 1);
-  constexpr int L = L0 > L1 ? (L0 > L2 ? L0 : L2) : (L1 > L2 ? L1 : L2);
-  __shared__ float smem[L];
-  if constexpr (has_preload_multi<P1>::value) P1::preload_multi(a, d);
+__device__ __forceinline__ void gemm_multi_body(const StepArgs& a, const MultiDims& d, float* smem) {
   const int b = blockIdx.x;
   const int xm = a.xcd_map;
   if (b < d.n[0]) multi_dispatch<P0, NW0, NT>(a, d, 0, (xm & 1) ? xcd_tile_id_range(b, 0, d.n[0]) : b, smem);
   else if (b < d.n[0] + d.n[1]) multi_dispatch<P1, NW1, NT>(a, d, 1, (xm & 2) ? xcd_tile_id_range(b, d.n[0], d.n[1]) : b - d.n[0], smem);
   else multi_dispatch<P2, NW2, NT>(a, d, 2, (xm & 4) ? xcd_tile_id_range(b, d.n[0] + d.n[1], d.n[2]) : b - d.n[0] - d.n[1], smem);
+}
+template <int NT, class P0, int NW0, class P1, int NW1, class P2, int NW2>
+__global__ void __launch_bounds__(NT) gemm_multi_kernel(SDQN_LEAD_PARAMS, const StepArgs a_, const MultiDims d_) {
+  constexpr int L0 = tile_lds_any<P0, NW0>() * (NW0 == 1 ? NT / 64 : 1), L1 = tile_lds_any<P1, NW1>() * (NW1 == 1 ? NT / 64 : 1),
+                L2 = tile_lds_any<P2, NW2>() * (NW2 == 1 ? NT / 64 : 1);
+  constexpr int L = L0 > L1 ? (L0 > L2 ? L0 : L2) : (L1 > L2 ? L1 : L2);
+  __shared__ float smem[L];
+  (void)lr0; (void)lr1;
+  if constexpr (has_lead_multi<P1>::value) {
+    StepArgs a = a_; MultiDims d = d_;
+    if (lctl & LEAD_ON) {
+      lead_scalars(a, lB, lctl); P1::lead_apply(a, lp0, lp1, lp2, lp3, lp4, ls1);
+      d.n[0] = ls0 & 0xFFFF; d.n[1] = (int)((unsigned)ls0 >> 16);
+      d.gx[0] = (P0::M(a) + tile_m<P0>() - 1) / tile_m<P0>(); d.gy[0] = (P0::N(a) + tile_n<P0>() - 1) / tile_n<P0>();
+      d.gx[1] = (P1::M(a) + tile_m<P1>() - 1) / tile_m<P1>(); d.gy[1] = (P1::N(a) + tile_n<P1>() - 1) / tile_n<P1>();
+      d.gx[2] = (P2::M(a) + tile_m<P2>() - 1) / tile_m<P2>(); d.gy[2] = (P2::N(a) + tile_n<P2>() - 1) / tile_n<P2>();
+    } else { if constexpr (has_preload_multi<P1>::value) P1::preload_multi(a_, d_); }
+    gemm_multi_body<NT, P0, NW0, P1, NW1, P2, NW2>(a, d, smem);
+  } else {
+    if constexpr (has_preload_multi<P1>::value) P1::preload_multi(a_, d_);
+    gemm_multi_body<NT, P0, NW0, P1, NW1, P2, NW2>(a_, d_, smem);
+  }
 }
 
 struct NoProblem {
@@ -555,7 +613,12 @@
 template <class P, int NW>
 inline hipError_t launch_gemm(const StepArgs& a, hipStream_t stream) {
   dim3 grid((P::M(a) + tile_m<P>() - 1) / tile_m<P>(), (P::N(a) + tile_n<P>() - 1) / tile_n<P>(), P::nbz(a));
-  SDQN_LAUNCH((gemm_kernel<P, NW>), grid, dim3(NW * 64), 0, stream, a);
+  Lead l; memset(&l, 0, sizeof l);
+  if constexpr (has_lead<P>::value) {
+    P::lead_pack(a, l); l.B = a.B; l.s0 = lead_grid(grid);
+    l.ctl = lead_ctl(a, a.arg_preload && lead_grid_fits(grid));
+  }
+  SDQN_LAUNCH((gemm_kernel<P, NW>), grid, dim3(NW * 64), 0, stream, SDQN_LEAD_ARGS(l), a);
   return hipGetLastError();
 }
 
@@ -573,7 +636,12 @@
   if (has1) multi_fill<NT, P1, NW1>(a, d, 1);
   if (has2) multi_fill<NT, P2, NW2>(a, d, 2);
   if (d.n[0] + d.n[1] + d.n[2] == 0) return hipSuccess;
-  SDQN_LAUNCH((gemm_multi_kernel<NT, P0, NW0, P1, NW1, P2, NW2>), dim3(d.n[0] + d.n[1] + d.n[2]), dim3(NT), 0, stream, a, d);
+  Lead l; memset(&l, 0, sizeof l);
+  if constexpr (has_lead_multi<P1>::value) {
+    P1::lead_pack(a, l); l.B = a.B; l.s0 = (int)((unsigned)d.n[0] | (unsigned)d.n[1] << 16);
+    l.ctl = lead_ctl(a, a.arg_preload && has1 && has2 && d.n[0] < 65536 && d.n[1] < 65536);
+  }
+  SDQN_LAUNCH((gemm_multi_kernel<NT, P0, NW0, P1, NW1, P2, NW2>), dim3(d.n[0] + d.n[1] + d.n[2]), dim3(NT), 0, stream, SDQN_LEAD_ARGS(l), a, d);
   return hipGetLastError();
 }
 
diff --git a/simple_dqn_amd/csrc/kernels.h b/simple_dqn_amd/csrc/kernels.h
--- a/simple_dqn_amd/csrc/kernels.h
+++ b/simple_dqn_amd/csrc/kernels.h
@@ -77,7 +77,8 @@
   half_t* wh;
   half_t* wht;
   unsigned short* w1p;
-  int reserved_[4];
+  int arg_preload;
+  int reserved_[3];
   int wt;
   int reserved2_[3];
   int64_t bn_first;
diff --git a/simple_dqn_amd/csrc/problems.h b/simple_dqn_amd/csrc/problems.h
--- a/simple_dqn_amd/csrc/problems.h
+++ b/simple_dqn_amd/csrc/problems.h
@@ -99,7 +99,8 @@
   int h16;
   int xcd_map;
   int post_off;
-  int reserved_[11];
+  int arg_preload;
+  int reserved_[10];
   float* __restrict__ theta_w;
   float* __restrict__ state;
   float bsz, rho, one_minus_rho, lr, eps;
diff --git a/simple_dqn_amd/csrc/problems_wt.h b/simple_dqn_amd/csrc/problems_wt.h
--- a/simple_dqn_amd/csrc/problems_wt.h
+++ b/simple_dqn_amd/csrc/problems_wt.h
@@ -25,12 +25,18 @@
 #endif
 struct Conv2FwdWT : Conv2Fwd {
   static constexpr bool PRELOAD = SDQN_PRELOAD != 0;
+  static constexpr bool LEAD = true;
+  SDQN_LEAD_FIELDS(a1, theta[0], theta[1], a2, a3, A)
+  __device__ static const float* b_ptr(const StepArgs& a, int z) { return (wslot(z) ? a.theta[1] : a.theta[0]) + OFF2; }
   __device__ static void preload(const StepArgs& a, unsigned g0, unsigned g1, unsigned g2) { SDQN_TOUCH("s"(a.a1), "s"(a.a2), "s"(a.theta[0]), "s"(a.theta[1]), "s"(a.B), "s"(a.nz), "s"(a.xcd_map), "s"(g0), "s"(g1), "s"(g2)); }
 
   __device__ static void store(const StepArgs& a, int z, int, int m, int n, float v) { wt_store(&a.a2[((int64_t)z * M(a) + m) * K2 + n], fmaxf(v, 0.0f)); }
 };
 struct Conv3FwdWT : Conv3Fwd {
   static constexpr bool PRELOAD = SDQN_PRELOAD != 0;
+  static constexpr bool LEAD = true;
+  SDQN_LEAD_FIELDS(a2, theta[0], theta[1], a3, a1, A)
+  __device__ static const float* b_ptr(const StepArgs& a, int z) { return (wslot(z) ? a.theta[1] : a.theta[0]) + OFF3; }
   __device__ static void preload(const StepArgs& a, unsigned g0, unsigned g1, unsigned g2) { SDQN_TOUCH("s"(a.a2), "s"(a.a3), "s"(a.theta[0]), "s"(a.theta[1]), "s"(a.B), "s"(a.nz), "s"(a.xcd_map), "s"(g0), "s"(g1), "s"(g2)); }
 
   __device__ static void store(const StepArgs& a, int z, int, int m, int n, float v) { wt_store(&a.a3[((int64_t)z * M(a) + m) * K3 + n], fmaxf(v, 0.0f)); }
@@ -41,6 +47,9 @@
 }
 struct Fc4FwdWT : Fc4Fwd {
   static constexpr bool PRELOAD = SDQN_PRELOAD != 0;
+  static constexpr bool LEAD = true;
+  SDQN_LEAD_FIELDS(a3, theta[0], theta[1], slab4, a4, A)
+  __device__ static const float* b_ptr(const StepArgs& a, int z) { return (wslot(z) ? a.theta[1] : a.theta[0]) + OFF4; }
   __device__ static void preload(const StepArgs& a, unsigned g0, unsigned g1, unsigned g2) { SDQN_TOUCH("s"(a.a3), "s"(a.slab4), "s"(a.theta[0]), "s"(a.theta[1]), "s"(a.B), "s"(a.nz), "s"(a.S4), "s"(a.xcd_map), "s"(g0), "s"(g1), "s"(g2)); }
 
   __device__ static f4 b_load4(const StepArgs& a, int z, int o) { return NT_W4 ? ld4_nt(a.theta[wslot(z)] + OFF4 + o) : ld4(a.theta[wslot(z)] + OFF4 + o); }
@@ -48,6 +57,8 @@
 };
 struct Fc4DgradWT : Fc4Dgrad {
   static constexpr bool PRELOAD = SDQN_PRELOAD != 0;
+  static constexpr bool LEAD = true;
+  SDQN_LEAD_FIELDS(d4, theta[0], a3, d3p, d3, A)
   __device__ static void preload(const StepArgs& a, unsigned g0, unsigned g1, unsigned g2) { SDQN_TOUCH("s"(a.d4), "s"(a.theta[0]), "s"(a.a3), "s"(a.d3p), "s"(a.d3), "s"(a.B), "s"(a.xcd_map), "s"(g0), "s"(g1), "s"(g2)); }
 
   __device__ static f4 b_load4(const StepArgs& a, int, int o) { return NT_W4 ? ld4_nt(a.theta[0] + OFF4 + o) : ld4(a.theta[0] + OFF4 + o); }
@@ -77,6 +88,8 @@
 };
 struct Conv3WgradWT : Conv3Wgrad {
   static constexpr bool PRELOAD = SDQN_PRELOAD != 0;
+  static constexpr bool LEAD_MULTI = true;
+  SDQN_LEAD_FIELDS(d3p, theta[0], a2, d3, a3, tps3)
   SDQN_PRELOAD_MULTI_DEF
   __device__ static void preload(const StepArgs& a, unsigned g0, unsigned g1, unsigned g2) { SDQN_TOUCH("s"(a.a2), "s"(a.d3), "s"(a.slab3), "s"(a.tps3), "s"(a.B), "s"(g0), "s"(g1), "s"(g2)); }
 
@@ -84,6 +97,8 @@
 };
 struct Conv2DgradWT : Conv2Dgrad {
   static constexpr bool PRELOAD = SDQN_PRELOAD != 0;
+  static constexpr bool LEAD_MULTI = true;
+  SDQN_LEAD_FIELDS(d2p, theta[0], a1, d2, d1, tps2)
   SDQN_PRELOAD_MULTI_DEF
   __device__ static void preload(const StepArgs& a, unsigned g0, unsigned g1, unsigned g2) { SDQN_TOUCH("s"(a.d2p), "s"(a.theta[0]), "s"(a.a1), "s"(a.d1), "s"(a.B), "s"(g0), "s"(g1), "s"(g2)); }
 
diff --git a/simple_dqn_amd/csrc/sdqn_api_net.hip b/simple_dqn_amd/csrc/sdqn_api_net.hip
--- a/simple_dqn_amd/csrc/sdqn_api_net.hip
+++ b/simple_dqn_amd/csrc/sdqn_api_net.hip
@@ -463,6 +463,7 @@
     HIPCHK(hipMemcpy(h->ovf_flag, st0, 16, hipMemcpyHostToDevice));
   }
   else if (!strcmp(name, "fused_launches")) h->fused_launches = value != 0;
+  else if (!strcmp(name, "arg_preload")) h->arg_preload = value != 0;
   else if (!strcmp(name, "conv1_bf16")) h->conv1_bf16 = value != 0;
   else if (!strcmp(name, "wt")) h->wt = value;
   else if (!strcmp(name, "prep_inline")) h->prep_inline = value != 0;
diff --git a/simple_dqn_amd/csrc/sdqn_api_step.hip b/simple_dqn_amd/csrc/sdqn_api_step.hip
--- a/simple_dqn_amd/csrc/sdqn_api_step.hip
+++ b/simple_dqn_amd/csrc/sdqn_api_step.hip
@@ -13,6 +13,7 @@
   a.S4 = h->S4; a.tps1 = h->tps1; a.tps2 = h->tps2; a.tps3 = h->tps3;
 
   a.xcd_map = h->xcd_map ? 7 : 0;
+  a.arg_preload = h->arg_preload ? 1 : 0;
   if (h->cfg.datatype == 1) {
     a.h16 = h->h16_wgrad_mfma ? 2 : 1; a.h_a1 = h->h_a1; a.h_a2 = h->h_a2; a.h_a3 = h->h_a3; a.h_d4 = h->h_d4; a.h_d3p = h->h_d3p; a.h_d3 = h->h_d3;
     a.h_d2p = h->h_d2p; a.h_d2 = h->h_d2; a.h_d1 = h->h_d1; a.wh[0] = h->wh[0]; a.wh[1] = h->wh[1]; a.wht[0] = h->wht[0]; a.wht[1] = h->wht[1];
@@ -103,6 +104,7 @@
 }
 UpdateArgs make_update_args(sdqn_net_s* h, const StepArgs& a) {
   UpdateArgs u; memset(&u, 0, sizeof u);
+  u.arg_preload = a.arg_preload;
   u.theta = h->theta; u.state = h->state; u.g = h->g;
   u.slab[0] = h->slab1; u.slab[1] = h->slab2; u.slab[2] = h->slab3; u.ns[0] = h->ns1; u.ns[1] = h->ns2; u.ns[2] = h->ns3;
   u.dq = h->dq; u.a4 = h->a4; u.cost_terms = h->cost_terms; u.cost_out = h->cost_out; u.cost_accum = h->cost_accum;
diff --git a/simple_dqn_amd/csrc/sdqn_kernels.hip b/simple_dqn_amd/csrc/sdqn_kernels.hip
--- a/simple_dqn_amd/csrc/sdqn_kernels.hip
+++ b/simple_dqn_amd/csrc/sdqn_kernels.hip
@@ -121,7 +121,13 @@
 }
 
 template <int AMAX, bool BN, bool QSYS, bool DDQN, bool PER, bool NSTEP>
-__global__ void __launch_bounds__(512) head_kernel(const StepArgs a, const HeadArgs h) {
+__global__ void __launch_bounds__(512) head_kernel(SDQN_LEAD_PARAMS, const StepArgs a_, const HeadArgs h) {
+  StepArgs a = a_;
+  (void)ls1; (void)lr0; (void)lr1;
+  if (lctl & LEAD_ON) {
+    lead_scalars(a, lB, lctl); a.A = ls0;
+    a.theta[0] = (const float*)lp0; a.theta[1] = (const float*)lp1; a.slab4 = (float*)lp2; a.a4 = (float*)lp3; a.d4 = (float*)lp4;
+  }
   SDQN_STAMP(0);
   const int n = blockIdx.x, j = threadIdx.x, lane = j & 63, wave = j >> 6;
   constexpr int NZ = (DDQN && !BN) ? 3 : 2;
@@ -131,7 +137,7 @@
   __shared__ int sh_act;
   const int nz = a.nz, A = a.A;
   const float* __restrict__ th0 = a.theta[0];
-  const float* __restrict__ th1 = a.theta[nz > 1 ? 1 : 0];
+  const float* __restrict__ th1 = nz > 1 ? a.theta[1] : a.theta[0];
   const float* __restrict__ slab = a.slab4;
   float a4v[NZ];
 #pragma unroll
@@ -285,7 +291,7 @@
 }
 #endif
 
-typedef void (*HeadKernel)(const StepArgs, const HeadArgs);
+typedef void (*HeadKernel)(SDQN_LEAD_PARAMS, const StepArgs, const HeadArgs);
 template <bool QSYS, bool DDQN, bool PER, bool NSTEP>
 static HeadKernel head_for(int bucket) {
   if constexpr (!QSYS) { if (bucket == 3) return head_kernel<MAX_ACTIONS, true, false, DDQN, PER, NSTEP>; }
@@ -303,29 +309,45 @@
     head_for<false, false, false, true>, head_for<false, true, false, true>, head_for<false, false, true, true>, head_for<false, true, true, true>,
     head_for<true, false, false, false>};
   const HeadKernel k = select[qsys ? 8 : (nstep ? 4 : 0) + (per ? 2 : 0) + (ddqn ? 1 : 0)](bucket);
-  SDQN_LAUNCH(k, dim3(a.B), dim3(512), 0, s, a, h);
+  Lead l; memset(&l, 0, sizeof l);
+  l.p[0] = a.theta[0]; l.p[1] = a.theta[1]; l.p[2] = a.slab4; l.p[3] = a.a4; l.p[4] = a.d4; l.B = a.B; l.s0 = a.A; l.ctl = lead_ctl(a, a.arg_preload != 0);
+  SDQN_LAUNCH(k, dim3(a.B), dim3(512), 0, s, SDQN_LEAD_ARGS(l), a, h);
   return hipGetLastError();
 }
 
 template <bool OVF>
-__global__ void __launch_bounds__(256) update_kernel(const UpdateArgs u) {
+__global__ void __launch_bounds__(256) update_kernel(SDQN_LEAD_PARAMS, const UpdateArgs u) {
   __shared__ float4 part[8][32];
   __shared__ float cost_sh[4096];
+  (void)lr0; (void)lr1;
+  UpdHot hot;
+  const int L = upd_layer((int)blockIdx.x);
+  if ((lctl & LEAD_ON) && (int)blockIdx.x < CONV_BLOCKS) {
+    hot = UpdHot{(float*)lp0, (float*)lp1, (const float*)(L == 0 ? lp2 : (L == 1 ? lp3 : lp4)), L == 0 ? (lB & 0xFFFF) : (L == 1 ? (int)((unsigned)lB >> 16) : ls0),
+                 (ls1 >> 8) & 15, (ls1 >> 12) & 1, ls1 & 255};
+  } else {
 #ifndef SDQN_NO_UPDATE_PRELOAD
   asm volatile("" :: "s"(u.theta), "s"(u.state), "s"(u.g), "s"(u.slab[0]), "s"(u.slab[1]), "s"(u.slab[2]), "s"(u.dq), "s"(u.a4), "s"(u.cost_terms),
                "s"(u.cost_out), "s"(u.cost_accum), "s"(u.w1p), "s"(u.next.meta), "s"(u.next.idx), "s"(u.next.actions), "s"(u.next.rewards),
                "s"(u.next.terminals), "s"(u.ns[0]), "s"(u.ns[1]), "s"(u.ns[2]), "s"(u.B), "s"(u.A), "s"(u.mode), "s"(u.skip_fc4), "s"(u.next.B),
                "s"(u.next.idx_in_valid), "s"(u.bsz), "s"(u.rho), "s"(u.one_minus_rho), "s"(u.lr));
 #endif
-  update_body<OVF>(u, (int)blockIdx.x, (int)gridDim.x, part, cost_sh);
+    hot = UpdHot{u.theta, u.state, u.slab[L], u.ns[L], u.mode, u.only_fc4, u.A};
+  }
+  update_body<OVF>(u, hot, (int)sizeof(Lead), (int)blockIdx.x, (int)gridDim.x, part, cost_sh);
 }
 
 hipError_t launch_update(const UpdateArgs& u, hipStream_t s) {
   int dense = 2;
   if (!u.skip_fc4) { dense = (NW4 / 4 + 255) / 256; if (dense > 1792) dense = 1792; }
   const dim3 grid(CONV_BLOCKS + u.A * FC5_BLOCKS_PER_ACTION + dense);
-  if (u.ovf_flag) SDQN_LAUNCH(update_kernel<true>, grid, dim3(256), 0, s, u);
-  else SDQN_LAUNCH(update_kernel<false>, grid, dim3(256), 0, s, u);
+  Lead l; memset(&l, 0, sizeof l);
+  l.p[0] = u.theta; l.p[1] = u.state; l.p[2] = u.slab[0]; l.p[3] = u.slab[1]; l.p[4] = u.slab[2];
+  l.B = (int)((unsigned)u.ns[0] | (unsigned)u.ns[1] << 16); l.s0 = u.ns[2]; l.s1 = u.A | u.mode << 8 | (u.only_fc4 ? 1 << 12 : 0);
+  const bool fits = u.ns[0] >= 0 && u.ns[0] < 65536 && u.ns[1] >= 0 && u.ns[1] < 65536 && u.A >= 0 && u.A < 256 && u.mode >= 0 && u.mode < 16 && u.ns[2] >= 0;
+  l.ctl = u.arg_preload && u.B < 128 && fits ? LEAD_ON : 0;
+  if (u.ovf_flag) SDQN_LAUNCH(update_kernel<true>, grid, dim3(256), 0, s, SDQN_LEAD_ARGS(l), u);
+  else SDQN_LAUNCH(update_kernel<false>, grid, dim3(256), 0, s, SDQN_LEAD_ARGS(l), u);
   return hipGetLastError();
 }
 
diff --git a/simple_dqn_amd/csrc/sdqn_kernels_r3.hip b/simple_dqn_amd/csrc/sdqn_kernels_r3.hip
--- a/simple_dqn_amd/csrc/sdqn_kernels_r3.hip
+++ b/simple_dqn_amd/csrc/sdqn_kernels_r3.hip
@@ -7,13 +7,10 @@
 namespace sdqn {
 
 template <class P>
-__global__ void __launch_bounds__(1024) gemm36_kernel(const StepArgs a) {
-  if constexpr (has_preload<P>::value) P::preload(a, gridDim.x, gridDim.y, gridDim.z);
+__device__ __forceinline__ void gemm36_body(const StepArgs& a, const int gx, const int gy, const int gz, float* smem) {
   static_assert(P::A_K && !P::B_K && P::B_REG, "36-deep routine: k-contiguous A (own-row loads), row-major B");
-  __shared__ float smem[16 * PANEL];
-  const int gx = gridDim.x, gy = gridDim.y;
   const int lin = blockIdx.x + gx * (blockIdx.y + gy * blockIdx.z);
-  const int tl = (a.xcd_map & 1) ? xcd_tile_id(lin, gx * gy * gridDim.z) : lin;
+  const int tl = (a.xcd_map & 1) ? xcd_tile_id(lin, gx * gy * gz) : lin;
   const int bz = tl / (gx * gy), rr = tl - bz * (gx * gy);
   const int bx = rr % gx, by = rr / gx;
   const int lane = threadIdx.x & 63;
@@ -57,6 +54,20 @@
 #pragma unroll
     for (int w = 1; w < 16; ++w) v += smem[w * PANEL + ml * 33 + nl];
     if (m0 + ml < M && n0 + nl < N) P::store(a, z, ks, m0 + ml, n0 + nl, v);
+  }
+}
+template <class P>
+__global__ void __launch_bounds__(1024) gemm36_kernel(SDQN_LEAD_PARAMS, const StepArgs a_) {
+  __shared__ float smem[16 * PANEL];
+  (void)lr0; (void)lr1;
+  if constexpr (has_lead<P>::value) {
+    StepArgs a = a_;
+    int gx, gy, gz;
+    lead_take<P>(a, gx, gy, gz, a_, SDQN_LEAD_FWD);
+    gemm36_body<P>(a, gx, gy, gz, smem);
+  } else {
+    if constexpr (has_preload<P>::value) P::preload(a_, gridDim.x, gridDim.y, gridDim.z);
+    gemm36_body<P>(a_, gridDim.x, gridDim.y, gridDim.z, smem);
   }
 }
 
@@ -114,15 +125,16 @@
   if (tile0 < tiles_per_net) load_tile(tile0, raw);
   SDQN_STAMP(1);
   {
-    const uint4* wp = reinterpret_cast<const uint4*>(c.w1p[wslot(z)]);
+    typedef uint32_t pl4 __attribute__((ext_vector_type(4)));
+    const pl4* wp = reinterpret_cast<const pl4*>(wslot(z) ? c.w1p[1] : c.w1p[0]);
     static_assert(3 * K1 * (CRS1 / 8) == 12 * 256, "3072 chunks of 8 bf16: 12 per thread");
-    uint4 v[12];
+    pl4 v[12];
 #pragma unroll
     for (int u = 0; u < 12; ++u) v[u] = wp[threadIdx.x + 256 * u];
 #pragma unroll
     for (int u = 0; u < 12; ++u) {
       const int cc = threadIdx.x + 256 * u, row = cc >> 5, col = cc & 31;
-      *reinterpret_cast<uint4*>(sw + row * W1P_PITCH + col * 8) = v[u];
+      *reinterpret_cast<pl4*>(sw + row * W1P_PITCH + col * 8) = v[u];
     }
   }
   SDQN_STAMP(2);
@@ -200,14 +212,20 @@
 }
 
 template <bool IDX_IN>
-__global__ void __launch_bounds__(256) conv1_bf16_kernel(const Conv1Args c, const IdxIn ix) {
+__global__ void __launch_bounds__(256) conv1_bf16_kernel(SDQN_LEAD_PARAMS, const Conv1Args c_, const IdxIn ix) {
   __shared__ __attribute__((aligned(16))) unsigned short sw[3 * K1 * W1P_PITCH];
   int64_t my_idx = 0;
   if constexpr (IDX_IN) {
     const char* ka = (const char*)__builtin_amdgcn_kernarg_segment_ptr();
-    my_idx = *reinterpret_cast<const int64_t*>(ka + sizeof(Conv1Args) + 8 * (threadIdx.x & 31));
-  }
-  (void)ix;
+    my_idx = *reinterpret_cast<const int64_t*>(ka + sizeof(Lead) + sizeof(Conv1Args) + 8 * (threadIdx.x & 31));
+  }
+  (void)ix; (void)lr0; (void)lr1;
+  Conv1Args c = c_;
+  if (lctl & LEAD_ON) {
+    c.src = (const uint8_t*)lp0; c.a1 = (float*)lp1; c.w1p[0] = (const unsigned short*)lp2; c.w1p[1] = (const unsigned short*)lp3; c.idx = (const int64_t*)lp4;
+    c.B = lB; c.tiles_per_net = ls0; c.wgs_per_net = ls1; c.xcd = lctl & 1; c.pad_ = (lctl >> 1) & 1; c.from_ring = (lctl >> 2) & 1;
+    c.tpw = (lctl >> 4) & 15; c.post_off = (int)((unsigned)lctl >> 16);
+  }
   conv1_bf16_body<IDX_IN>(c, my_idx, (int)blockIdx.x, sw);
 }
 
@@ -228,23 +246,31 @@
 struct C1wArgs { const uint8_t* src; const float* d1; float* slab1; const int64_t* idx; int B, from_ring, tps1, Kt, xcd, pad_; };
 
 template <bool IDX_IN>
-__global__ void __launch_bounds__(1024) conv1_wgrad_bf16_kernel(const C1wArgs c, const IdxIn ix) {
+__global__ void __launch_bounds__(1024) conv1_wgrad_bf16_kernel(SDQN_LEAD_PARAMS, const C1wArgs c_, const IdxIn ix) {
   __shared__ float smem[16 * PANEL];
   const int lane = threadIdx.x & 63, i = lane & 31, h = lane >> 5;
   int64_t my_idx = 0;
   if constexpr (IDX_IN) {
     const char* ka = (const char*)__builtin_amdgcn_kernarg_segment_ptr();
-    my_idx = *reinterpret_cast<const int64_t*>(ka + sizeof(C1wArgs) + 8 * i);
-  }
-  (void)ix;
+    my_idx = *reinterpret_cast<const int64_t*>(ka + sizeof(Lead) + sizeof(C1wArgs) + 8 * i);
+  }
+  (void)ix; (void)lp4; (void)lr0; (void)lr1;
+  C1wArgs c = c_;
+  int gxw = CRS1 / 32, gzw;
+  if (!(lctl & LEAD_ON)) { gxw = (int)gridDim.x; gzw = (int)gridDim.z; }
+  else {
+    gzw = (int)((unsigned)lctl >> 16);
+    c.src = (const uint8_t*)lp0; c.d1 = (const float*)lp1; c.slab1 = (float*)lp2; c.idx = (const int64_t*)lp3;
+    c.B = lB; c.tps1 = ls0; c.Kt = ls1; c.xcd = lctl & 1; c.pad_ = (lctl >> 1) & 1; c.from_ring = (lctl >> 2) & 1;
+  }
   {
     const uint8_t* f0 = c.src; const float* f1 = c.d1; float* f2 = c.slab1; const int64_t* f4 = c.idx;
     int g0 = c.B, g1 = c.from_ring, g2 = c.tps1, g3 = c.Kt;
     asm volatile("" :: "s"(f0), "s"(f1), "s"(f2), "s"(f4), "s"(g0), "s"(g1), "s"(g2), "s"(g3));
   }
   const int wave = __builtin_amdgcn_readfirstlane(threadIdx.x >> 6);
-  const int lin = (int)(blockIdx.x + gridDim.x * blockIdx.z);
-  const int tl = c.xcd ? xcd_tile_id(lin, (int)(gridDim.x * gridDim.z)) : lin;
+  const int lin = (int)blockIdx.x + gxw * (int)blockIdx.z;
+  const int tl = c.xcd ? xcd_tile_id(lin, gxw * gzw) : lin;
   const int bx = tl & 7, ks = tl >> 3;
   const int m = 32 * bx + i;
   const int colm = (m >> 6) * FRAME + ((m >> 3) & 7) * W0 + (m & 7);
@@ -556,7 +582,10 @@
     Conv1Args c; c.src = a.src; c.a1 = a.a1; c.w1p[0] = a.w1p[0]; c.w1p[1] = a.w1p[1]; c.idx = a.idx;
     c.B = a.B; c.nz = a.nz; c.from_ring = a.from_ring; c.tiles_per_net = tiles; c.wgs_per_net = wgs; c.tpw = tpw; c.xcd = t.r3_xcd & 1; c.pad_ = (t.wt & WT_CONV1_FWD) ? 1 : 0;
     c.post_off = a.post_off; c.reserved_ = 0;
-    static_assert(sizeof(Conv1Args) == 80 && offsetof(Conv1Args, post_off) == 72, "the index block follows 8-byte aligned at byte 80");
+    static_assert(sizeof(Conv1Args) == 80 && offsetof(Conv1Args, post_off) == 72, "the index block follows 8-byte aligned at byte 64 + 80");
+    Lead l; memset(&l, 0, sizeof l);
+    l.p[0] = c.src; l.p[1] = c.a1; l.p[2] = c.w1p[0]; l.p[3] = c.w1p[1]; l.p[4] = c.idx; l.B = c.B; l.s0 = tiles; l.s1 = wgs;
+    l.ctl = c.xcd | c.pad_ << 1 | (c.from_ring ? 4 : 0) | (tpw & 15) << 4 | (a.arg_preload && a.B < 128 && tpw >= 0 && tpw < 16 && c.xcd < 2 && c.pad_ < 2 && c.post_off >= 0 && c.post_off < 32768 ? LEAD_ON : 0) | (int)((unsigned)c.post_off << 16);
     if (a.B >= 128 && t.bt[K_CONV1_FWD] >= 0) {
       const int cap = 256 / a.nz, per = (a.B + cap - 1) / cap;
       c.wgs_per_net = (a.B + per - 1) / per;
@@ -567,22 +596,25 @@
     if (t.host_idx && a.from_ring && a.B <= 32) {
       memset(ix.v, 0, sizeof ix.v);
       memcpy(ix.v, t.host_idx, (size_t)a.B * sizeof(int64_t));
-      SDQN_LAUNCH(conv1_bf16_kernel<true>, dim3(a.nz * wgs), dim3(256), 0, s, c, ix);
+      SDQN_LAUNCH(conv1_bf16_kernel<true>, dim3(a.nz * wgs), dim3(256), 0, s, SDQN_LEAD_ARGS(l), c, ix);
     } else {
       memset(ix.v, 0, sizeof ix.v);
-      SDQN_LAUNCH(conv1_bf16_kernel<false>, dim3(a.nz * wgs), dim3(256), 0, s, c, ix);
+      SDQN_LAUNCH(conv1_bf16_kernel<false>, dim3(a.nz * wgs), dim3(256), 0, s, SDQN_LEAD_ARGS(l), c, ix);
     }
     return hipGetLastError();
   }
   if ((id == K_BWD1 || id == K_CONV1_WGRAD) && (t.variant & LV_CONV1_WGRAD_BF16) && (id == K_CONV1_WGRAD || a.f4w_count == 0) && !a.h16 && !a.bn) {
     C1wArgs c; c.src = a.src; c.d1 = a.d1; c.slab1 = a.slab1; c.idx = a.idx; c.B = a.B; c.from_ring = a.from_ring; c.tps1 = a.tps1; c.Kt = a.B * PIX1; c.xcd = (t.r3_xcd >> 1) & 1; c.pad_ = (t.wt & WT_CONV1_WGRAD) ? 1 : 0;
-    static_assert(sizeof(C1wArgs) == 56, "the index block follows at byte 56 of the argument segment");
+    static_assert(sizeof(C1wArgs) == 56, "the index block follows at byte 64 + 56 of the argument segment");
     const dim3 grid(CRS1 / 32, 1, Conv1Wgrad::nbz(a));
     IdxIn ix; memset(ix.v, 0, sizeof ix.v);
+    Lead l; memset(&l, 0, sizeof l);
+    l.p[0] = c.src; l.p[1] = c.d1; l.p[2] = c.slab1; l.p[3] = c.idx; l.B = c.B; l.s0 = c.tps1; l.s1 = c.Kt;
+    l.ctl = c.xcd | c.pad_ << 1 | (c.from_ring ? 4 : 0) | (a.arg_preload && a.B < 128 && grid.z < 32768u ? LEAD_ON : 0) | (int)(grid.z << 16);
     if (t.host_idx && a.from_ring && a.B <= 32) {
       memcpy(ix.v, t.host_idx, (size_t)a.B * sizeof(int64_t));
-      SDQN_LAUNCH(conv1_wgrad_bf16_kernel<true>, grid, dim3(1024), 0, s, c, ix);
-    } else SDQN_LAUNCH(conv1_wgrad_bf16_kernel<false>, grid, dim3(1024), 0, s, c, ix);
+      SDQN_LAUNCH(conv1_wgrad_bf16_kernel<true>, grid, dim3(1024), 0, s, SDQN_LEAD_ARGS(l), c, ix);
+    } else SDQN_LAUNCH(conv1_wgrad_bf16_kernel<false>, grid, dim3(1024), 0, s, SDQN_LEAD_ARGS(l), c, ix);
     return hipGetLastError();
   }
   if (a.B <= 32 && a.h16 == 2 && !a.bn && t.wt && !(id >= 0 && id < 12 && t.nw_override[id] > 0)) {
@@ -613,8 +645,11 @@
   if (id == K_CONV3_FWD && (t.variant & LV_CONV3_C36) && a.B < 128 && !a.h16 && !a.bn) {
     static_assert(CRS3 == 16 * 36, "conv3's K is 16 chunks of 36");
     const dim3 grid((Conv3Fwd::M(a) + 31) / 32, (Conv3Fwd::N(a) + 31) / 32, Conv3Fwd::nbz(a));
-    if ((t.wt & WT_CONV3_FWD) && a.B <= 32) SDQN_LAUNCH((gemm36_kernel<Conv3FwdWT>), grid, dim3(1024), 0, s, a);
-    else SDQN_LAUNCH((gemm36_kernel<Conv3Fwd>), grid, dim3(1024), 0, s, a);
+    Lead l; memset(&l, 0, sizeof l);
+    if ((t.wt & WT_CONV3_FWD) && a.B <= 32) {
+      Conv3FwdWT::lead_pack(a, l); l.B = a.B; l.s0 = lead_grid(grid); l.ctl = lead_ctl(a, a.arg_preload && lead_grid_fits(grid));
+      SDQN_LAUNCH((gemm36_kernel<Conv3FwdWT>), grid, dim3(1024), 0, s, SDQN_LEAD_ARGS(l), a);
+    } else SDQN_LAUNCH((gemm36_kernel<Conv3Fwd>), grid, dim3(1024), 0, s, SDQN_LEAD_ARGS(l), a);
     return hipGetLastError();
   }
   *handled = false;
diff --git a/simple_dqn_amd/csrc/update_body.h b/simple_dqn_amd/csrc/update_body.h
--- a/simple_dqn_amd/csrc/update_body.h
+++ b/simple_dqn_amd/csrc/update_body.h
@@ -46,8 +46,10 @@
 constexpr int CONV_BLOCKS = CONV_F4 / 32;
 constexpr int FC5_BLOCKS_PER_ACTION = NFC / 4 / 32;
 
+struct UpdHot { float* theta; float* state; const float* slab; int ns, mode, only_fc4, A; };
+__device__ __forceinline__ int upd_layer(int bid) { const int64_t e = (int64_t)bid * 128; return e < OFF2 ? 0 : (e < OFF3 ? 1 : 2); }
 template <bool OVF>
-__device__ __forceinline__ void update_body(const UpdateArgs& u, const int bid, const int nblocks, float4 (*part)[32], float* cost_sh) {
+__device__ __forceinline__ void update_body(const UpdateArgs& u, const UpdHot& hot, const int arg_off, const int bid, const int nblocks, float4 (*part)[32], float* cost_sh) {
   const int t = threadIdx.x;
 #ifdef SDQN_TIMING
   SDQN_STAMP(0);
@@ -62,22 +64,22 @@
       else if (u.ovf_dynamic && ++st[2] >= 200) { st[2] = 0; if (st[1] < 15) st[1] += 1; }
     }
   }
-  if (u.only_fc4 && bid < CONV_BLOCKS + u.A * FC5_BLOCKS_PER_ACTION) return;
+  if (hot.only_fc4 && bid < CONV_BLOCKS + hot.A * FC5_BLOCKS_PER_ACTION) return;
   if (bid < CONV_BLOCKS) {
     const int c4 = t & 31, sg = t >> 5;
     const int64_t e = ((int64_t)bid * 32 + c4) * 4;
     float4 gs = make_float4(0.f, 0.f, 0.f, 0.f);
     float4 pre[2] = {gs, gs};
-    const bool applies = sg == 0 && u.mode != 1 && !skip_apply;
-    if (applies) { pre[0] = *reinterpret_cast<const float4*>(u.theta + e); pre[1] = *reinterpret_cast<const float4*>(u.state + e); }
-    if (u.mode == 2) {
+    const bool applies = sg == 0 && hot.mode != 1 && !skip_apply;
+    if (applies) { pre[0] = *reinterpret_cast<const float4*>(hot.theta + e); pre[1] = *reinterpret_cast<const float4*>(hot.state + e); }
+    if (hot.mode == 2) {
       if (sg == 0) gs = *reinterpret_cast<const float4*>(u.g + e);
     } else {
       const int L = e < OFF2 ? 0 : (e < OFF3 ? 1 : 2);
       const int64_t off = e - (L == 0 ? OFF1 : (L == 1 ? OFF2 : OFF3));
       const int64_t nw = L == 0 ? NW1 : (L == 1 ? NW2 : NW3);
-      const float* sp = u.slab[L] + off;
-      const int ns = u.ns[L];
+      const float* sp = hot.slab + off;
+      const int ns = hot.ns;
       if (ns > 32) {
         for (int s = sg; s < ns; s += 128) {
           float4 v[16];
@@ -104,10 +106,10 @@
         *reinterpret_cast<float4*>(u.g + e) = gs;
       }
     }
-    if (applies) opt_apply4(u.theta, u.state, u.state2, e, gs, u, pre);
+    if (applies) opt_apply4(hot.theta, hot.state, u.state2, e, gs, u, pre);
     return;
   }
-  const int fc5_blocks = u.A * FC5_BLOCKS_PER_ACTION;
+  const int fc5_blocks = hot.A * FC5_BLOCKS_PER_ACTION;
   if (bid < CONV_BLOCKS + fc5_blocks) {
     const int fb = bid - CONV_BLOCKS, c4 = t & 31, sg = t >> 5;
     const int act = fb / FC5_BLOCKS_PER_ACTION, j0 = ((fb - act * FC5_BLOCKS_PER_ACTION) * 32 + c4) * 4;
@@ -155,7 +157,7 @@
     }
   }
   if (u.next.B > 0 && bid == first_dense) {
-    const char* ka = (const char*)__builtin_amdgcn_kernarg_segment_ptr() + offsetof(UpdateArgs, next) + offsetof(PrepArgs, idx_in);
+    const char* ka = (const char*)__builtin_amdgcn_kernarg_segment_ptr() + arg_off + offsetof(UpdateArgs, next) + offsetof(PrepArgs, idx_in);
     for (int n = t; n < u.next.B; n += 256) {
       const int64_t i = u.next.idx_in_valid ? *reinterpret_cast<const int64_t*>(ka + 8 * (n & 31)) : u.next.idx_pinned[n];
       u.next.idx[n] = i;
```
